# puzzlepaint/surfelmeshing

Measured on NVIDIA H100. Metric: RGB-D frames/s at 640x480 (depth pre-processing + Integrate()), higher is better.
Workload: dtype f32

## Files before the change

### surfelmeshing_b200/csrc/api.cu

```cuda

#include <algorithm>
#include <atomic>
#include <chrono>
#include <cstdio>
#include <cstdlib>
#include <cstring>
#include <limits>
#include <mutex>
#include <string>
#include <vector>

#include "sm_handle.cuh"

namespace smb {

namespace {
thread_local std::string g_last_error;
std::atomic<unsigned long long> g_launches{0};
}

int SetError(int code, const char* message) {
  g_last_error = message ? message : "";
  return code;
}
// ... 143 lines not shown
}

using namespace smb;

#define SM_CUDA(call)                                                                        \
  do {                                                                                       \
    const cudaError_t e_ = (call);                                                           \
    if (e_ != cudaSuccess) {                                                                 \
      g_last_error = std::string(#call) + ": " + cudaGetErrorString(e_);                     \
      return SM_ERR_CUDA;                                                                    \
    }                                                                                        \
  } while (0)

namespace smb {

int FetchCounters(sm_reconstruction* r, cudaStream_t stream) {
  SM_CUDA(cudaMemcpyAsync(r->host_counters, r->d.counters, sizeof(Counters), cudaMemcpyDeviceToHost, stream));
  SM_CUDA(cudaStreamSynchronize(stream));
  if (r->host_counters->capacity_overflow) {
    return SetError(SM_ERR_CAPACITY, "surfel cap exceeded: new surfels of at least one frame were dropped "
                                     "(the reference writes out of bounds here)");
  }
  return SM_OK;
}

FrameParams MakeFrameParams(const sm_reconstruction* r, u32 frame_index, int count_slot, const sm_integrate_params& p,
                            u16* depth, size_t depth_pitch, const u16* depth_pre, size_t depth_pre_pitch,
                            const float* normals, size_t normals_pitch, const float* radius, size_t radius_pitch,
                            const uint8_t* color, size_t color_pitch, const float* global_T_local,
                            const float* local_T_global) {
  FrameParams f;
  f.frame_index = frame_index;
  f.count_slot = count_slot;
  f.skip = 0;
  f.op_epoch = r->op_epoch;
  f.tb = MakeTieBreak(r->tiebreak, frame_index);
  f.active_window = p.surfel_integration_active_window_size;
  f.fx = r->fx; f.fy = r->fy; f.cx = r->cx; f.cy = r->cy;
  f.fx_inv = 1.0f / r->fx;
  f.fy_inv = 1.0f / r->fy;
  const float cx_pixel_center = r->cx - 0.5f;
  const float cy_pixel_center = r->cy - 0.5f;
  f.cx_inv = -cx_pixel_center / r->fx;
  f.cy_inv = -cy_pixel_center / r->fy;
  f.sensor_noise_factor = p.sensor_noise_factor;
  f.cos_normal_compatibility_threshold = cosf(M_PI / 180.0f * p.normal_compatibility_threshold_deg);
  f.max_surfel_confidence = p.max_surfel_confidence;
  f.inv_depth_scaling = 1.0f / p.depth_scaling;
  f.depth_scaling = 1.0f / f.inv_depth_scaling;
  f.radius_factor_squared =
      p.radius_factor_for_regularization_neighbors * p.radius_factor_for_regularization_neighbors;
  f.blend_radius = p.measurement_blending_radius;
  f.local_T_global = MakeMat3x4(local_T_global);
  f.global_T_local = MakeMat3x4(global_T_local);
  f.depth = depth; f.depth_pitch = depth_pitch;
  f.depth_pre = depth_pre; f.depth_pre_pitch = depth_pre_pitch;
  f.normals = reinterpret_cast<const float2*>(normals); f.normals_pitch = normals_pitch;
  f.radius = radius; f.radius_pitch = radius_pitch;
  f.color = reinterpret_cast<const uchar3*>(color); f.color_pitch = color_pitch;
  return f;
}

int IntegrateImpl(sm_reconstruction* r, cudaStream_t stream, u32 frame_index, const sm_integrate_params& p,
                  u16* depth, size_t depth_pitch, const float* normals, size_t normals_pitch, const float* radius,
                  size_t radius_pitch, const uint8_t* color, size_t color_pitch, const float* global_T_local,
                  const float* local_T_global) {
  r->last_stream = stream;
  RecordOperation(r, static_cast<int>(frame_index - static_cast<u32>(p.regularization_frame_window_size)));
  const u16* depth_pre = depth;
  size_t depth_pre_pitch = depth_pitch;
  if (p.do_blending) {
    SM_CUDA(cudaMemcpy2DAsync(r->blend_src, r->blend_src_pitch, depth, depth_pitch, r->d.width * sizeof(u16),
                              r->d.height, cudaMemcpyDeviceToDevice, stream));
    depth_pre = r->blend_src;
    depth_pre_pitch = r->blend_src_pitch;
  }
  const FrameParams f = MakeFrameParams(r, frame_index, r->count_slot, p, depth, depth_pitch, depth_pre, depth_pre_pitch,
                                        normals, normals_pitch, radius, radius_pitch, color, color_pitch,
                                        global_T_local, local_T_global);
  r->last_tiebreak = f.tb;
  int status = IntegrateFrame(stream, r->d, f, p.do_blending != 0, r->rasters_cleared, r->plan, &r->events);
  r->rasters_cleared = false;
  if (status != SM_OK) return status;
  const int old_slot = r->count_slot;
  r->count_slot = (r->count_slot + 1) % kCountSlots;
  if (r->events.enabled) cudaEventRecord(r->events.ev[12], stream);
  const int iterations = p.regularization_iterations_per_integration_iteration;
  if (iterations == 0) {
    status = RegularizeSurfels(stream, r->d,  true, frame_index,
                               p.radius_factor_for_regularization_neighbors, p.regularizer_weight,
                               p.regularization_frame_window_size, r->count_slot, old_slot, r->plan);
  } else {
    for (int i = 0; i < iterations && status == SM_OK; ++i) {
      status = RegularizeSurfels(stream, r->d,  false, frame_index,
                                 p.radius_factor_for_regularization_neighbors, p.regularizer_weight,
                                 p.regularization_frame_window_size, r->count_slot, i == 0 ? old_slot : -1, r->plan);
    }
  }
  if (r->events.enabled) cudaEventRecord(r->events.ev[13], stream);
  return status;
}

}

namespace {

int CreateImpl(sm_reconstruction* r, uint64_t max_surfel_count, int32_t width, int32_t height, float fx, float fy,
               float cx, float cy) {
  SM_CUDA(cudaGetDevice(&r->device));
  cudaDeviceProp prop;
  SM_CUDA(cudaGetDeviceProperties(&prop, r->device));
  r->sm_count = prop.multiProcessorCount;
  r->plan.sm_count = r->sm_count;
  {
    const char* e = std::getenv("SM_B200_CARVEOUT");
    const int percent = e ? std::atoi(e) : 47;
    int status = ConfigurePreprocessKernels(percent);
    if (status == SM_OK) status = ConfigureIntegrateKernels(percent, &r->plan);
    if (status == SM_OK) status = ConfigureRegularizeKernels(percent, &r->plan);
    if (status != SM_OK) return status;
  }
  r->fx = fx; r->fy = fy; r->cx = cx; r->cy = cy;
  DeviceState& d = r->d;
  d.width = width; d.height = height;
  d.capacity = static_cast<u32>(max_surfel_count);
  const size_t padded = (max_surfel_count + kSegment - 1) / kSegment * kSegment;
  d.stride = padded;
  const size_t P = static_cast<size_t>(width) * height;
  const size_t scan_tiles = (P + kSegment - 1) / kSegment;
  SM_CUDA(cudaMalloc(&d.surfels, sizeof(float) * SM_ROW_COUNT * d.stride));
  SM_CUDA(cudaMalloc(&d.gradient, sizeof(float4) * d.stride));
  SM_CUDA(cudaMalloc(&r->smooth_alt, sizeof(float) * 3 * d.stride));
  d.smooth = d.surfels + static_cast<size_t>(SM_ROW_SMOOTH_X) * d.stride;
  d.smooth_next = r->smooth_alt;
  SM_CUDA(cudaMemset(d.gradient, 0, sizeof(float4) * d.stride));
  for (int i = 0; i < kSets; ++i) {
    SM_CUDA(cudaMalloc(&r->assoc_set[i], sizeof(PixelAssoc) * P));
    SM_CUDA(cudaMalloc(&r->first_depth_set[i], sizeof(float) * P));
    SM_CUDA(cudaMalloc(&r->supported_set[i], P));
    SM_CUDA(cudaMalloc(&r->vis_set[i], sizeof(VisEntry) * padded));
    SM_CUDA(cudaMalloc(&r->seg_count_set[i], sizeof(u32) * (padded / kSegment)));
    SM_CUDA(cudaMalloc(&r->merge_flag_set[i], padded));
  }
  d.assoc = r->assoc_set[0]; d.first_depth = r->first_depth_set[0]; d.supported = r->supported_set[0];
  d.vis = r->vis_set[0]; d.seg_count = r->seg_count_set[0]; d.merge_flag = r->merge_flag_set[0];
  SM_CUDA(cudaMalloc(&d.new_list, sizeof(u32) * P));
  SM_CUDA(cudaMalloc(&d.new_flag, P));
  SM_CUDA(cudaMalloc(&d.new_index, sizeof(u32) * P));
  SM_CUDA(cudaMalloc(&d.scan_state, sizeof(unsigned long long) * scan_tiles));
  SM_CUDA(cudaMalloc(&d.counters, sizeof(Counters)));
  SM_CUDA(cudaMemset(d.counters, 0, sizeof(Counters)));
  d.timeline = nullptr;
  d.timeline_frames = 0;
  SM_CUDA(cudaMemset(d.new_flag, 0, P));
  SM_CUDA(cudaMemset(d.new_index, 0, sizeof(u32) * P));
  SM_CUDA(cudaMemset(d.scan_state, 0, sizeof(unsigned long long) * scan_tiles));
  SM_CUDA(cudaMallocHost(&r->host_counters, sizeof(Counters)));
  std::memset(r->host_counters, 0, sizeof(Counters));
  SM_CUDA(cudaMallocPitch(reinterpret_cast<void**>(&r->scratch_B), &r->scratch_B_pitch, width * sizeof(u16), height));
  SM_CUDA(cudaMallocPitch(reinterpret_cast<void**>(&r->blend_src), &r->blend_src_pitch, width * sizeof(u16), height));
  {
    const char* e = std::getenv("SM_B200_TAIL_FILL");
    const bool want_tma = !(e && std::string(e) == "vector");
    if (want_tma) {
      const int status = MakeDepthTensorMap(&r->scratch_B_map, r->scratch_B, r->scratch_B_pitch, width, height);
      if (status != SM_OK) return status;
      r->scratch_B_map_valid = true;
    }
  }
  for (int i = 0; i < 14; ++i) SM_CUDA(cudaEventCreate(&r->events.ev[i]));
  r->events.enabled = false;
  {
    u32 wave = kDefaultTieBreakWave, lanes = 1u << kDefaultTieBreakLaneShift;
    double early = kDefaultTieBreakEarlyFraction, index_order = kDefaultTieBreakIndexOrderFraction;
    u32 offset = kDefaultTieBreakWaveOffset;
    if (const char* e = std::getenv("SM_B200_TIEBREAK")) {
      unsigned w = 0, l = 0, o = 0; double q = 0, b = 0;
      const int got = std::sscanf(e, "%u,%lf,%lf,%u,%u", &w, &q, &b, &l, &o);
      if (got >= 2) { wave = w; early = q; }
      if (got >= 3) index_order = b;
      if (got >= 4) lanes = l;
      if (got >= 5) offset = o ? 1u : 0u;
    }
    r->tiebreak.wave_offset = offset;
    u32 lane_shift = 0;
    while ((1u << lane_shift) < lanes && lane_shift < 10) ++lane_shift;
    if (wave != 0 && (static_cast<unsigned long long>(d.capacity) / wave + 2) * 2ull * wave >= 0xFFFFFFFFull) wave = 0;
    r->tiebreak.lane_request = lane_shift;
    const int status = SetTieBreakWave(&r->tiebreak, wave, d.capacity);
    if (status != SM_OK) return status;
    r->tiebreak.early_fraction = early;
    r->tiebreak.index_order_fraction = index_order;
    r->tiebreak.early_fraction_later = kDefaultTieBreakEarlyFractionLater;
    r->tiebreak.index_order_fraction_later = kDefaultTieBreakIndexOrderFractionLater;
    r->tiebreak.early_fraction_second = kDefaultTieBreakEarlyFractionSecond;
  }
  const int status = ClearAssociationRasters(nullptr, d);
  if (status != SM_OK) return status;
  SM_CUDA(cudaDeviceSynchronize());
  return SM_OK;
}

}

extern "C" {

void sm_default_integrate_params(sm_integrate_params* p) {
  p->depth_scaling = 5000;
  p->sensor_noise_factor = 0.05f;
  p->max_surfel_confidence = 5.0f;
  p->regularizer_weight = 10.0f;
  p->regularization_frame_window_size = 30;
  p->do_blending = 1;
  p->measurement_blending_radius = 12;
  p->regularization_iterations_per_integration_iteration = 1;
  p->radius_factor_for_regularization_neighbors = 2;
  p->normal_compatibility_threshold_deg = 40;
  p->surfel_integration_active_window_size = std::numeric_limits<int>::max();
}

void sm_default_preprocess_params(sm_preprocess_params* p) {
  p->depth_scaling = 5000;
  p->max_depth = 3.0f;
  p->depth_valid_region_radius = 333;
  p->bilateral_filter_sigma_xy = 3;
  p->bilateral_filter_radius_factor = 2.0f;
  p->bilateral_filter_sigma_depth_factor = 0.05;
  p->outlier_filtering_frame_count = 8;
  p->outlier_filtering_required_inliers = -1;
  p->outlier_filtering_depth_tolerance_factor = 0.02f;
  p->depth_erosion_radius = 2;
  p->observation_angle_threshold_deg = 85;
  p->point_radius_extension_factor = 1.5f;
  p->point_radius_clamp_factor = std::numeric_limits<float>::infinity();
}

const char* sm_last_error(void) { return g_last_error.c_str(); }
const char* sm_version(void) { return "surfel_b200 0.1 (sm_90a)"; }
uint64_t sm_kernel_launch_count(void) { return g_launches.load(); }

int sm_profile_kernels(int32_t enable) {
  std::lock_guard<std::mutex> lock(g_profile_mutex);
  g_profile_enabled = enable != 0;
  return SM_OK;
}

int32_t sm_profile_kernel_count(void) { return KID_COUNT; }
const char* sm_profile_kernel_name(int32_t id) { return KernelName(id); }

int sm_profile_report(double* total_ms, uint64_t* launches, int32_t n) {
  SM_CUDA(cudaDeviceSynchronize());
  std::lock_guard<std::mutex> lock(g_profile_mutex);
  for (int i = 0; i < n; ++i) { total_ms[i] = 0; launches[i] = 0; }
  for (const ProfileRecord& r : g_profile_records) {
    float ms = 0;
    if (cudaEventElapsedTime(&ms, r.start, r.stop) == cudaSuccess && r.id < n) {
      total_ms[r.id] += ms;
      launches[r.id] += 1;
    }
    g_event_pool.push_back(r.start);
    g_event_pool.push_back(r.stop);
  }
  g_profile_records.clear();
  return SM_OK;
}

int sm_create(sm_reconstruction** out, uint64_t max_surfel_count, int32_t width, int32_t height, float fx, float fy,
              float cx, float cy) {
  if (out) *out = nullptr;
  if (!out || width <= 0 || height <= 0 || max_surfel_count == 0 || max_surfel_count > 0x7FFFFFFFull - kSegment) {
    return SetError(SM_ERR_INVALID_ARGUMENT, "sm_create: bad argument");
  }
  sm_reconstruction* r = new sm_reconstruction();
  const int status = CreateImpl(r, max_surfel_count, width, height, fx, fy, cx, cy);
  if (status != SM_OK) {
    const std::string message = g_last_error;
    sm_destroy(r);
    g_last_error = message;
    return status;
  }
  *out = r;
  return SM_OK;
}

int sm_destroy(sm_reconstruction* r) {
  if (!r) return SM_OK;
  cudaDeviceSynchronize();
  cudaGetLastError();
  DestroyFrameGraph(r->graph);
  DeviceState& d = r->d;
  cudaFree(d.surfels); cudaFree(d.gradient); cudaFree(r->smooth_alt); cudaFree(d.new_list);
  for (int i = 0; i < kSets; ++i) {
    cudaFree(r->vis_set[i]); cudaFree(r->seg_count_set[i]); cudaFree(r->merge_flag_set[i]);
    cudaFree(r->assoc_set[i]); cudaFree(r->first_depth_set[i]); cudaFree(r->supported_set[i]);
    cudaFree(r->run_depth[i]); cudaFree(r->run_depth_pre[i]); cudaFree(r->run_normals[i]); cudaFree(r->run_radius[i]);
  }
  cudaFree(d.new_flag); cudaFree(d.new_index); cudaFree(d.scan_state); cudaFree(d.counters);
  cudaFree(d.timeline);
  if (r->host_counters) cudaFreeHost(r->host_counters);
  cudaFree(r->scratch_B);
  cudaFree(r->blend_src);
  cudaFree(r->median_stage[0]); cudaFree(r->median_stage[1]);
  cudaFree(r->pyramid_depth_stage); cudaFree(r->pyramid_color_stage);
  FreeTransferBuffers(r);
  for (int i = 0; i < 2; ++i) {
    if (r->pipe.ev_create[i]) cudaEventDestroy(r->pipe.ev_create[i]);
    if (r->pipe.ev_update[i]) cudaEventDestroy(r->pipe.ev_update[i]);
    if (r->pre_done[i]) cudaEventDestroy(r->pre_done[i]);
    if (r->int_done[i]) cudaEventDestroy(r->int_done[i]);
  }
  for (cudaStream_t st : {r->pre_stream, r->pipe.crit, r->pipe.front, r->pipe.side, r->upload_stream, r->graph_stream})
    if (st) cudaStreamDestroy(st);
  for (cudaEvent_t e : {r->pipe.ev_assoc, r->pipe.ev_merge, r->pipe.ev_blend, r->pipe.ev_integrate, r->pipe.ev_reg,
                        r->entry_event, r->upload_done, r->graph_exit})
    if (e) cudaEventDestroy(e);
  for (cudaEvent_t e : r->iteration_done) if (e) cudaEventDestroy(e);
  for (u16* b : r->ring_depth) cudaFree(b);
  for (uchar3* b : r->ring_color) cudaFree(b);
  for (int i = 0; i < 14; ++i) if (r->events.ev[i]) cudaEventDestroy(r->events.ev[i]);
  delete r;
  cudaGetLastError();
  return SM_OK;
}

int sm_reset(sm_reconstruction* r, void* stream) {
  SM_CUDA(cudaMemsetAsync(r->d.counters, 0, sizeof(Counters), static_cast<cudaStream_t>(stream)));
  r->count_slot = 0;
  r->rasters_cleared = false;
  r->last_stream = static_cast<cudaStream_t>(stream);
  ++r->state_generation;
  r->op_history.clear();
  return SM_OK;
}

int sm_preprocess(sm_reconstruction* r, void* stream, const sm_preprocess_params* p, const uint16_t* raw_depth,
                  size_t raw_pitch, const uint16_t* const* other_depths, const size_t* other_pitches,
                  const float* others_TR_reference, uint16_t* out_depth, size_t out_depth_pitch, float* out_normals,
                  size_t out_normals_pitch, float* out_radius, size_t out_radius_pitch) {
  const int status = PreprocessFused(static_cast<cudaStream_t>(stream), *p, r->d.width, r->d.height, r->fx, r->fy,
                                     r->cx, r->cy, raw_depth, raw_pitch, other_depths, other_pitches,
                                     others_TR_reference, r->scratch_B, r->scratch_B_pitch, out_depth,
                                     out_depth_pitch, reinterpret_cast<float2*>(out_normals), out_normals_pitch,
                                     out_radius, out_radius_pitch, r->d.assoc, r->d.first_depth, r->d.supported, nullptr, 0,
                                     nullptr, nullptr, r->ScratchBMap());
  if (status == SM_OK) r->rasters_cleared = true;
  return status;
}

int sm_bilateral_filter_and_depth_cutoff(void* stream, float sigma_xy, float sigma_value_factor,
                                         uint16_t value_to_ignore, float radius_factor, uint16_t max_depth,
                                         float depth_valid_region_radius, int32_t width, int32_t height,
                                         const uint16_t* in_depth, size_t in_pitch, uint16_t* out_depth,
                                         size_t out_pitch) {
  return StageBilateral(static_cast<cudaStream_t>(stream), sigma_xy, sigma_value_factor, value_to_ignore,
                        radius_factor, max_depth, depth_valid_region_radius, width, height, in_depth, in_pitch,
                        out_depth, out_pitch);
}

int sm_outlier_depth_map_fusion(void* stream, int32_t other_count, int32_t required_count, float tolerance, float fx,
                                float fy, float cx, float cy, int32_t width, int32_t height, const uint16_t* in_depth,
                                size_t in_pitch, const uint16_t* const* other_depths, const size_t* other_pitches,
                                const float* others_TR_reference, uint16_t* out_depth, size_t out_pitch) {
  return StageOutlier(static_cast<cudaStream_t>(stream), other_count, required_count, tolerance, fx, fy, cx, cy,
                      width, height, in_depth, in_pitch, other_depths, other_pitches, others_TR_reference, out_depth,
                      out_pitch);
}

int sm_median_filter_and_densify_depth_map(void* stream, int32_t iterations, int32_t width, int32_t height,
                                           const uint16_t* in_depth, size_t in_pitch, uint16_t* out_depth,
                                           size_t out_pitch, uint16_t* scratch, size_t scratch_pitch) {
  return StageMedianDensify(static_cast<cudaStream_t>(stream), iterations, width, height, in_depth, in_pitch, out_depth,
                            out_pitch, scratch, scratch_pitch);
}

int sm_downscale_using_median_while_excluding(void* stream, uint16_t value_to_ignore, int32_t in_width,
                                              int32_t in_height, const uint16_t* in, size_t in_pitch,
// ... 62 lines not shown
  return status;
}

int sm_transfer_all_to_cpu(sm_reconstruction* r, void* stream_v, uint32_t , float* x, float* y,
                           float* z, float* radius_squared, float* nx, float* ny, float* nz,
                           uint32_t* last_update_stamp, uint64_t* out_count) {
  cudaStream_t stream = static_cast<cudaStream_t>(stream_v);
  const int status = FetchCounters(r, stream);
  const u32 n = r->host_counters->surfel_count[r->count_slot];
  if (out_count) *out_count = n;
  if (n == 0) return status;
  const size_t bytes = sizeof(float) * n;
  const float* s = r->d.surfels;
  const size_t st = r->d.stride;
  SM_CUDA(cudaMemcpyAsync(x, r->d.smooth + 0 * st, bytes, cudaMemcpyDeviceToHost, stream));
  SM_CUDA(cudaMemcpyAsync(y, r->d.smooth + 1 * st, bytes, cudaMemcpyDeviceToHost, stream));
  SM_CUDA(cudaMemcpyAsync(z, r->d.smooth + 2 * st, bytes, cudaMemcpyDeviceToHost, stream));
  SM_CUDA(cudaMemcpyAsync(radius_squared, s + SM_ROW_RADIUS_SQUARED * st, bytes, cudaMemcpyDeviceToHost, stream));
  SM_CUDA(cudaMemcpyAsync(nx, s + SM_ROW_NORMAL_X * st, bytes, cudaMemcpyDeviceToHost, stream));
  SM_CUDA(cudaMemcpyAsync(ny, s + SM_ROW_NORMAL_Y * st, bytes, cudaMemcpyDeviceToHost, stream));
  SM_CUDA(cudaMemcpyAsync(nz, s + SM_ROW_NORMAL_Z * st, bytes, cudaMemcpyDeviceToHost, stream));
  SM_CUDA(cudaMemcpyAsync(last_update_stamp, s + SM_ROW_LAST_UPDATE_STAMP * st, bytes, cudaMemcpyDeviceToHost, stream));
  return status;
}

int sm_transfer_delta_to_cpu(sm_reconstruction* r, void* stream, uint32_t frame_index, sm_transfer_token* token,
                             float* x, float* y, float* z, float* radius_squared, float* nx, float* ny, float* nz,
                             uint32_t* last_update_stamp, sm_transfer_stats* stats) {
  if (!r || !token) return SetError(SM_ERR_INVALID_ARGUMENT, "sm_transfer_delta_to_cpu: null argument");
  return TransferDelta(r, static_cast<cudaStream_t>(stream), frame_index, token, x, y, z, radius_squared, nx, ny, nz,
                       last_update_stamp, stats);
}

int sm_update_visualization_buffers(sm_reconstruction* r, void* stream, const sm_visualization_params* p,
                                    float* vertex_buffer, uint32_t* neighbor_index_buffer, float* normal_vertex_buffer) {
  if (!r || !p) return SetError(SM_ERR_INVALID_ARGUMENT, "sm_update_visualization_buffers: null argument");
  return UpdateVisualizationBuffers(r, static_cast<cudaStream_t>(stream), *p, vertex_buffer, neighbor_index_buffer,
                                    normal_vertex_buffer);
}

int sm_export_vertices(sm_reconstruction* r, void* stream, float* position_buffer, uint8_t* color_buffer) {
  return ExportVertices(static_cast<cudaStream_t>(stream), r->d, r->count_slot, r->sm_count, position_buffer,
                        color_buffer);
}

int sm_get_timings(sm_reconstruction* r, float out_ms[7]) {
  if (!r->events.enabled) return SetError(SM_ERR_INVALID_ARGUMENT, "timings are not enabled (sm_enable_timings)");
  SM_CUDA(cudaEventSynchronize(r->events.ev[13]));
  for (int i = 0; i < 7; ++i) SM_CUDA(cudaEventElapsedTime(&out_ms[i], r->events.ev[2 * i], r->events.ev[2 * i + 1]));
  return SM_OK;
}

int sm_enable_timings(sm_reconstruction* r, int32_t enable) {
  r->events.enabled = enable != 0;
  return SM_OK;
}

int sm_dump_state(sm_reconstruction* r, void* stream_v, float* host_rows, uint64_t host_row_stride_elems,
                  uint32_t* surfels_size, uint32_t* merge_count) {
  cudaStream_t stream = static_cast<cudaStream_t>(stream_v);
  const int status = FetchCounters(r, stream);
  const u32 n = r->host_counters->surfel_count[r->count_slot];
  if (surfels_size) *surfels_size = n;
  if (merge_count) *merge_count = r->host_counters->merge_count;
  if (host_rows && n > host_row_stride_elems) return SetError(SM_ERR_INVALID_ARGUMENT, "sm_dump_state: host rows shorter than surfels_size()");
  if (host_rows && n > 0) {
    SM_CUDA(cudaMemcpy2DAsync(host_rows, host_row_stride_elems * sizeof(float), r->d.surfels,
                              r->d.stride * sizeof(float), n * sizeof(float), SM_ROW_COUNT, cudaMemcpyDeviceToHost,
                              stream));
    SM_CUDA(cudaMemcpy2DAsync(host_rows + SM_ROW_SMOOTH_X * host_row_stride_elems, host_row_stride_elems * sizeof(float),
                              r->d.smooth, r->d.stride * sizeof(float), n * sizeof(float), 3, cudaMemcpyDeviceToHost,
                              stream));
    SM_CUDA(cudaStreamSynchronize(stream));
  }
  return status;
}

int sm_load_state(sm_reconstruction* r, void* stream_v, const float* host_rows, uint64_t host_row_stride_elems,
                  uint32_t surfels_size, uint32_t merge_count) {
  cudaStream_t stream = static_cast<cudaStream_t>(stream_v);
  if (surfels_size > r->d.capacity) return SetError(SM_ERR_CAPACITY, "sm_load_state: state larger than the surfel cap");
  r->d.smooth = r->d.surfels + static_cast<size_t>(SM_ROW_SMOOTH_X) * r->d.stride;
  r->d.smooth_next = r->smooth_alt;
  if (surfels_size > 0) {
    SM_CUDA(cudaMemcpy2DAsync(r->d.surfels, r->d.stride * sizeof(float), host_rows,
                              host_row_stride_elems * sizeof(float), surfels_size * sizeof(float), SM_ROW_COUNT,
                              cudaMemcpyHostToDevice, stream));
    SM_CUDA(cudaMemsetAsync(r->d.gradient, 0, surfels_size * sizeof(float4), stream));
    const int zero_rows[4] = {SM_ROW_GRADIENT_X, SM_ROW_GRADIENT_Y, SM_ROW_GRADIENT_Z, SM_ROW_GRADIENT_COUNT};
    for (int row : zero_rows) {
      SM_CUDA(cudaMemsetAsync(r->d.surfels + row * r->d.stride, 0, surfels_size * sizeof(float), stream));
    }
    SM_CUDA(cudaMemsetAsync(r->d.surfels + kRowMergeEpoch * r->d.stride, 0, surfels_size * sizeof(float), stream));
    const int status = RebuildMetaRow(stream, r->d, surfels_size, r->sm_count);
    if (status != SM_OK) return status;
  }
  Counters c{};
  for (int i = 0; i < kCountSlots; ++i) c.surfel_count[i] = surfels_size;
  c.merge_count = merge_count;
  *r->host_counters = c;
  SM_CUDA(cudaMemcpyAsync(r->d.counters, r->host_counters, sizeof(Counters), cudaMemcpyHostToDevice, stream));
  SM_CUDA(cudaStreamSynchronize(stream));
  r->count_slot = 0;
  r->last_stream = stream;
  ++r->state_generation;
  r->op_history.clear();
  return SM_OK;
}

int sm_download_rasters(sm_reconstruction* r, void* stream_v, uint32_t* supporting_surfels,
                        uint32_t* supporting_surfel_counts, float* supporting_surfel_depth_sums,
                        uint32_t* conflicting_surfels, float* first_surfel_depth, uint8_t* new_surfel_flag_vector,
                        uint32_t* new_surfel_indices) {
  cudaStream_t stream = static_cast<cudaStream_t>(stream_v);
  const size_t P = static_cast<size_t>(r->d.width) * r->d.height;
  std::vector<PixelAssoc> assoc(P);
  SM_CUDA(cudaMemcpyAsync(assoc.data(), r->d.assoc, sizeof(PixelAssoc) * P, cudaMemcpyDeviceToHost, stream));
  if (first_surfel_depth)
    SM_CUDA(cudaMemcpyAsync(first_surfel_depth, r->d.first_depth, sizeof(float) * P, cudaMemcpyDeviceToHost, stream));
  if (new_surfel_flag_vector)
    SM_CUDA(cudaMemcpyAsync(new_surfel_flag_vector, r->d.new_flag, P, cudaMemcpyDeviceToHost, stream));
  if (new_surfel_indices)
    SM_CUDA(cudaMemcpyAsync(new_surfel_indices, r->d.new_index, sizeof(u32) * P, cudaMemcpyDeviceToHost, stream));
  SM_CUDA(cudaStreamSynchronize(stream));
  for (size_t i = 0; i < P; ++i) {
    if (supporting_surfels) supporting_surfels[i] = supporting_index(r->last_tiebreak, assoc[i].x, static_cast<u32>(i));
    if (conflicting_surfels) conflicting_surfels[i] = assoc[i].y;
    if (supporting_surfel_counts) supporting_surfel_counts[i] = assoc[i].z;
    if (supporting_surfel_depth_sums) std::memcpy(&supporting_surfel_depth_sums[i], &assoc[i].w, sizeof(float));
  }
  return SM_OK;
}

int sm_frame_counters(sm_reconstruction* r, void* stream_v, uint64_t out[4]) {
  cudaStream_t stream = static_cast<cudaStream_t>(stream_v);
  const int status = FetchCounters(r, stream);
  const u32 n_after = r->host_counters->surfel_count[r->count_slot];
  const u32 n_swept = n_after - r->host_counters->new_surfel_count;
  const size_t segments = (static_cast<size_t>(n_swept) + kSegment - 1) / kSegment;
  std::vector<u32> seg(segments);
  if (segments) SM_CUDA(cudaMemcpy(seg.data(), r->d.seg_count, sizeof(u32) * segments, cudaMemcpyDeviceToHost));
  uint64_t visible = 0;
  for (u32 c : seg) visible += c;
  const size_t P = static_cast<size_t>(r->d.width) * r->d.height;
  std::vector<PixelAssoc> assoc(P);
  SM_CUDA(cudaMemcpy(assoc.data(), r->d.assoc, sizeof(PixelAssoc) * P, cudaMemcpyDeviceToHost));
  uint64_t support = 0;
  for (const PixelAssoc& a : assoc) support += a.z;
  out[0] = n_swept; out[1] = visible; out[2] = support; out[3] = r->host_counters->new_surfel_count;
  return status;
}

int sm_timeline_enable(sm_reconstruction* r, int32_t frames) {
  if (r == nullptr || frames < 0) return SetError(SM_ERR_INVALID_ARGUMENT, "sm_timeline_enable: bad arguments");
  SM_CUDA(cudaDeviceSynchronize());
  if (r->d.timeline) {
    cudaFree(r->d.timeline);
    r->d.timeline = nullptr;
    r->d.timeline_frames = 0;
  }
  if (frames == 0) return SM_OK;
  const size_t slots = static_cast<size_t>(frames) * KID_COUNT;
  SM_CUDA(cudaMalloc(&r->d.timeline, slots * 2 * sizeof(unsigned long long)));
  std::vector<unsigned long long> init(slots * 2);
  for (size_t i = 0; i < slots; ++i) { init[2 * i] = ~0ull; init[2 * i + 1] = 0ull; }
  SM_CUDA(cudaMemcpy(r->d.timeline, init.data(), init.size() * sizeof(unsigned long long), cudaMemcpyHostToDevice));
// ... 69 lines not shown
```

### surfelmeshing_b200/csrc/integrate.cu

```cuda

#include <algorithm>
#include <cstdio>
#include <cstdlib>

#include "sm_kernels.cuh"

namespace smb {

namespace {

#define SM_S(row, i) d.surfels[static_cast<size_t>(row) * d.stride + (i)]
#define SM_SU(row, i) reinterpret_cast<u32*>(d.surfels)[static_cast<size_t>(row) * d.stride + (i)]
#define SM_SMOOTH(axis, i) d.smooth[static_cast<size_t>(axis) * d.stride + (i)]

constexpr int kBlock = 256;

__device__ __forceinline__ bool is_active(u32 last_update_stamp, u32 frame_index, int window) {
  return static_cast<int>(last_update_stamp) > static_cast<int>(frame_index - static_cast<u32>(window));
}

struct Projection {
  float u, v;
  int px, py;
  bool in_image;
};

__device__ __forceinline__ Projection project(const FrameParams& f, int width, int height, float x, float y, float z) {
  Projection p;
  const float inv_z = frcp(z);
  p.u = ffma(fmul(x, inv_z), f.fx, f.cx);
  p.v = ffma(fmul(y, inv_z), f.fy, f.cy);
  p.px = f2i_trunc(p.u);
  p.py = f2i_trunc(p.v);
  p.in_image = !(p.u < 0.f || p.v < 0.f || p.px < 0 || p.py < 0 || p.px >= width || p.py >= height);
  return p;
}

__device__ __forceinline__ bool secondary_pixel(const Projection& p, int width, int height, int* ox, int* oy) {
  const float x_frac = fsub(p.u, i2f(p.px));
  const float y_frac = fsub(p.v, i2f(p.py));
  if (x_frac < y_frac) {
    if (x_frac < fadd(-y_frac, 1.0f)) {
      if (p.px > 1) { *ox = p.px - 1; *oy = p.py; return true; }
      return false;
    }
    if (p.py < height - 1) { *ox = p.px; *oy = p.py + 1; return true; }
    return false;
  }
  if (x_frac < fadd(-y_frac, 1.0f)) {
    if (p.py > 0) { *ox = p.px; *oy = p.py - 1; return true; }
    return false;
  }
  if (p.px < width - 1) { *ox = p.px + 1; *oy = p.py; return true; }
  return false;
}

__device__ __forceinline__ float normal_z_abs(float nx, float ny) {
  return fsqrt_approx(fmaxf(0.f, ffma(-ny, ny, ffma(-nx, nx, 1.0f))));
}

__device__ __forceinline__ float facing_dot(const FrameParams& f, float x, float y, float z, float nx, float ny,
                                            float nz, float3* local_normal) {
  const float rs = frsqrt_approx(squared_norm(x, y, z));
  *local_normal = rotate_vec(f.local_T_global, nx, ny, nz);
  return fmul(rs, ffma(z, local_normal->z, ffma(x, local_normal->x, fmul(y, local_normal->y))));
}

template <typename Body>
__device__ __forceinline__ void for_each_visible(const DeviceState& d, const u32* surfel_count, Body&& body) {
  constexpr u32 kItemsPerSegment = kSegment / kBlock;
  const u32 max_items = ((d.capacity + kSegment - 1) / kSegment) * kItemsPerSegment;
  const u32 n = *surfel_count;
  u32 item = blockIdx.x;
  u32 cnt = 0;
  VisEntry e = make_uint4(0u, 0u, 0u, 0u);
  if (item < max_items) {
    cnt = d.seg_count[item / kItemsPerSegment];
    e = d.vis[static_cast<size_t>(item) * kBlock + threadIdx.x];
  }
  const u32 items = ((n + kSegment - 1) / kSegment) * kItemsPerSegment;
  while (item < items) {
    const u32 next = item + gridDim.x;
    u32 cnt_next = 0;
    VisEntry e_next = e;
    if (next < items) {
      cnt_next = d.seg_count[next / kItemsPerSegment];
      e_next = d.vis[static_cast<size_t>(next) * kBlock + threadIdx.x];
    }
    const u32 k = (item % kItemsPerSegment) * kBlock + threadIdx.x;
    if (k < cnt) body(static_cast<size_t>(item) * kBlock + threadIdx.x, e);
    item = next;
    cnt = cnt_next;
    e = e_next;
  }
}

__global__ void __launch_bounds__(kBlock) k_clear(DeviceState d) {
  pdl_prologue();
  const int n = d.width * d.height;
  for (int i = blockIdx.x * blockDim.x + threadIdx.x; i < n; i += gridDim.x * blockDim.x) {
    d.assoc[i] = make_uint4(kInvalidIndex, kInvalidIndex, 0u, 0u);
    d.first_depth[i] = __int_as_float(0x7f800000);
    d.supported[i] = 0;
  }
}

constexpr int kProjectBlock = 512;

enum { kProjectAll = 0, kProjectMain = 1, kProjectTail = 2 };

__global__ void __launch_bounds__(kProjectBlock) k_project(DeviceState d, FrameParams f, int part) {
  pdl_prologue();
  if (f.skip) return;
  const TimelineScope timeline_scope(d, f.frame_index, part == kProjectTail ? KID_PROJECT_TAIL : KID_PROJECT);
  __shared__ u32 warp_totals[kProjectBlock / 32];
  const int lane = threadIdx.x & 31, warp = threadIdx.x >> 5;
  const u32 first_seg_if_all = blockIdx.x;

  if (blockIdx.x == 0 && part != kProjectMain) {
    const int tiles = (d.width * d.height + kSegment - 1) / kSegment;
    for (int t = threadIdx.x; t < tiles; t += blockDim.x) d.scan_state[t] = 0ull;
    if (threadIdx.x == 0) d.counters->scan_ticket = 0;
  }

  struct SlotRows { float2 X, Y, Z; uint2 T; };
  auto fetch = [&](u32 seg) {
    SlotRows r;
    const size_t base = static_cast<size_t>(seg) * kSegment + threadIdx.x * 2;
    r.X = *reinterpret_cast<const float2*>(&SM_S(SM_ROW_X, base));
    r.Y = *reinterpret_cast<const float2*>(&SM_S(SM_ROW_Y, base));
    r.Z = *reinterpret_cast<const float2*>(&SM_S(SM_ROW_Z, base));
    r.T = *reinterpret_cast<const uint2*>(&SM_SU(SM_ROW_LAST_UPDATE_STAMP, base));
    return r;
  };
  SlotRows rows = {};
  if (part != kProjectTail && (static_cast<size_t>(first_seg_if_all) + 1) * kSegment <= d.stride) rows = fetch(first_seg_if_all);
  const u32 n_before = part == kProjectAll ? 0u : d.counters->surfel_count[(f.count_slot + kCountSlots - 1) % kCountSlots];
  const u32 seg_begin = part == kProjectTail ? n_before / kSegment : 0u;
  const u32 n = part == kProjectMain ? (n_before / kSegment) * kSegment
                                     : d.counters->surfel_count[f.count_slot];
  if (part == kProjectTail && static_cast<u64>(seg_begin + blockIdx.x) * kSegment < n) rows = fetch(seg_begin + blockIdx.x);
  for (u32 seg = seg_begin + blockIdx.x; static_cast<u64>(seg) * kSegment < n; seg += gridDim.x) {
    const u32 base = seg * kSegment + threadIdx.x * 2;
    const SlotRows cur = rows;
    if (static_cast<u64>(seg + gridDim.x) * kSegment < n) rows = fetch(seg + gridDim.x);
    VisEntry e[2];
    bool visible[2] = {false, false};
    u32 cnt = 0;
    if (base < n) {
      const float xs[2] = {cur.X.x, cur.X.y}, ys[2] = {cur.Y.x, cur.Y.y}, zs[2] = {cur.Z.x, cur.Z.y};
      const u32 ts[2] = {cur.T.x, cur.T.y};
#pragma unroll
      for (int j = 0; j < 2; ++j) {
        const u32 i = base + j;
        if (i >= n) break;
        const float z = transform_row(f.local_T_global.r2, xs[j], ys[j], zs[j]);
        if (!(z > 0.f)) continue;
        const float x = transform_row(f.local_T_global.r0, xs[j], ys[j], zs[j]);
        const float y = transform_row(f.local_T_global.r1, xs[j], ys[j], zs[j]);
        const Projection p = project(f, d.width, d.height, x, y, z);
        if (!p.in_image) continue;
        const bool active = is_active(ts[j], f.frame_index, f.active_window);
        e[j] = make_uint4(i | (active ? kActiveBit : 0u), __float_as_uint(x), __float_as_uint(y), __float_as_uint(z));
        visible[j] = true;
        ++cnt;
        if (active) {
          atomicMin(reinterpret_cast<int*>(&d.first_depth[p.py * d.width + p.px]), __float_as_int(z));
          int ox, oy;
          if (secondary_pixel(p, d.width, d.height, &ox, &oy)) {
            atomicMin(reinterpret_cast<int*>(&d.first_depth[oy * d.width + ox]), __float_as_int(z));
          }
        }
      }
    }
    u32 incl = cnt;
#pragma unroll
    for (int o = 1; o < 32; o <<= 1) {
      const u32 t = __shfl_up_sync(0xffffffffu, incl, o);
      if (lane >= o) incl += t;
    }
    if (lane == 31) warp_totals[warp] = incl;
    __syncthreads();
    u32 warp_base = 0, total = 0;
#pragma unroll
    for (int w = 0; w < kProjectBlock / 32; ++w) {
      const u32 t = warp_totals[w];
      if (w < warp) warp_base += t;
      total += t;
    }
    VisEntry* out = d.vis + static_cast<size_t>(seg) * kSegment + warp_base + (incl - cnt);
#pragma unroll
    for (int j = 0; j < 2; ++j) {
      if (visible[j]) *out++ = e[j];
    }
    if (threadIdx.x == 0) d.seg_count[seg] = total;
    __syncthreads();
  }
}


struct PixelGate {
  float measurement_depth;
  float first;
  float2 normal;
};
// ... 504 lines not shown
}

__device__ __forceinline__ void integrate_or_conflict(const FrameParams& f, const PixelMeasurement& m, int x, int y,
                                                      u32 idx, float cx_, float cy_, float cz_, SurfelState& s) {
  if (!(m.measurement_depth > 0.f)) return;
  bool integrate = true, conflicting = false;
  if (m.first < fmul(m.measurement_depth, fadd(-f.sensor_noise_factor, 1.0f))) {
    if (m.first == cz_ && m.conflicting == idx) conflicting = true;
    integrate = false;
  }
  if (!integrate && !conflicting) return;
  if (cz_ > fmul(fadd(f.sensor_noise_factor, 1.0f), m.measurement_depth)) integrate = false;
  if (!integrate && !conflicting) return;

  const float lx = fmul(m.measurement_depth, ffma(i2f(x), f.fx_inv, f.cx_inv));
  const float ly = fmul(m.measurement_depth, ffma(i2f(y), f.fy_inv, f.cy_inv));
  const float3 g = transform_point(f.global_T_local, lx, ly, m.measurement_depth);
  const float3 gn = rotate_vec(f.global_T_local, m.normal.x, m.normal.y, -normal_z_abs(m.normal.x, m.normal.y));

  if (conflicting) {
    const float confidence = fadd(s.confidence, -1.0f);
    if (confidence <= 0.f) {
      s.x = g.x; s.y = g.y; s.z = g.z;
      s.smooth_x = g.x; s.smooth_y = g.y; s.smooth_z = g.z;
      s.nx = gn.x; s.ny = gn.y; s.nz = gn.z;
      s.color = m.r | (m.g << 8) | (m.b << 16) | (1u << 24);
      s.radius_squared = m.radius_squared;
      s.confidence = 1.0f;
      s.creation_stamp = f.frame_index;
      s.stamped = true;
      s.replaced = true;
    } else {
      s.confidence = confidence;
    }
    s.dirty = true;
  }
  if (!integrate) return;

  float3 ln;
  if (facing_dot(f, cx_, cy_, cz_, s.nx, s.ny, s.nz, &ln) > 0.f) return;
  if (m.measurement_depth < cz_) {
    if (ffma(gn.z, s.nz, ffma(gn.x, s.nx, fmul(gn.y, s.ny))) < f.cos_normal_compatibility_threshold) return;
  }
  if (s.radius_squared < 0.f) return;

  const float weight = frcp(u2f(max(1u, m.count)));
  if (s.creation_stamp < f.frame_index) {
    const float confidence = s.confidence;
    const float cw = fadd(weight, confidence);
    s.confidence = (cw < f.max_surfel_confidence) ? cw : f.max_surfel_confidence;
    const float normalization_factor = frcp(cw);
    s.x = fmul(normalization_factor, ffma(g.x, weight, fmul(confidence, s.x)));
    s.y = fmul(normalization_factor, ffma(g.y, weight, fmul(confidence, s.y)));
    s.z = fmul(normalization_factor, ffma(g.z, weight, fmul(confidence, s.z)));
    const float nx = ffma(gn.x, weight, fmul(confidence, s.nx));
    const float ny = ffma(gn.y, weight, fmul(confidence, s.ny));
    const float nz = ffma(gn.z, weight, fmul(confidence, s.nz));
    const float normal_normalization = frsqrt_approx(ffma(nz, nz, ffma(nx, nx, fmul(ny, ny))));
    s.nx = fmul(nx, normal_normalization);
    s.ny = fmul(ny, normal_normalization);
    s.nz = fmul(nz, normal_normalization);
    s.radius_squared = fminf(s.radius_squared, m.radius_squared);
    const u32 old_color = s.color;
    const u32 r = f2u_trunc(ffma(normalization_factor, ffma(u2f(m.r), weight, fmul(confidence, u2f(old_color & 0xFFu))), 0.5f));
    const u32 gr = f2u_trunc(ffma(normalization_factor, ffma(u2f(m.g), weight, fmul(confidence, u2f((old_color >> 8) & 0xFFu))), 0.5f));
    const u32 b = f2u_trunc(ffma(normalization_factor, ffma(u2f(m.b), weight, fmul(confidence, u2f((old_color >> 16) & 0xFFu))), 0.5f));
    s.color = (r & 0xFFu) | ((gr & 0xFFu) << 8) | ((b & 0xFFu) << 16);
    s.stamped = true;
    s.dirty = true;
  }
}

#ifndef SM_INTEGRATE_LEVELS
#define SM_INTEGRATE_LEVELS 2
#endif

__device__ __forceinline__ bool pixel_can_touch(const FrameParams& f, float measurement_depth, float first, u32 conflicting,
                                                u32 idx, float cz_) {
  if (!(measurement_depth > 0.f)) return false;
  if (first < fmul(measurement_depth, fadd(-f.sensor_noise_factor, 1.0f))) return first == cz_ && conflicting == idx;
  return !(cz_ > fmul(fadd(f.sensor_noise_factor, 1.0f), measurement_depth));
}

__global__ void __launch_bounds__(kBlock, 4) k_integrate(DeviceState d, FrameParams f) {
  pdl_prologue();
  if (f.skip) return;
  const TimelineScope timeline_scope(d, f.frame_index, KID_INTEGRATE);
  for_each_visible(d, &d.counters->surfel_count[f.count_slot], [&](size_t pos, const VisEntry& e) {
    const u32 idx = e.x & ~kActiveBit;
    const float x = __uint_as_float(e.y), y = __uint_as_float(e.z), z = __uint_as_float(e.w);
    const Projection p = project(f, d.width, d.height, x, y, z);
    int ox = p.px, oy = p.py;
    const bool has2 = secondary_pixel(p, d.width, d.height, &ox, &oy);
    const u8 merged = d.merge_flag[pos];
    SurfelState s;
    PixelMeasurement m0, m1;
#if SM_INTEGRATE_LEVELS == 1
    m0 = load_pixel_measurement(d, f, p.px, p.py);
    m1 = load_pixel_measurement(d, f, ox, oy);
    s.x = SM_S(SM_ROW_X, idx); s.y = SM_S(SM_ROW_Y, idx); s.z = SM_S(SM_ROW_Z, idx);
    s.confidence = SM_S(SM_ROW_CONFIDENCE, idx);
    s.radius_squared = SM_S(SM_ROW_RADIUS_SQUARED, idx);
    s.nx = SM_S(SM_ROW_NORMAL_X, idx); s.ny = SM_S(SM_ROW_NORMAL_Y, idx); s.nz = SM_S(SM_ROW_NORMAL_Z, idx);
    s.color = SM_SU(SM_ROW_COLOR, idx);
    s.creation_stamp = SM_SU(SM_ROW_CREATION_STAMP, idx);
#else
    const int p0 = p.py * d.width + p.px, p1 = oy * d.width + ox;
    m0.measurement_depth = fmul(u2f(row_ptr(f.depth, f.depth_pitch, p.py)[p.px]), f.inv_depth_scaling);
    m1.measurement_depth = fmul(u2f(row_ptr(f.depth, f.depth_pitch, oy)[ox]), f.inv_depth_scaling);
    m0.first = d.first_depth[p0];
    m1.first = d.first_depth[p1];
    const PixelAssoc a0 = d.assoc[p0], a1 = d.assoc[p1];
    m0.conflicting = a0.y; m0.count = a0.z;
    m1.conflicting = a1.y; m1.count = a1.z;
    s.radius_squared = SM_S(SM_ROW_RADIUS_SQUARED, idx);
#endif
    s.last_update_stamp = 0;
    s.smooth_x = s.smooth_y = s.smooth_z = 0.f;
    s.replaced = false; s.dirty = false; s.stamped = false;
    if (merged) {
      SM_SU(SM_ROW_LAST_UPDATE_STAMP, idx) = 0;
      SM_S(SM_ROW_RADIUS_SQUARED, idx) = -1.0f;
      reinterpret_cast<u8*>(&SM_SU(SM_ROW_COLOR, idx))[3] = 1;
      SM_SU(kRowMeta, idx) = kMetaDetachBit;
      SM_SU(kRowMergeEpoch, idx) = f.op_epoch;
      return;
    }
    if (!(e.x & kActiveBit)) return;
    if (s.radius_squared < 0.f) return;
#if SM_INTEGRATE_LEVELS != 1
    const bool touch0 = pixel_can_touch(f, m0.measurement_depth, m0.first, m0.conflicting, idx, z);
    const bool touch1 = has2 && pixel_can_touch(f, m1.measurement_depth, m1.first, m1.conflicting, idx, z);
    if (!touch0 && !touch1) return;
    {
      const int qx0 = touch0 ? p.px : ox, qy0 = touch0 ? p.py : oy;
      const int qx1 = touch1 ? ox : qx0, qy1 = touch1 ? oy : qy0;
      m0.normal = row_ptr(f.normals, f.normals_pitch, qy0)[qx0];
      m1.normal = row_ptr(f.normals, f.normals_pitch, qy1)[qx1];
      m0.radius_squared = row_ptr(f.radius, f.radius_pitch, qy0)[qx0];
      m1.radius_squared = row_ptr(f.radius, f.radius_pitch, qy1)[qx1];
      const uchar3 c0 = row_ptr(f.color, f.color_pitch, qy0)[qx0];
      const uchar3 c1 = row_ptr(f.color, f.color_pitch, qy1)[qx1];
      m0.r = c0.x; m0.g = c0.y; m0.b = c0.z;
      m1.r = c1.x; m1.g = c1.y; m1.b = c1.z;
      s.x = SM_S(SM_ROW_X, idx); s.y = SM_S(SM_ROW_Y, idx); s.z = SM_S(SM_ROW_Z, idx);
      s.confidence = SM_S(SM_ROW_CONFIDENCE, idx);
      s.nx = SM_S(SM_ROW_NORMAL_X, idx); s.ny = SM_S(SM_ROW_NORMAL_Y, idx); s.nz = SM_S(SM_ROW_NORMAL_Z, idx);
      s.color = SM_SU(SM_ROW_COLOR, idx);
      s.creation_stamp = SM_SU(SM_ROW_CREATION_STAMP, idx);
    }
    if (touch0) integrate_or_conflict(f, m0, p.px, p.py, idx, x, y, z, s);
    if (touch1) integrate_or_conflict(f, m1, ox, oy, idx, x, y, z, s);
#else
    integrate_or_conflict(f, m0, p.px, p.py, idx, x, y, z, s);
    if (has2) integrate_or_conflict(f, m1, ox, oy, idx, x, y, z, s);
#endif
    if (!s.dirty) return;
    SM_S(SM_ROW_X, idx) = s.x; SM_S(SM_ROW_Y, idx) = s.y; SM_S(SM_ROW_Z, idx) = s.z;
    SM_S(SM_ROW_CONFIDENCE, idx) = s.confidence;
    SM_S(SM_ROW_RADIUS_SQUARED, idx) = s.radius_squared;
    SM_S(SM_ROW_NORMAL_X, idx) = s.nx; SM_S(SM_ROW_NORMAL_Y, idx) = s.ny; SM_S(SM_ROW_NORMAL_Z, idx) = s.nz;
    SM_SU(SM_ROW_COLOR, idx) = s.color;
    if (s.stamped) {
      SM_SU(SM_ROW_LAST_UPDATE_STAMP, idx) = f.frame_index;
      SM_SU(kRowMeta, idx) = f.frame_index | (((s.color >> 24) & 1u) ? kMetaDetachBit : 0u);
    }
    if (s.replaced) {
      SM_SMOOTH(0, idx) = s.smooth_x; SM_SMOOTH(1, idx) = s.smooth_y; SM_SMOOTH(2, idx) = s.smooth_z;
      SM_SU(SM_ROW_CREATION_STAMP, idx) = f.frame_index;
#pragma unroll
      for (int i = 0; i < 4; ++i) SM_SU(SM_ROW_NEIGHBOR0 + i, idx) = kInvalidIndex;
    }
  });
}

#ifndef SM_UPDATE_ANYNEW_FIRST
#define SM_UPDATE_ANYNEW_FIRST 0
#endif
#ifndef SM_UPDATE_EARLY_GATE
#define SM_UPDATE_EARLY_GATE 1
#endif
#ifndef SM_UPDATE_COMPACT
#define SM_UPDATE_COMPACT 0
#endif

#ifndef SM_UPDATE_COMPACT_MIN_BLOCKS
#define SM_UPDATE_COMPACT_MIN_BLOCKS 3
#endif
#if SM_UPDATE_COMPACT
__device__ __forceinline__ void update_neighbors_survivor(const DeviceState& d, const FrameParams& f, u32 idx, int x, int y) {
  const int kDirectionsX[4] = {-1, 1, 0, 0};
  const int kDirectionsY[4] = {0, 0, -1, 1};
  const float gx = SM_S(SM_ROW_X, idx), gy = SM_S(SM_ROW_Y, idx), gz = SM_S(SM_ROW_Z, idx);
  const float nx = SM_S(SM_ROW_NORMAL_X, idx), ny = SM_S(SM_ROW_NORMAL_Y, idx), nz = SM_S(SM_ROW_NORMAL_Z, idx);
  const float radius_squared = SM_S(SM_ROW_RADIUS_SQUARED, idx);
  u32 neighbor_surfel_indices[4];
#pragma unroll
  for (int m = 0; m < 4; ++m) neighbor_surfel_indices[m] = SM_SU(SM_ROW_NEIGHBOR0 + m, idx);
  const float observation_radius_squared = row_ptr(f.radius, f.radius_pitch, y)[x];
  u32 candidate[4];
#pragma unroll
  for (int direction = 0; direction < 4; ++direction) {
    const int candidate_pixel = (y + kDirectionsY[direction]) * d.width + x + kDirectionsX[direction];
    candidate[direction] = supporting_index(f.tb, d.assoc[candidate_pixel].x, static_cast<u32>(candidate_pixel));
  }
  const float cz_ = transform_row(f.local_T_global.r2, gx, gy, gz);
  const float cx_ = transform_row(f.local_T_global.r0, gx, gy, gz);
  const float cy_ = transform_row(f.local_T_global.r1, gx, gy, gz);
  float3 ln;
  if (facing_dot(f, cx_, cy_, cz_, nx, ny, nz, &ln) > 0.f) return;
  if (radius_squared < 0.f) return;
  if (fmul(observation_radius_squared, frcp(radius_squared)) > 2.25f) return;
  bool any_new = false;
#pragma unroll
  for (int direction = 0; direction < 4; ++direction) {
    const u32 q = candidate[direction];
    if (q == kInvalidIndex || q == idx) { candidate[direction] = kInvalidIndex; continue; }
    any_new |= q != neighbor_surfel_indices[0] && q != neighbor_surfel_indices[1] &&
               q != neighbor_surfel_indices[2] && q != neighbor_surfel_indices[3];
  }
  if (!any_new) return;

  float neighbor_distances_squared[4];
#pragma unroll
  for (int m = 0; m < 4; ++m) {
    const u32 q = neighbor_surfel_indices[m];
    if (q == kInvalidIndex) {
      neighbor_distances_squared[m] = __int_as_float(0x7f800000);
    } else {
      neighbor_distances_squared[m] = squared_norm(fsub(gx, SM_S(SM_ROW_X, q)), fsub(gy, SM_S(SM_ROW_Y, q)),
                                                   fsub(gz, SM_S(SM_ROW_Z, q)));
    }
  }
  const float max_distance_squared = fmul(radius_squared, f.radius_factor_squared);
  float cand_distance[4], cand_dot[4];
#pragma unroll
  for (int direction = 0; direction < 4; ++direction) {
    const u32 q = candidate[direction];
    if (q == kInvalidIndex) continue;
    cand_distance[direction] = squared_norm(fsub(SM_S(SM_ROW_X, q), gx), fsub(SM_S(SM_ROW_Y, q), gy),
                                            fsub(SM_S(SM_ROW_Z, q), gz));
    cand_dot[direction] = dot3(nx, ny, nz, SM_S(SM_ROW_NORMAL_X, q), SM_S(SM_ROW_NORMAL_Y, q), SM_S(SM_ROW_NORMAL_Z, q));
  }
  bool changed = false;
#pragma unroll
  for (int direction = 0; direction < 4; ++direction) {
    const u32 q = candidate[direction];
    if (q == kInvalidIndex) continue;
    const float distance_squared = cand_distance[direction];
    if (distance_squared > max_distance_squared) continue;
    if (cand_dot[direction] <= 0.f) continue;
    int best_n = -1;
    float best_distance_squared = -1.f;
#pragma unroll
    for (int m = 0; m < 4; ++m) {
      if (q == neighbor_surfel_indices[m]) { best_n = -1; break; }
      if (neighbor_distances_squared[m] > best_distance_squared) {
        best_n = m;
        best_distance_squared = neighbor_distances_squared[m];
      }
    }
    if (best_n >= 0 && distance_squared < best_distance_squared) {
#pragma unroll
      for (int m = 0; m < 4; ++m) {
        if (m == best_n) { neighbor_surfel_indices[m] = q; neighbor_distances_squared[m] = distance_squared; }
      }
      changed = true;
    }
  }
  if (changed) {
#pragma unroll
    for (int m = 0; m < 4; ++m) SM_SU(SM_ROW_NEIGHBOR0 + m, idx) = neighbor_surfel_indices[m];
  }
}

__global__ void __launch_bounds__(kBlock, SM_UPDATE_COMPACT_MIN_BLOCKS) k_update_neighbors(DeviceState d, FrameParams f) {
  pdl_prologue();
  if (f.skip) return;
  const TimelineScope timeline_scope(d, f.frame_index, KID_UPDATE_NEIGHBORS);
  constexpr int kPerThread = kSegment / kBlock;
  constexpr int kBorder = 1;
  __shared__ u32 s_survivor[kSegment];
  __shared__ u32 s_pixel[kSegment];
  __shared__ u32 s_count;
  const u32 n = d.counters->surfel_count[f.count_slot];
  const u32 segments = (n + kSegment - 1) / kSegment;
  const int lane = threadIdx.x & 31;
  for (u32 segment = blockIdx.x; segment < segments; segment += gridDim.x) {
    if (threadIdx.x == 0) s_count = 0;
    __syncthreads();
    const u32 cnt = d.seg_count[segment];
    u32 surfel[kPerThread], stamp[kPerThread];
    float gx[kPerThread], gy[kPerThread], gz[kPerThread];
    u16 raw_depth[kPerThread];
    int cached_px[kPerThread], cached_py[kPerThread];
    bool live[kPerThread];
    {
      VisEntry e[kPerThread];
#pragma unroll
      for (int u = 0; u < kPerThread; ++u) {
        const u32 k = u * kBlock + threadIdx.x;
        live[u] = k < cnt;
        if (live[u]) e[u] = d.vis[static_cast<size_t>(segment) * kSegment + k];
      }
#pragma unroll
      for (int u = 0; u < kPerThread; ++u) {
        if (!live[u]) continue;
        surfel[u] = e[u].x & ~kActiveBit;
        const Projection cached = project(f, d.width, d.height, __uint_as_float(e[u].y), __uint_as_float(e[u].z), __uint_as_float(e[u].w));
        cached_px[u] = cached.px;
        cached_py[u] = cached.py;
      }
    }
#pragma unroll
    for (int u = 0; u < kPerThread; ++u) {
      if (!live[u]) continue;
      const u32 idx = surfel[u];
      stamp[u] = SM_SU(SM_ROW_LAST_UPDATE_STAMP, idx);
      gx[u] = SM_S(SM_ROW_X, idx); gy[u] = SM_S(SM_ROW_Y, idx); gz[u] = SM_S(SM_ROW_Z, idx);
      raw_depth[u] = row_ptr(f.depth, f.depth_pitch, cached_py[u])[cached_px[u]];
    }
#pragma unroll
    for (int u = 0; u < kPerThread; ++u) {
      bool pass = live[u];
      int x = 0, y = 0;
      if (pass) pass = is_active(stamp[u], f.frame_index, f.active_window);
      if (pass) {
        const float cz_ = transform_row(f.local_T_global.r2, gx[u], gy[u], gz[u]);
        pass = cz_ > 0.f;
        if (pass) {
          const float cx_ = transform_row(f.local_T_global.r0, gx[u], gy[u], gz[u]);
          const float cy_ = transform_row(f.local_T_global.r1, gx[u], gy[u], gz[u]);
          const float inv_z = frcp(cz_);
          x = f2i_trunc(ffma(fmul(cx_, inv_z), f.fx, f.cx));
          y = f2i_trunc(ffma(fmul(cy_, inv_z), f.fy, f.cy));
          pass = !(x < kBorder || y < kBorder || x >= d.width - kBorder || y >= d.height - kBorder);
          if (pass) {
            u16 depth_here = raw_depth[u];
            if (x != cached_px[u] || y != cached_py[u]) depth_here = row_ptr(f.depth, f.depth_pitch, y)[x];
            const float measurement_depth = fmul(u2f(depth_here), f.inv_depth_scaling);
            pass = !(cz_ > fmul(measurement_depth, fadd(f.sensor_noise_factor, 1.0f)));
          }
        }
      }
      const unsigned ballot = __ballot_sync(0xFFFFFFFFu, pass);
      if (ballot) {
        u32 base = 0;
        if (lane == 0) base = atomicAdd(&s_count, static_cast<u32>(__popc(ballot)));
        base = __shfl_sync(0xFFFFFFFFu, base, 0);
        if (pass) {
          const u32 slot = base + __popc(ballot & ((1u << lane) - 1u));
          s_survivor[slot] = surfel[u];
          s_pixel[slot] = static_cast<u32>(x) | (static_cast<u32>(y) << 16);
        }
      }
    }
    __syncthreads();
    const u32 survivors = s_count;
    for (u32 q = threadIdx.x; q < survivors; q += kBlock) {
      const u32 pixel = s_pixel[q];
      update_neighbors_survivor(d, f, s_survivor[q], static_cast<int>(pixel & 0xFFFFu), static_cast<int>(pixel >> 16));
    }
    __syncthreads();
  }
}
#else
__global__ void __launch_bounds__(kBlock) k_update_neighbors(DeviceState d, FrameParams f) {
  pdl_prologue();
  if (f.skip) return;
  const TimelineScope timeline_scope(d, f.frame_index, KID_UPDATE_NEIGHBORS);
  for_each_visible(d, &d.counters->surfel_count[f.count_slot], [&](size_t, const VisEntry& e) {
    const u32 idx = e.x & ~kActiveBit;
    constexpr int kBorder = 1;
    const int kDirectionsX[4] = {-1, 1, 0, 0};
    const int kDirectionsY[4] = {0, 0, -1, 1};
#if SM_UPDATE_EARLY_GATE
    const Projection cached = project(f, d.width, d.height, __uint_as_float(e.y), __uint_as_float(e.z), __uint_as_float(e.w));
    const u32 stamp = SM_SU(SM_ROW_LAST_UPDATE_STAMP, idx);
    const float gx = SM_S(SM_ROW_X, idx), gy = SM_S(SM_ROW_Y, idx), gz = SM_S(SM_ROW_Z, idx);
    u16 raw_depth = row_ptr(f.depth, f.depth_pitch, cached.py)[cached.px];
    if (!is_active(stamp, f.frame_index, f.active_window)) return;
    const float cz_ = transform_row(f.local_T_global.r2, gx, gy, gz);
    if (!(cz_ > 0.f)) return;
    const float cx_ = transform_row(f.local_T_global.r0, gx, gy, gz);
    const float cy_ = transform_row(f.local_T_global.r1, gx, gy, gz);
    const float inv_z = frcp(cz_);
    const int x = f2i_trunc(ffma(fmul(cx_, inv_z), f.fx, f.cx));
    const int y = f2i_trunc(ffma(fmul(cy_, inv_z), f.fy, f.cy));
    if (x < kBorder || y < kBorder || x >= d.width - kBorder || y >= d.height - kBorder) return;
    if (x != cached.px || y != cached.py) raw_depth = row_ptr(f.depth, f.depth_pitch, y)[x];
    const float measurement_depth = fmul(u2f(raw_depth), f.inv_depth_scaling);
    if (cz_ > fmul(measurement_depth, fadd(f.sensor_noise_factor, 1.0f))) return;
#if SM_UPDATE_ANYNEW_FIRST
    u32 neighbor_surfel_indices[4];
#pragma unroll
    for (int m = 0; m < 4; ++m) neighbor_surfel_indices[m] = SM_SU(SM_ROW_NEIGHBOR0 + m, idx);
    u32 candidate[4];
#pragma unroll
    for (int direction = 0; direction < 4; ++direction) {
      const int candidate_pixel = (y + kDirectionsY[direction]) * d.width + x + kDirectionsX[direction];
      candidate[direction] = supporting_index(f.tb, d.assoc[candidate_pixel].x, static_cast<u32>(candidate_pixel));
    }
    {
      bool any_new_first = false;
#pragma unroll
      for (int direction = 0; direction < 4; ++direction) {
        const u32 q = candidate[direction];
        if (q == kInvalidIndex || q == idx) continue;
        any_new_first |= q != neighbor_surfel_indices[0] && q != neighbor_surfel_indices[1] &&
                         q != neighbor_surfel_indices[2] && q != neighbor_surfel_indices[3];
      }
      if (!any_new_first) return;
    }
    const float nx = SM_S(SM_ROW_NORMAL_X, idx), ny = SM_S(SM_ROW_NORMAL_Y, idx), nz = SM_S(SM_ROW_NORMAL_Z, idx);
    const float radius_squared = SM_S(SM_ROW_RADIUS_SQUARED, idx);
    const float observation_radius_squared = row_ptr(f.radius, f.radius_pitch, y)[x];
#else
    const float nx = SM_S(SM_ROW_NORMAL_X, idx), ny = SM_S(SM_ROW_NORMAL_Y, idx), nz = SM_S(SM_ROW_NORMAL_Z, idx);
    const float radius_squared = SM_S(SM_ROW_RADIUS_SQUARED, idx);
    u32 neighbor_surfel_indices[4];
#pragma unroll
    for (int m = 0; m < 4; ++m) neighbor_surfel_indices[m] = SM_SU(SM_ROW_NEIGHBOR0 + m, idx);
    const float observation_radius_squared = row_ptr(f.radius, f.radius_pitch, y)[x];
    u32 candidate[4];
#pragma unroll
    for (int direction = 0; direction < 4; ++direction) {
      const int candidate_pixel = (y + kDirectionsY[direction]) * d.width + x + kDirectionsX[direction];
      candidate[direction] = supporting_index(f.tb, d.assoc[candidate_pixel].x, static_cast<u32>(candidate_pixel));
    }
#endif
#else
    const u32 stamp = SM_SU(SM_ROW_LAST_UPDATE_STAMP, idx);
    const float gx = SM_S(SM_ROW_X, idx), gy = SM_S(SM_ROW_Y, idx), gz = SM_S(SM_ROW_Z, idx);
    const float nx = SM_S(SM_ROW_NORMAL_X, idx), ny = SM_S(SM_ROW_NORMAL_Y, idx), nz = SM_S(SM_ROW_NORMAL_Z, idx);
    const float radius_squared = SM_S(SM_ROW_RADIUS_SQUARED, idx);
    u32 neighbor_surfel_indices[4];
#pragma unroll
    for (int m = 0; m < 4; ++m) neighbor_surfel_indices[m] = SM_SU(SM_ROW_NEIGHBOR0 + m, idx);
    if (!is_active(stamp, f.frame_index, f.active_window)) return;
    const float cz_ = transform_row(f.local_T_global.r2, gx, gy, gz);
    if (!(cz_ > 0.f)) return;
    const float cx_ = transform_row(f.local_T_global.r0, gx, gy, gz);
    const float cy_ = transform_row(f.local_T_global.r1, gx, gy, gz);
    const float inv_z = frcp(cz_);
    const int x = f2i_trunc(ffma(fmul(cx_, inv_z), f.fx, f.cx));
    const int y = f2i_trunc(ffma(fmul(cy_, inv_z), f.fy, f.cy));
    if (x < kBorder || y < kBorder || x >= d.width - kBorder || y >= d.height - kBorder) return;

    const float measurement_depth = fmul(u2f(row_ptr(f.depth, f.depth_pitch, y)[x]), f.inv_depth_scaling);
    const float observation_radius_squared = row_ptr(f.radius, f.radius_pitch, y)[x];
    u32 candidate[4];
#pragma unroll
    for (int direction = 0; direction < 4; ++direction) {
      const int candidate_pixel = (y + kDirectionsY[direction]) * d.width + x + kDirectionsX[direction];
      candidate[direction] = supporting_index(f.tb, d.assoc[candidate_pixel].x, static_cast<u32>(candidate_pixel));
    }
    if (cz_ > fmul(measurement_depth, fadd(f.sensor_noise_factor, 1.0f))) return;
#endif
    float3 ln;
    if (facing_dot(f, cx_, cy_, cz_, nx, ny, nz, &ln) > 0.f) return;
    if (radius_squared < 0.f) return;
    if (fmul(observation_radius_squared, frcp(radius_squared)) > 2.25f) return;
    bool any_new = false;
#pragma unroll
    for (int direction = 0; direction < 4; ++direction) {
      const u32 q = candidate[direction];
      if (q == kInvalidIndex || q == idx) { candidate[direction] = kInvalidIndex; continue; }
      any_new |= q != neighbor_surfel_indices[0] && q != neighbor_surfel_indices[1] &&
                 q != neighbor_surfel_indices[2] && q != neighbor_surfel_indices[3];
    }
    if (!any_new) return;

    float neighbor_distances_squared[4];
#pragma unroll
    for (int m = 0; m < 4; ++m) {
      const u32 q = neighbor_surfel_indices[m];
      if (q == kInvalidIndex) {
        neighbor_distances_squared[m] = __int_as_float(0x7f800000);
      } else {
        neighbor_distances_squared[m] = squared_norm(fsub(gx, SM_S(SM_ROW_X, q)), fsub(gy, SM_S(SM_ROW_Y, q)),
                                                     fsub(gz, SM_S(SM_ROW_Z, q)));
      }
    }
    const float max_distance_squared = fmul(radius_squared, f.radius_factor_squared);
    float cand_distance[4], cand_dot[4];
#pragma unroll
    for (int direction = 0; direction < 4; ++direction) {
      const u32 q = candidate[direction];
      if (q == kInvalidIndex) continue;
      cand_distance[direction] = squared_norm(fsub(SM_S(SM_ROW_X, q), gx), fsub(SM_S(SM_ROW_Y, q), gy),
                                              fsub(SM_S(SM_ROW_Z, q), gz));
      cand_dot[direction] = dot3(nx, ny, nz, SM_S(SM_ROW_NORMAL_X, q), SM_S(SM_ROW_NORMAL_Y, q), SM_S(SM_ROW_NORMAL_Z, q));
    }
    bool changed = false;
#pragma unroll
    for (int direction = 0; direction < 4; ++direction) {
      const u32 q = candidate[direction];
      if (q == kInvalidIndex) continue;
      const float distance_squared = cand_distance[direction];
      if (distance_squared > max_distance_squared) continue;
      if (cand_dot[direction] <= 0.f) continue;
      int best_n = -1;
      float best_distance_squared = -1.f;
#pragma unroll
      for (int m = 0; m < 4; ++m) {
        if (q == neighbor_surfel_indices[m]) { best_n = -1; break; }
        if (neighbor_distances_squared[m] > best_distance_squared) {
          best_n = m;
          best_distance_squared = neighbor_distances_squared[m];
        }
      }
      if (best_n >= 0 && distance_squared < best_distance_squared) {
#pragma unroll
        for (int m = 0; m < 4; ++m) {
          if (m == best_n) { neighbor_surfel_indices[m] = q; neighbor_distances_squared[m] = distance_squared; }
        }
        changed = true;
      }
    }
    if (changed) {
#pragma unroll
      for (int m = 0; m < 4; ++m) SM_SU(SM_ROW_NEIGHBOR0 + m, idx) = neighbor_surfel_indices[m];
    }
  });
}
#endif

__device__ __forceinline__ unsigned long long load_scan_state(unsigned long long* p) { return atomicAdd(p, 0ull); }

__global__ void __launch_bounds__(kBlock) k_new_surfel_scan(DeviceState d, FrameParams f) {
  pdl_prologue();
  if (f.skip) return;
  const TimelineScope timeline_scope(d, f.frame_index, KID_NEW_SURFEL_SCAN);
  __shared__ u32 s_tile, s_prefix;
  __shared__ u32 warp_totals[kBlock / 32];
  const int total_pixels = d.width * d.height;
  const int tiles = (total_pixels + kSegment - 1) / kSegment;
  if (threadIdx.x == 0) s_tile = atomicAdd(&d.counters->scan_ticket, 1u);
  __syncthreads();
  const u32 tile = s_tile;
  if (tile >= static_cast<u32>(tiles)) return;

  const int base = tile * kSegment + threadIdx.x * 4;
  u32 flags[4];
  u32 cnt = 0;
#pragma unroll
  for (int j = 0; j < 4; ++j) {
    const int seq = base + j;
    u32 flag = 0;
    if (seq < total_pixels) {
      const int y = seq / d.width, x = seq - y * d.width;
      constexpr int kBorder = 1;
      if (x >= kBorder && y >= kBorder && x < d.width - kBorder && y < d.height - kBorder &&
          row_ptr(f.depth, f.depth_pitch, y)[x] > 0 && !d.supported[seq]) {
        flag = (d.assoc[seq].y == kInvalidIndex) ? 1u : 0u;
      }
    }
    flags[j] = flag;
    cnt += flag;
  }
  const int lane = threadIdx.x & 31, warp = threadIdx.x >> 5;
  u32 incl = cnt;
#pragma unroll
  for (int o = 1; o < 32; o <<= 1) {
    const u32 t = __shfl_up_sync(0xffffffffu, incl, o);
    if (lane >= o) incl += t;
  }
  if (lane == 31) warp_totals[warp] = incl;
  __syncthreads();
  u32 warp_base = 0, block_total = 0;
#pragma unroll
  for (int w = 0; w < kBlock / 32; ++w) {
    const u32 t = warp_totals[w];
    if (w < warp) warp_base += t;
    block_total += t;
  }
  if (warp == 0) {
    if (lane == 0) atomicExch(&d.scan_state[tile], ((tile == 0 ? 2ull : 1ull) << 32) | block_total);
    u32 exclusive = 0;
    int window_end = static_cast<int>(tile) - 1;
    while (window_end >= 0) {
      const int t = window_end - lane;
      unsigned long long v = 2ull << 32;
      if (t >= 0) {
        do { v = load_scan_state(&d.scan_state[t]); } while ((v >> 32) == 0ull);
      }
      const unsigned inclusive_mask = __ballot_sync(0xffffffffu, (v >> 32) == 2ull);
      const int first_inclusive = __ffs(inclusive_mask) - 1;
      const u32 contribution = (first_inclusive < 0 || lane <= first_inclusive) ? static_cast<u32>(v) : 0u;
      exclusive += __reduce_add_sync(0xffffffffu, contribution);
      if (first_inclusive >= 0) break;
      window_end -= 32;
    }
    if (lane == 0) {
      if (tile != 0) atomicExch(&d.scan_state[tile], (2ull << 32) | (exclusive + block_total));
      s_prefix = exclusive;
      if (tile == static_cast<u32>(tiles) - 1) {
        const u32 n_old = d.counters->surfel_count[f.count_slot];
        u32 new_count = exclusive + block_total;
        if (static_cast<u64>(n_old) + new_count > d.capacity) {
          d.counters->capacity_overflow = 1;
          new_count = 0;
        }
        d.counters->new_surfel_count = new_count;
        d.counters->surfel_count[(f.count_slot + 1) % kCountSlots] = n_old + new_count;
      }
    }
  }
  __syncthreads();
// ... 5 lines not shown
      d.new_flag[seq] = static_cast<u8>(flags[j]);
      d.new_index[seq] = running;
      if (flags[j]) d.new_list[running] = seq;
    }
    running += flags[j];
  }
}

__global__ void __launch_bounds__(kBlock) k_create_surfels(DeviceState d, FrameParams f) {
  pdl_prologue();
  if (f.skip) return;
  const TimelineScope timeline_scope(d, f.frame_index, KID_CREATE_SURFELS);
  const u32 new_count = d.counters->new_surfel_count;
  const u32 surfel_count = d.counters->surfel_count[f.count_slot];
  for (u32 k = blockIdx.x * blockDim.x + threadIdx.x; k < new_count; k += gridDim.x * blockDim.x) {
    const int seq = d.new_list[k];
    const int y = seq / d.width, x = seq - y * d.width;
    const u32 idx = surfel_count + k;
    const float depth = fmul(u2f(row_ptr(f.depth, f.depth_pitch, y)[x]), f.inv_depth_scaling);
    const float2 nm = row_ptr(f.normals, f.normals_pitch, y)[x];
    const uchar3 color = row_ptr(f.color, f.color_pitch, y)[x];
    const float radius_squared = row_ptr(f.radius, f.radius_pitch, y)[x];
    const int kDirectionsX[4] = {-1, 1, 0, 0};
    const int kDirectionsY[4] = {0, 0, -1, 1};
    u32 neighbor_index[4], neighbor_new_index[4];
    u8 neighbor_is_new[4];
    u16 neighbor_depth[4];
#pragma unroll
    for (int direction = 0; direction < 4; ++direction) {
      const int nx_ = x + kDirectionsX[direction], ny_ = y + kDirectionsY[direction];
      const int nseq = ny_ * d.width + nx_;
      neighbor_index[direction] = supporting_index(f.tb, d.assoc[nseq].x, static_cast<u32>(nseq));
      neighbor_is_new[direction] = d.new_flag[nseq];
      neighbor_new_index[direction] = d.new_index[nseq];
      neighbor_depth[direction] = row_ptr(f.depth, f.depth_pitch, ny_)[nx_];
    }
    const float lx = fmul(depth, ffma(i2f(x), f.fx_inv, f.cx_inv));
    const float ly = fmul(depth, ffma(u2f(y), f.fy_inv, f.cy_inv));
    const float3 g = transform_point(f.global_T_local, lx, ly, depth);
    const float3 gn = rotate_vec(f.global_T_local, nm.x, nm.y, -normal_z_abs(nm.x, nm.y));
    const float max_distance_squared = fmul(radius_squared, f.radius_factor_squared);
    float ndist[4], nsx[4], nsy[4], nsz[4];
#pragma unroll
    for (int direction = 0; direction < 4; ++direction) {
      const u32 q = neighbor_index[direction];
      if (q == kInvalidIndex) continue;
      ndist[direction] = squared_norm(fsub(SM_S(SM_ROW_X, q), g.x), fsub(SM_S(SM_ROW_Y, q), g.y), fsub(SM_S(SM_ROW_Z, q), g.z));
      nsx[direction] = SM_SMOOTH(0, q);
      nsy[direction] = SM_SMOOTH(1, q);
      nsz[direction] = SM_SMOOTH(2, q);
    }
    float sum_x = 0.f, sum_y = 0.f, sum_z = 0.f;
    int existing_neighbor_count_plus_1 = 1;
#pragma unroll
    for (int direction = 0; direction < 4; ++direction) {
      u32 q = neighbor_index[direction];
      if (q != kInvalidIndex) {
        if (ndist[direction] > max_distance_squared) {
          q = kInvalidIndex;
        } else {
          sum_x = fadd(sum_x, nsx[direction]);
          sum_y = fadd(sum_y, nsy[direction]);
          sum_z = fadd(sum_z, nsz[direction]);
          ++existing_neighbor_count_plus_1;
        }
      } else if (neighbor_is_new[direction] == 1) {
        const float diff = ffma(-u2f(neighbor_depth[direction]), f.inv_depth_scaling, depth);
        if (!(fmul(diff, diff) > max_distance_squared)) q = surfel_count + neighbor_new_index[direction];
      }
      SM_SU(SM_ROW_NEIGHBOR0 + direction, idx) = q;
    }
    SM_S(SM_ROW_X, idx) = g.x; SM_S(SM_ROW_Y, idx) = g.y; SM_S(SM_ROW_Z, idx) = g.z;
    SM_S(SM_ROW_NORMAL_X, idx) = gn.x; SM_S(SM_ROW_NORMAL_Y, idx) = gn.y; SM_S(SM_ROW_NORMAL_Z, idx) = gn.z;
    SM_SU(SM_ROW_COLOR, idx) = color.x | (color.y << 8) | (color.z << 16);
    SM_S(SM_ROW_CONFIDENCE, idx) = 1.0f;
    SM_SU(SM_ROW_CREATION_STAMP, idx) = f.frame_index;
    SM_SU(SM_ROW_LAST_UPDATE_STAMP, idx) = f.frame_index;
    SM_SU(kRowMeta, idx) = f.frame_index;
    SM_S(SM_ROW_RADIUS_SQUARED, idx) = radius_squared;
    SM_S(SM_ROW_GRADIENT_X, idx) = 0.f; SM_S(SM_ROW_GRADIENT_Y, idx) = 0.f; SM_S(SM_ROW_GRADIENT_Z, idx) = 0.f;
    SM_S(SM_ROW_GRADIENT_COUNT, idx) = 0.f;
    d.gradient[idx] = make_float4(0.f, 0.f, 0.f, 0.f);
    const float rcp_count = frcp(i2f(existing_neighbor_count_plus_1));
    SM_SMOOTH(0, idx) = fmul(fadd(g.x, sum_x), rcp_count);
    SM_SMOOTH(1, idx) = fmul(fadd(g.y, sum_y), rcp_count);
    SM_SMOOTH(2, idx) = fmul(fadd(g.z, sum_z), rcp_count);
  }
}

__global__ void __launch_bounds__(kBlock) k_export_vertices(DeviceState d, int count_slot, float* position_buffer,
                                                            u8* color_buffer) {
  pdl_prologue();
  const u32 n = d.counters->surfel_count[count_slot];
  for (u32 i = blockIdx.x * blockDim.x + threadIdx.x; i < n; i += gridDim.x * blockDim.x) {
    const bool merged = SM_S(SM_ROW_RADIUS_SQUARED, i) < 0.f;
    const float nan = __int_as_float(0x7fffffff);
    position_buffer[3 * i + 0] = merged ? nan : SM_SMOOTH(0, i);
    position_buffer[3 * i + 1] = merged ? nan : SM_SMOOTH(1, i);
    position_buffer[3 * i + 2] = merged ? nan : SM_SMOOTH(2, i);
    const u32 c = SM_SU(SM_ROW_COLOR, i);
    color_buffer[3 * i + 0] = c & 0xFF;
    color_buffer[3 * i + 1] = (c >> 8) & 0xFF;
    color_buffer[3 * i + 2] = (c >> 16) & 0xFF;
  }
}

}

namespace {
size_t BlendSmemBytes(int radius) {
  const size_t rw = kBlendTileW + 2 * blend_halo_x(radius), rh = kBlendTileH + 2 * blend_halo_y(radius);
  const size_t rn16 = (rw * rh + 15) & ~static_cast<size_t>(15);
  const size_t mask_words = rh * ((rw + 31) / 32);
  return rn16 * 14 + mask_words * 11 * 4 + 16;
}
constexpr size_t kBlendSmemLimit = 224 * 1024;

#define SM_EV(call)                                                              \
  do {                                                                           \
    const cudaError_t e_ = (call);                                               \
    if (e_ != cudaSuccess) return SetError(SM_ERR_CUDA, cudaGetErrorString(e_)); \
  } while (0)
}

int DescribeFrameKernel(FrameKernel which, const LaunchPlan& plan, const DeviceState& d, const FrameParams& f,
                        KernelLaunch* out) {
  static_assert(sizeof(DeviceState) + sizeof(FrameParams) + 32 <= sizeof(out->storage), "KernelLaunch::storage too small");
  const int scan_tiles = (d.width * d.height + kSegment - 1) / kSegment;
  switch (which) {
    case FK_PROJECT:
    case FK_PROJECT_MAIN:
      out->Reset(reinterpret_cast<const void*>(k_project), dim3(plan.project), dim3(kProjectBlock), 0, KID_PROJECT);
      break;
    case FK_PROJECT_TAIL:
      out->Reset(reinterpret_cast<const void*>(k_project), dim3(plan.sm_count), dim3(kProjectBlock), 0, KID_PROJECT_TAIL);
      break;
    case FK_ASSOCIATE:
      out->Reset(reinterpret_cast<const void*>(k_associate), dim3(plan.associate), dim3(kBlock), 0, KID_ASSOCIATE);
      break;
    case FK_MERGE:
      out->Reset(reinterpret_cast<const void*>(k_merge), dim3(plan.merge), dim3(kBlock), 0, KID_MERGE);
      break;
    case FK_BLEND: {
      const size_t smem = BlendSmemBytes(f.blend_radius);
      if (f.blend_radius < 1 || f.blend_radius > kMaxBlendRadius || smem > kBlendSmemLimit)
        return SetError(SM_ERR_INVALID_ARGUMENT, "measurement_blending_radius too large for one tile region per SM");
      const dim3 pixel_tiles((d.width + kBlendTileW - 1) / kBlendTileW, (d.height + kBlendTileH - 1) / kBlendTileH);
      out->Reset(reinterpret_cast<const void*>(k_blend), pixel_tiles, dim3(kBlendBlock), smem, KID_BLEND);
      break;
    }
    case FK_INTEGRATE:
      out->Reset(reinterpret_cast<const void*>(k_integrate), dim3(plan.integrate), dim3(kBlock), 0, KID_INTEGRATE);
      break;
    case FK_UPDATE_NEIGHBORS:
      out->Reset(reinterpret_cast<const void*>(k_update_neighbors), dim3(plan.update_neighbors), dim3(kBlock), 0,
                 KID_UPDATE_NEIGHBORS);
      break;
    case FK_SCAN:
      out->Reset(reinterpret_cast<const void*>(k_new_surfel_scan), dim3(scan_tiles), dim3(kBlock), 0, KID_NEW_SURFEL_SCAN);
      break;
    case FK_CREATE:
      out->Reset(reinterpret_cast<const void*>(k_create_surfels), dim3(plan.sm_count * 2), dim3(kBlock), 0, KID_CREATE_SURFELS);
      break;
    default:
      return SetError(SM_ERR_INVALID_ARGUMENT, "DescribeFrameKernel");
  }
  out->Arg(d);
  out->Arg(f);
  if (which == FK_PROJECT) out->Arg(static_cast<int>(kProjectAll));
// ... 2 lines not shown
  return SM_OK;
}

namespace {
int LaunchFrameKernel(cudaStream_t stream, FrameKernel which, const LaunchPlan& plan, const DeviceState& d,
                      const FrameParams& f, bool dependent) {
  KernelLaunch k;
  const int status = DescribeFrameKernel(which, plan, d, f, &k);
  if (status != SM_OK) return status;
  LaunchOnStream(stream, k, dependent);
  return SM_OK;
}
}

int ClearAssociationRasters(cudaStream_t stream, const DeviceState& d) {
  const int blocks = (d.width * d.height + kBlock * 4 - 1) / (kBlock * 4);
  { LaunchScope scope(stream, KID_CLEAR); LaunchKernel(k_clear, dim3(blocks), dim3(kBlock), 0, stream, d); }
  return CheckLaunch("clear");
}

int IntegrateFrame(cudaStream_t stream, const DeviceState& d, const FrameParams& f, bool do_blending,
                   bool rasters_already_cleared, const LaunchPlan& plan, const IntegrateEvents* events) {
  const bool timed = events && events->enabled;
  auto record = [&](int i) { if (timed) cudaEventRecord(events->ev[i], stream); };
  int status = SM_OK;
  auto launch = [&](FrameKernel which, bool dependent) {
    if (status == SM_OK) status = LaunchFrameKernel(stream, which, plan, d, f, dependent);
  };
  record(0);
  if (!rasters_already_cleared) {
    status = ClearAssociationRasters(stream, d);
    if (status != SM_OK) return status;
  }
  launch(FK_PROJECT, false);
  launch(FK_ASSOCIATE, true);
  record(1); record(2);
  launch(FK_MERGE, false);
  record(3); record(4);
  if (do_blending) launch(FK_BLEND, true);
  record(5); record(6);
  launch(FK_INTEGRATE, false);
  record(7); record(8);
  launch(FK_UPDATE_NEIGHBORS, false);
  record(9); record(10);
  launch(FK_SCAN, false);
  launch(FK_CREATE, false);
  record(11);
  if (status != SM_OK) return status;
  return CheckLaunch("integrate");
}

int IntegrateFramePipelined(cudaStream_t stream, PipelineCtx* pc, int set, DeviceState& d, const FrameParams& f,
                            bool do_blending, const RegularizeArgs& reg, const LaunchPlan& plan) {
  cudaStream_t crit = pc->crit, side = pc->side;
  int status = SM_OK;
  auto launch = [&](cudaStream_t s, FrameKernel which, bool dependent) {
    if (status == SM_OK) status = LaunchFrameKernel(s, which, plan, d, f, dependent);
  };
  if (pc->have_frame) SM_EV(cudaStreamWaitEvent(stream, pc->ev_create[set ^ 1], 0));
  launch(stream, FK_PROJECT, false);
  launch(stream, FK_ASSOCIATE, true);
  SM_EV(cudaEventRecord(pc->ev_assoc, stream));
  SM_EV(cudaStreamWaitEvent(side, pc->ev_assoc, 0));
  launch(side, FK_MERGE, false);
  SM_EV(cudaEventRecord(pc->ev_merge, side));
  if (do_blending) launch(stream, FK_BLEND, true);
  SM_EV(cudaEventRecord(pc->ev_blend, stream));
  SM_EV(cudaStreamWaitEvent(side, pc->ev_blend, 0));
  launch(side, FK_SCAN, false);
  SM_EV(cudaStreamWaitEvent(crit, pc->ev_blend, 0));
  SM_EV(cudaStreamWaitEvent(crit, pc->ev_merge, 0));
  launch(crit, FK_INTEGRATE, false);
  SM_EV(cudaEventRecord(pc->ev_integrate, crit));
  launch(crit, FK_UPDATE_NEIGHBORS, true);
  SM_EV(cudaEventRecord(pc->ev_update[set], crit));
  SM_EV(cudaStreamWaitEvent(side, pc->ev_integrate, 0));
  launch(side, FK_CREATE, false);
  SM_EV(cudaEventRecord(pc->ev_create[set], side));
  SM_EV(cudaStreamWaitEvent(crit, pc->ev_create[set], 0));
  if (status != SM_OK) return status;
  status = CheckLaunch("integrate (pipelined)");
  if (status != SM_OK) return status;
  const int old_slot = f.count_slot, new_slot = (f.count_slot + 1) % kCountSlots;
  if (reg.disable_denoising) {
    status = RegularizeSurfels(crit, d, true, f.frame_index, reg.radius_factor, reg.regularizer_weight, reg.window,
                               new_slot, old_slot, plan);
  } else {
    for (int i = 0; i < reg.iterations && status == SM_OK; ++i) {
      status = RegularizeSurfels(crit, d, false, f.frame_index, reg.radius_factor, reg.regularizer_weight, reg.window,
                                 new_slot, i == 0 ? old_slot : -1, plan);
    }
  }
  SM_EV(cudaEventRecord(pc->ev_reg, crit));
  pc->have_frame = true;
  return status;
}

int ExportVertices(cudaStream_t stream, const DeviceState& d, int count_slot, int sm_count, float* position_buffer,
                   u8* color_buffer) {
  { LaunchScope scope(stream, KID_EXPORT_VERTICES); LaunchKernel(k_export_vertices, dim3(sm_count * 8), dim3(kBlock), 0, stream, d, count_slot, position_buffer, color_buffer); }
  return CheckLaunch("export vertices");
}

int ConfigureIntegrateKernels(int carveout_percent, LaunchPlan* plan) {
  if (carveout_percent >= 0) {
    cudaFuncSetAttribute(k_clear, cudaFuncAttributePreferredSharedMemoryCarveout, carveout_percent);
    cudaFuncSetAttribute(k_project, cudaFuncAttributePreferredSharedMemoryCarveout, carveout_percent);
    cudaFuncSetAttribute(k_associate, cudaFuncAttributePreferredSharedMemoryCarveout, carveout_percent);
    cudaFuncSetAttribute(k_merge, cudaFuncAttributePreferredSharedMemoryCarveout, carveout_percent);
    cudaFuncSetAttribute(k_blend, cudaFuncAttributePreferredSharedMemoryCarveout, carveout_percent);
    cudaFuncSetAttribute(k_integrate, cudaFuncAttributePreferredSharedMemoryCarveout, carveout_percent);
    cudaFuncSetAttribute(k_update_neighbors, cudaFuncAttributePreferredSharedMemoryCarveout, carveout_percent);
    cudaFuncSetAttribute(k_new_surfel_scan, cudaFuncAttributePreferredSharedMemoryCarveout, carveout_percent);
    cudaFuncSetAttribute(k_create_surfels, cudaFuncAttributePreferredSharedMemoryCarveout, carveout_percent);
    cudaFuncSetAttribute(k_export_vertices, cudaFuncAttributePreferredSharedMemoryCarveout, carveout_percent);
    cudaGetLastError();
  }
  if (cudaFuncSetAttribute(k_blend, cudaFuncAttributeMaxDynamicSharedMemorySize, static_cast<int>(kBlendSmemLimit)) != cudaSuccess) {
    return SetError(SM_ERR_CUDA, "cudaFuncSetAttribute(k_blend, MaxDynamicSharedMemorySize)");
  }
  const int sm_count = plan->sm_count;
  const char* e = std::getenv("SM_B200_RESIDENT_GRIDS");
  if (e && e[0] == '0') {
    plan->project = sm_count * 4;
    plan->associate = plan->merge = plan->integrate = plan->update_neighbors = sm_count * 8;
    return SM_OK;
  }
  auto resident = [&](auto kernel, int block, int fallback_per_sm) {
    int per_sm = 0;
    if (cudaOccupancyMaxActiveBlocksPerMultiprocessor(&per_sm, kernel, block, 0) != cudaSuccess || per_sm < 1) {
      cudaGetLastError();
      per_sm = fallback_per_sm;
    }
    return ScaleGrid(sm_count * per_sm);
  };
  plan->project = resident(k_project, kProjectBlock, 2);
  plan->associate = resident(k_associate, kBlock, 8);
  plan->merge = resident(k_merge, kBlock, 4);
  plan->integrate = resident(k_integrate, kBlock, 3);
  plan->update_neighbors = resident(k_update_neighbors, kBlock, 3);
#if SM_UPDATE_COMPACT
  plan->update_neighbors = ScaleGrid(sm_count * 8);
#endif
  if (const char* pe = std::getenv("SM_B200_OFFCHAIN_GRID_PERCENT")) {
    const int percent = std::atoi(pe);
    if (percent > 0 && percent < 100) {
      plan->update_neighbors = std::max(sm_count, plan->update_neighbors * percent / 100);
      plan->merge = std::max(sm_count, plan->merge * percent / 100);
    }
  }
  return SM_OK;
}

}
```

### surfelmeshing_b200/csrc/pipeline.cu

```cuda

#include <chrono>
#include <cstdio>
#include <cstdlib>
#include <string>

#include "sm_handle.cuh"

namespace smb {

namespace {

#define SM_CUDA(call)                                                                                   \
  do {                                                                                                  \
    const cudaError_t e_ = (call);                                                                      \
    if (e_ != cudaSuccess) return SetError(SM_ERR_CUDA, (std::string(#call) + ": " + cudaGetErrorString(e_)).c_str()); \
  } while (0)

constexpr int kDepthRing = 16;
constexpr int kColorRing = 6;
constexpr int kIterationEvents = 32;

int EnvInt(const char* name, int fallback) {
  const char* e = std::getenv(name);
  return (e && e[0]) ? std::atoi(e) : fallback;
// ... 22 lines not shown
    SM_CUDA(cudaEventCreateWithFlags(&r->graph_exit, cudaEventDisableTiming));
    int least_priority = 0, greatest_priority = 0;
    SM_CUDA(cudaDeviceGetStreamPriorityRange(&least_priority, &greatest_priority));
    const int prio_mode = EnvInt("SM_B200_PRIO", 0);
    SM_CUDA(cudaStreamCreateWithPriority(&r->pipe.crit, cudaStreamNonBlocking, prio_mode >= 1 ? greatest_priority : least_priority));
    SM_CUDA(cudaStreamCreateWithPriority(&r->pipe.side, cudaStreamNonBlocking, prio_mode >= 1 ? greatest_priority : least_priority));
    SM_CUDA(cudaStreamCreateWithPriority(&r->pipe.front, cudaStreamNonBlocking, prio_mode >= 2 ? greatest_priority : least_priority));
    for (cudaEvent_t* e : {&r->pipe.ev_assoc, &r->pipe.ev_merge, &r->pipe.ev_blend, &r->pipe.ev_integrate,
                           &r->pipe.ev_reg}) {
      SM_CUDA(cudaEventCreateWithFlags(e, cudaEventDisableTiming));
    }
  }
  if ((on_host || depth_ring) && !r->upload_stream) {
    SM_CUDA(cudaStreamCreateWithFlags(&r->upload_stream, cudaStreamNonBlocking));
    SM_CUDA(cudaEventCreateWithFlags(&r->upload_done, cudaEventDisableTiming));
    r->iteration_done.assign(kIterationEvents, nullptr);
    for (auto& e : r->iteration_done) SM_CUDA(cudaEventCreateWithFlags(&e, cudaEventDisableTiming));
  }
  if (depth_ring && r->ring_depth.empty()) {
    r->ring_depth.assign(kDepthRing, nullptr);
    for (auto& b : r->ring_depth) {
      SM_CUDA(cudaMallocPitch(reinterpret_cast<void**>(&b), &r->ring_depth_pitch, W * sizeof(u16), H));
    }
  }
  if (color_ring && r->ring_color.empty()) {
    r->ring_color.assign(kColorRing, nullptr);
    for (auto& b : r->ring_color) {
      SM_CUDA(cudaMallocPitch(reinterpret_cast<void**>(&b), &r->ring_color_pitch, W * 3, H));
    }
  }
  if (on_host && r->pyramid_level > 0 &&
      (r->pyramid_stage_width != source_width || r->pyramid_stage_height != source_height)) {
    SM_CUDA(cudaFree(r->pyramid_depth_stage));
    SM_CUDA(cudaFree(r->pyramid_color_stage));
    r->pyramid_depth_stage = nullptr;
    r->pyramid_color_stage = nullptr;
    r->pyramid_stage_width = r->pyramid_stage_height = 0;
    SM_CUDA(cudaMallocPitch(reinterpret_cast<void**>(&r->pyramid_depth_stage), &r->pyramid_depth_stage_pitch,
                            source_width * sizeof(u16), source_height));
    SM_CUDA(cudaMallocPitch(reinterpret_cast<void**>(&r->pyramid_color_stage), &r->pyramid_color_stage_pitch,
                            static_cast<size_t>(source_width) * 3, source_height));
    r->pyramid_stage_width = source_width;
    r->pyramid_stage_height = source_height;
  }
  if (r->median_iterations > 0 && !r->median_stage[0]) {
    for (int i = 0; i < 2; ++i) {
      SM_CUDA(cudaMallocPitch(reinterpret_cast<void**>(&r->median_stage[i]), &r->median_stage_pitch, W * sizeof(u16), H));
    }
  }
  return SM_OK;
}

struct RunContext {
  sm_reconstruction* r;
  const sm_stream_desc* s;
  const sm_preprocess_params* pp;
  const sm_integrate_params* ip;
  int W, H, K, half, first, last;
  size_t frame_elems;
  int pyramid;
  int source_W, source_H;
  size_t source_elems;
  bool on_host;
  bool depth_ring;
  bool color_ring;
  int base_slot;
  uint64_t h2d = 0;

  int CountSlot(int frame) const { return (base_slot + (frame - first)) % kCountSlots; }
  const u16* Raw(int frame, size_t* pitch) const {
    if (depth_ring) { *pitch = r->ring_depth_pitch; return r->ring_depth[frame % kDepthRing]; }
    *pitch = W * sizeof(u16);
    return s->depth + frame_elems * frame;
  }
  const uint8_t* Color(int frame, size_t* pitch) const {
    if (color_ring) { *pitch = r->ring_color_pitch; return reinterpret_cast<const uint8_t*>(r->ring_color[frame % kColorRing]); }
    *pitch = static_cast<size_t>(W) * 3;
    return s->color + 3 * frame_elems * frame;
  }
  DeviceState SetState(int set) const {
    DeviceState d = r->d;
    d.assoc = r->assoc_set[set]; d.first_depth = r->first_depth_set[set]; d.supported = r->supported_set[set];
    d.vis = r->vis_set[set]; d.seg_count = r->seg_count_set[set]; d.merge_flag = r->merge_flag_set[set];
    return d;
  }
  FrameParams Params(int frame, int set) const {
    size_t color_pitch;
    const uint8_t* color = Color(frame, &color_pitch);
    return MakeFrameParams(r, static_cast<u32>(frame), CountSlot(frame), *ip, r->run_depth[set], r->run_depth_pitch,
                           r->run_depth_pre[set], r->run_depth_pitch,
                           reinterpret_cast<const float*>(r->run_normals[set]), r->run_normals_pitch,
                           r->run_radius[set], r->run_radius_pitch, color, color_pitch, s->global_T_frame + 12 * frame,
                           s->frame_T_global + 12 * frame);
  }
  int EnqueueRawFrame(int frame) {
    u16* const slot = r->ring_depth[frame % kDepthRing];
    const u16* const src = s->depth + source_elems * frame;
    if (pyramid > 0) {
      const u16* full = src;
      size_t full_pitch = source_W * sizeof(u16);
      if (on_host) {
        SM_CUDA(cudaMemcpy2DAsync(r->pyramid_depth_stage, r->pyramid_depth_stage_pitch, src, full_pitch, full_pitch,
                                  source_H, cudaMemcpyHostToDevice, r->upload_stream));
        h2d += source_elems * sizeof(u16);
        full = r->pyramid_depth_stage;
        full_pitch = r->pyramid_depth_stage_pitch;
      }
      return StageDownscaleMedian(r->upload_stream, 0, source_W, source_H, full, full_pitch, W, H, slot,
                                  r->ring_depth_pitch);
    }
    const int n = r->median_iterations;
    u16* const target = n > 0 ? r->median_stage[0] : slot;
    const size_t target_pitch = n > 0 ? r->median_stage_pitch : r->ring_depth_pitch;
    SM_CUDA(cudaMemcpy2DAsync(target, target_pitch, src, W * sizeof(u16), W * sizeof(u16), H, cudaMemcpyDefault, r->upload_stream));
    if (on_host) h2d += frame_elems * sizeof(u16);
    if (n > 0) {
      return StageMedianDensify(r->upload_stream, n, W, H, r->median_stage[0], r->median_stage_pitch, slot,
                                r->ring_depth_pitch, r->median_stage[1], r->median_stage_pitch);
    }
    return SM_OK;
  }
  int EnqueueColorFrame(int frame) {
    if (pyramid > 0) {
      const uint8_t* full = s->color + 3 * source_elems * frame;
      size_t full_pitch = static_cast<size_t>(source_W) * 3;
      if (on_host) {
        SM_CUDA(cudaMemcpy2DAsync(r->pyramid_color_stage, r->pyramid_color_stage_pitch, full, full_pitch, full_pitch,
                                  source_H, cudaMemcpyHostToDevice, r->upload_stream));
        h2d += source_elems * 3;
        full = r->pyramid_color_stage;
        full_pitch = r->pyramid_color_stage_pitch;
      }
      return StageColorPyramid(r->upload_stream, pyramid, source_W, source_H, full, full_pitch,
                               reinterpret_cast<u8*>(r->ring_color[frame % kColorRing]), r->ring_color_pitch);
    }
    SM_CUDA(cudaMemcpy2DAsync(r->ring_color[frame % kColorRing], r->ring_color_pitch, s->color + 3 * frame_elems * frame,
                              static_cast<size_t>(W) * 3, static_cast<size_t>(W) * 3, H, cudaMemcpyHostToDevice,
                              r->upload_stream));
    h2d += frame_elems * 3;
    return SM_OK;
  }
  void Others(int frame, const u16** others, size_t* pitches) const {
    for (int i = 0; i < half; ++i) {
      others[i] = Raw(frame - (i + 1), &pitches[i]);
      others[half + i] = Raw(frame + (i + 1), &pitches[half + i]);
    }
  }
};

int RunStreams(RunContext& c, cudaStream_t stream, bool pipelined, uint32_t* integrated) {
  sm_reconstruction* r = c.r;
  const int W = c.W, H = c.H, half = c.half;
  r->pipe.have_frame = false;
  SM_CUDA(cudaEventRecord(r->entry_event, stream));
  for (cudaStream_t st : {r->pre_stream, r->pipe.crit, r->pipe.front, r->pipe.side}) {
    SM_CUDA(cudaStreamWaitEvent(st, r->entry_event, 0));
  }
  if (c.depth_ring) SM_CUDA(cudaStreamWaitEvent(r->upload_stream, r->entry_event, 0));
  int uploaded_until = c.first - half - 1;

  auto enqueue_preprocess = [&](int frame) -> int {
    const int set = frame & 1;
    const bool reuse = frame >= c.first + 2;
    if (c.depth_ring) {
      if (reuse) {
        SM_CUDA(cudaStreamWaitEvent(r->upload_stream, r->pre_done[set], 0));
        SM_CUDA(cudaStreamWaitEvent(r->upload_stream, pipelined ? r->pipe.ev_create[set] : r->int_done[set], 0));
      }
      for (int f = uploaded_until + 1; f <= frame + half; ++f) {
        const int st = c.EnqueueRawFrame(f);
        if (st != SM_OK) return st;
      }
      uploaded_until = frame + half;
      if (c.color_ring) {
        const int st = c.EnqueueColorFrame(frame);
        if (st != SM_OK) return st;
      }
      SM_CUDA(cudaEventRecord(r->upload_done, r->upload_stream));
      SM_CUDA(cudaStreamWaitEvent(r->pre_stream, r->upload_done, 0));
    }
    if (reuse) {
      if (pipelined) {
        SM_CUDA(cudaStreamWaitEvent(r->pre_stream, r->pipe.ev_create[set], 0));
        SM_CUDA(cudaStreamWaitEvent(r->pre_stream, r->pipe.ev_update[set], 0));
      } else {
        SM_CUDA(cudaStreamWaitEvent(r->pre_stream, r->int_done[set], 0));
      }
    }
    const u16* others[8];
    size_t other_pitches[8];
    c.Others(frame, others, other_pitches);
    size_t raw_pitch;
    const u16* raw = c.Raw(frame, &raw_pitch);
    const int st = PreprocessFused(r->pre_stream, *c.pp, W, H, r->fx, r->fy, r->cx, r->cy, raw, raw_pitch, others,
                                   other_pitches, c.s->others_TR_reference + static_cast<size_t>(frame) * c.K * 12,
                                   r->scratch_B, r->scratch_B_pitch, r->run_depth[set], r->run_depth_pitch,
                                   r->run_normals[set], r->run_normals_pitch, r->run_radius[set], r->run_radius_pitch,
                                   r->assoc_set[set], r->first_depth_set[set], r->supported_set[set],
                                   pipelined ? r->run_depth_pre[set] : nullptr, r->run_depth_pitch,
                                   TimelineSlot(r->d, static_cast<u32>(frame), KID_BILATERAL_OUTLIER),
                                   TimelineSlot(r->d, static_cast<u32>(frame), KID_ERODE_NORMALS_RADII), r->ScratchBMap());
    if (st != SM_OK) return st;
    SM_CUDA(cudaEventRecord(r->pre_done[set], r->pre_stream));
    return SM_OK;
  };

  int status = SM_OK;
  if (c.first < c.last) {
    status = enqueue_preprocess(c.first);
    if (status != SM_OK) return status;
  }
  for (int frame = c.first; frame < c.last; ++frame) {
    const int set = frame & 1;
    if (frame + 1 < c.last) {
      status = enqueue_preprocess(frame + 1);
      if (status != SM_OK) return status;
    }
    SM_CUDA(cudaStreamWaitEvent(pipelined ? r->pipe.front : stream, r->pre_done[set], 0));
    r->d.assoc = r->assoc_set[set]; r->d.first_depth = r->first_depth_set[set]; r->d.supported = r->supported_set[set];
    r->d.vis = r->vis_set[set]; r->d.seg_count = r->seg_count_set[set]; r->d.merge_flag = r->merge_flag_set[set];
    if (pipelined) {
      RecordOperation(r, static_cast<int>(static_cast<u32>(frame) - static_cast<u32>(c.ip->regularization_frame_window_size)));
      const FrameParams f = c.Params(frame, set);
      r->last_tiebreak = f.tb;
      RegularizeArgs reg;
      reg.iterations = c.ip->regularization_iterations_per_integration_iteration;
      reg.disable_denoising = reg.iterations == 0;
      reg.radius_factor = c.ip->radius_factor_for_regularization_neighbors;
      reg.regularizer_weight = c.ip->regularizer_weight;
      reg.window = c.ip->regularization_frame_window_size;
      status = IntegrateFramePipelined(r->pipe.front, &r->pipe, set, r->d, f, c.ip->do_blending != 0, reg, r->plan);
      if (status != SM_OK) return status;
      r->count_slot = (r->count_slot + 1) % kCountSlots;
    } else {
      r->rasters_cleared = true;
      size_t color_pitch;
      const uint8_t* color = c.Color(frame, &color_pitch);
      status = IntegrateImpl(r, stream, static_cast<u32>(frame), *c.ip, r->run_depth[set], r->run_depth_pitch,
                             reinterpret_cast<const float*>(r->run_normals[set]), r->run_normals_pitch,
                             r->run_radius[set], r->run_radius_pitch, color, color_pitch,
                             c.s->global_T_frame + 12 * frame, c.s->frame_T_global + 12 * frame);
      if (status != SM_OK) return status;
      SM_CUDA(cudaEventRecord(r->int_done[set], stream));
    }
    ++*integrated;
  }
  if (pipelined && r->pipe.have_frame) SM_CUDA(cudaStreamWaitEvent(stream, r->pipe.ev_reg, 0));
  return SM_OK;
}

}

struct FrameGraph {
  cudaGraph_t graph = nullptr;
  cudaGraphExec_t exec = nullptr;
  std::vector<cudaGraphNode_t> nodes;
  std::vector<const void*> funcs;
  int blending = -1, reg_launches = -1, pdl = -1, prio = -1, order = -1;
  size_t blend_smem = 0;
  dim3 scan_grid;
};

void DestroyFrameGraph(FrameGraph* g) {
  if (!g) return;
  if (g->exec) cudaGraphExecDestroy(g->exec);
  if (g->graph) cudaGraphDestroy(g->graph);
  delete g;
}

namespace {

struct StepLayout {
  int integrate, scan, update, create, reg0, reg_count, project, project_tail , associate,
      merge, blend , bilateral, tail, count;
};

StepLayout MakeLayout(bool blending, int reg_launches, bool split_project) {
  StepLayout l;
  int n = 0;
  l.integrate = n++; l.scan = n++; l.update = n++; l.create = n++;
  l.reg0 = n; l.reg_count = reg_launches; n += reg_launches;
  l.project = n++;
  l.project_tail = split_project ? n++ : -1;
  l.associate = n++; l.merge = n++;
  l.blend = blending ? n++ : -1;
  l.bilateral = n++; l.tail = n++;
  l.count = n;
  return l;
}

cudaKernelNodeParams NodeParams(const KernelLaunch& k) {
  cudaKernelNodeParams p = {};
  p.func = const_cast<void*>(k.func);
  p.gridDim = k.grid;
  p.blockDim = k.block;
  p.sharedMemBytes = static_cast<unsigned>(k.smem);
  p.kernelParams = const_cast<void**>(k.args);
  p.extra = nullptr;
  return p;
}

constexpr int kDefaultGraphOrder = 0;

// ... 44 lines not shown
  if (l.project_tail >= 0) {
    edge(l.integrate, l.project, false);
    edge(l.create, l.project_tail, false);
    edge(l.project, l.associate, false);
    edge(l.project_tail, l.associate, false);
  } else {
    edge(l.create, l.project, false);
    edge(l.project, l.associate, true);
  }
  edge(l.associate, l.merge, false);
  if (l.blend >= 0) edge(l.associate, l.blend, true);
  edge(l.bilateral, l.tail, true);
  const int order = EnvInt("SM_B200_GRAPH_ORDER", kDefaultGraphOrder);
  if (order & 1) edge(l.create, l.update, false);
  if ((order & 2) && l.reg_count > 0) edge(l.associate, l.reg0, false);
  if ((order & 4) && l.reg_count > 0) edge(l.merge, l.reg0, false);
  if (order & 8) edge(l.project_tail >= 0 ? l.project_tail : l.project, l.update, false);
  SM_CUDA(cudaGraphAddDependencies_v2(g->graph, from.data(), to.data(), data.data(), from.size()));
  SM_CUDA(cudaGraphInstantiate(&g->exec, g->graph, 0));
  return SM_OK;
}

int RunGraph(RunContext& c, cudaStream_t stream, uint32_t* integrated) {
  sm_reconstruction* r = c.r;
  const int W = c.W, H = c.H, half = c.half;
  const bool blending = c.ip->do_blending != 0;
  const int iterations = c.ip->regularization_iterations_per_integration_iteration;
  const bool disable_denoising = iterations == 0;
  const int reg_launches = disable_denoising ? 1 : 2 * iterations;
  const bool split_project = EnvInt("SM_B200_SPLIT_PROJECT", 0) != 0;
  const StepLayout l = MakeLayout(blending, reg_launches, split_project);
  const int pdl = EnvInt("SM_B200_GRAPH_PDL", 0);
  std::vector<KernelLaunch> launches(l.count);

  cudaStream_t gs = r->graph_stream;
  SM_CUDA(cudaEventRecord(r->entry_event, stream));
  SM_CUDA(cudaStreamWaitEvent(gs, r->entry_event, 0));
  if (c.depth_ring) SM_CUDA(cudaStreamWaitEvent(r->upload_stream, r->entry_event, 0));
  int uploaded_until = c.first - half - 1;
  const int it0 = c.first - 2;

  float* smooth = r->d.smooth;
  float* smooth_next = r->d.smooth_next;

  auto active = [&](int frame) { return frame >= c.first && frame < c.last; };
  auto clamp_frame = [&](int frame) { return frame < c.first ? c.first : (frame >= c.last ? c.last - 1 : frame); };

  for (int it = it0; it < c.last; ++it) {
    const int crit = it, front = it + 1, pre = it + 2;
    if (c.depth_ring && active(pre)) {
      for (int f = uploaded_until + 1; f <= pre + half; ++f) {
        const int last_reader_step = f - kDepthRing + half - 2;
        if (last_reader_step >= it0) SM_CUDA(cudaStreamWaitEvent(r->upload_stream, r->iteration_done[(last_reader_step - it0) % kIterationEvents], 0));
        const int st = c.EnqueueRawFrame(f);
        if (st != SM_OK) return st;
      }
      uploaded_until = pre + half;
      if (c.color_ring) {
        const int last_color_step = pre - kColorRing;
        if (last_color_step >= it0) SM_CUDA(cudaStreamWaitEvent(r->upload_stream, r->iteration_done[(last_color_step - it0) % kIterationEvents], 0));
        const int st = c.EnqueueColorFrame(pre);
        if (st != SM_OK) return st;
      }
      SM_CUDA(cudaEventRecord(r->upload_done, r->upload_stream));
      SM_CUDA(cudaStreamWaitEvent(gs, r->upload_done, 0));
    }

    int status = SM_OK;
    {
      const int frame = clamp_frame(crit), set = frame % kSets;
      DeviceState d = c.SetState(set);
      d.smooth = smooth; d.smooth_next = smooth_next;
      if (active(crit)) RecordOperation(r, static_cast<int>(static_cast<u32>(frame) - static_cast<u32>(c.ip->regularization_frame_window_size)));
      FrameParams f = c.Params(frame, set);
      f.skip = active(crit) ? 0 : 1;
      if (active(crit)) r->last_tiebreak = f.tb;
      const FrameKernel kernels[4] = {FK_INTEGRATE, FK_SCAN, FK_UPDATE_NEIGHBORS, FK_CREATE};
      const int slots[4] = {l.integrate, l.scan, l.update, l.create};
      for (int i = 0; i < 4; ++i) {
        status = DescribeFrameKernel(kernels[i], r->plan, d, f, &launches[slots[i]]);
        if (status != SM_OK) return status;
      }
      const int old_slot = f.count_slot, new_slot = (f.count_slot + 1) % kCountSlots;
      for (int i = 0; i < (disable_denoising ? 1 : iterations); ++i) {
        KernelLaunch* first = &launches[l.reg0 + (disable_denoising ? 0 : 2 * i)];
        KernelLaunch* second = disable_denoising ? nullptr : first + 1;
        DescribeRegularize(first, second, !active(crit), r->plan, d, disable_denoising, static_cast<u32>(frame),
                           c.ip->radius_factor_for_regularization_neighbors, c.ip->regularizer_weight,
                           c.ip->regularization_frame_window_size, new_slot, i == 0 ? old_slot : -1);
        if (!disable_denoising && active(crit)) {
          float* const filled = smooth_next;
          smooth_next = smooth;
          smooth = filled;
          d.smooth = smooth; d.smooth_next = smooth_next;
        }
      }
      if (active(crit)) ++*integrated;
    }
    {
      const int frame = clamp_frame(front), set = frame % kSets;
      const DeviceState d = c.SetState(set);
      FrameParams f = c.Params(frame, set);
      f.skip = active(front) ? 0 : 1;
      const FrameKernel kernels[5] = {split_project ? FK_PROJECT_MAIN : FK_PROJECT, FK_PROJECT_TAIL, FK_ASSOCIATE, FK_MERGE, FK_BLEND};
      const int slots[5] = {l.project, l.project_tail, l.associate, l.merge, l.blend};
      for (int i = 0; i < 5; ++i) {
        if (slots[i] < 0) continue;
        status = DescribeFrameKernel(kernels[i], r->plan, d, f, &launches[slots[i]]);
        if (status != SM_OK) return status;
      }
    }
    {
      const int frame = clamp_frame(pre), set = frame % kSets;
      const u16* others[8];
      size_t other_pitches[8];
      c.Others(frame, others, other_pitches);
      size_t raw_pitch;
      const u16* raw = c.Raw(frame, &raw_pitch);
      status = DescribePreprocess(&launches[l.bilateral], &launches[l.tail], !active(pre), *c.pp, W, H, r->fx, r->fy,
                                  r->cx, r->cy, raw, raw_pitch, others, other_pitches,
                                  c.s->others_TR_reference + static_cast<size_t>(frame) * c.K * 12, r->scratch_B,
                                  r->scratch_B_pitch, r->run_depth[set], r->run_depth_pitch, r->run_normals[set],
                                  r->run_normals_pitch, r->run_radius[set], r->run_radius_pitch, r->assoc_set[set],
                                  r->first_depth_set[set], r->supported_set[set], r->run_depth_pre[set],
                                  r->run_depth_pitch, TimelineSlot(r->d, static_cast<u32>(frame), KID_BILATERAL_OUTLIER),
                                  TimelineSlot(r->d, static_cast<u32>(frame), KID_ERODE_NORMALS_RADII), r->ScratchBMap());
      if (status != SM_OK) return status;
    }

    FrameGraph* g = r->graph;
    const int prio = EnvInt("SM_B200_GRAPH_PRIO", 0);
    const int order = EnvInt("SM_B200_GRAPH_ORDER", kDefaultGraphOrder);
    bool rebuild = g == nullptr || g->blending != (blending ? 1 : 0) || g->reg_launches != reg_launches || g->pdl != pdl ||
                   g->prio != prio || g->order != order || static_cast<int>(g->nodes.size()) != l.count;
    if (!rebuild) {
      for (int i = 0; i < l.count && !rebuild; ++i) rebuild = g->funcs[i] != launches[i].func;
      if (l.blend >= 0) rebuild = rebuild || g->blend_smem != launches[l.blend].smem;
    }
    if (rebuild) {
      if (g) { SM_CUDA(cudaStreamSynchronize(gs)); DestroyFrameGraph(g); r->graph = nullptr; }
      g = new FrameGraph();
      r->graph = g;
      g->blending = blending ? 1 : 0; g->reg_launches = reg_launches; g->pdl = pdl; g->prio = prio; g->order = order;
      g->blend_smem = l.blend >= 0 ? launches[l.blend].smem : 0;
      status = BuildFrameGraph(g, l, launches, pdl);
      if (status != SM_OK) return status;
    } else {
      for (int i = 0; i < l.count; ++i) {
        const cudaKernelNodeParams p = NodeParams(launches[i]);
        SM_CUDA(cudaGraphExecKernelNodeSetParams(g->exec, g->nodes[i], &p));
      }
    }
    SM_CUDA(cudaGraphLaunch(g->exec, gs));
    CountLaunches(static_cast<unsigned long long>(l.count));
    if (c.depth_ring) SM_CUDA(cudaEventRecord(r->iteration_done[(it - it0) % kIterationEvents], gs));
  }
  r->d.smooth = smooth;
  r->d.smooth_next = smooth_next;
  {
    const DeviceState last_set = c.SetState((c.last - 1) % kSets);
    r->d.assoc = last_set.assoc; r->d.first_depth = last_set.first_depth; r->d.supported = last_set.supported;
    r->d.vis = last_set.vis; r->d.seg_count = last_set.seg_count; r->d.merge_flag = last_set.merge_flag;
  }
  r->count_slot = c.CountSlot(c.last);
  SM_CUDA(cudaEventRecord(r->graph_exit, gs));
  SM_CUDA(cudaStreamWaitEvent(stream, r->graph_exit, 0));
  return SM_OK;
}

}

int StreamRun(sm_reconstruction* r, cudaStream_t stream, const sm_stream_desc* s, const sm_preprocess_params* pp,
              const sm_integrate_params* ip, int first_frame, int last_frame, sm_stream_stats* stats) {
  RunContext c;
  c.r = r; c.s = s; c.pp = pp; c.ip = ip;
  c.W = r->d.width; c.H = r->d.height;
  c.pyramid = r->pyramid_level;
  if (c.pyramid > 0) {
    if (r->median_iterations > 0) {
      return SetError(SM_ERR_INVALID_ARGUMENT, "pyramid_level > 0 cannot be combined with median_filter_and_densify_iterations > 0");
    }
    const int step = 1 << c.pyramid;
    if (s->width <= 0 || s->height <= 0 || s->width % step != 0 || s->height % step != 0 ||
        (s->width >> c.pyramid) != c.W || (s->height >> c.pyramid) != c.H) {
      return SetError(SM_ERR_INVALID_ARGUMENT, "stream size must be the handle's size times 2^pyramid_level");
    }
  } else if (s->width != c.W || s->height != c.H) {
    return SetError(SM_ERR_INVALID_ARGUMENT, "stream size mismatch");
  }
  c.source_W = s->width; c.source_H = s->height;
  c.source_elems = static_cast<size_t>(c.source_W) * c.source_H;
  c.K = pp->outlier_filtering_frame_count;
  c.half = c.K / 2;
  if (c.K < 2 || c.K > 8 || first_frame < c.half || last_frame > s->frame_count - c.half || first_frame > last_frame) {
    return SetError(SM_ERR_INVALID_ARGUMENT,
                    "frame range needs outlier_filtering_frame_count/2 frames on both sides (main.cc:987-992)");
  }
  c.first = first_frame; c.last = last_frame;
  c.frame_elems = static_cast<size_t>(c.W) * c.H;
  c.on_host = s->frames_on_host != 0;
  c.depth_ring = c.on_host || r->median_iterations > 0 || c.pyramid > 0;
  c.color_ring = c.on_host || c.pyramid > 0;
  c.base_slot = r->count_slot;
  int status = EnsureRunBuffers(r, c.on_host, c.depth_ring, c.color_ring, c.source_W, c.source_H);
  if (status != SM_OK) return status;
  const unsigned long long launches_before = LaunchCount();
  const auto host_t0 = std::chrono::steady_clock::now();
  r->last_stream = stream;

  const bool serial = r->events.enabled || ProfilingEnabled();
  const int radius = static_cast<int>(pp->bilateral_filter_radius_factor * pp->bilateral_filter_sigma_xy + 0.5f);
  const bool use_graph = !serial && EnvInt("SM_B200_GRAPH", 1) != 0 && radius == 6 && first_frame < last_frame;
  uint32_t integrated = 0;
  if (use_graph) {
    status = RunGraph(c, stream, &integrated);
    if (status != SM_OK) cudaStreamSynchronize(r->graph_stream);
  } else {
    status = RunStreams(c, stream, !serial, &integrated);
    if (status != SM_OK) cudaDeviceSynchronize();
  }
  if (status != SM_OK) return status;
  const double host_enqueue_ms = std::chrono::duration<double, std::milli>(std::chrono::steady_clock::now() - host_t0).count();
  status = FetchCounters(r, stream);
  if (stats) {
    stats->frames_integrated = integrated;
    stats->surfels_size = r->host_counters->surfel_count[r->count_slot];
    stats->surfel_count = stats->surfels_size - r->host_counters->merge_count;
    stats->kernel_launches = LaunchCount() - launches_before;
    stats->h2d_bytes = c.h2d;
    stats->d2h_bytes = sizeof(Counters);
    stats->host_enqueue_ms = host_enqueue_ms;
  }
  return status;
}

}
```

### surfelmeshing_b200/csrc/regularize.cu

```cuda

#include <algorithm>
#include <cstdlib>

#include "sm_kernels.cuh"

namespace smb {

namespace {

#define SM_S(row, i) d.surfels[static_cast<size_t>(row) * d.stride + (i)]
#define SM_SU(row, i) reinterpret_cast<u32*>(d.surfels)[static_cast<size_t>(row) * d.stride + (i)]
#define SM_SMOOTH(axis, i) d.smooth[static_cast<size_t>(axis) * d.stride + (i)]
#define SM_SMOOTH_NEXT(axis, i) d.smooth_next[static_cast<size_t>(axis) * d.stride + (i)]

constexpr int kBlock = 256;
#ifndef SM_REG_ACCUMULATE_MIN_BLOCKS
#define SM_REG_ACCUMULATE_MIN_BLOCKS 1
#endif
#ifndef SM_REG_STEP_MIN_BLOCKS
#define SM_REG_STEP_MIN_BLOCKS 1
#endif

struct RegParams {
  u32 frame_index;
  int window;
  float radius_factor_squared;
  float regularizer_weight;
  int count_slot;
  int remove_below_slot;
  int skip;
};

__device__ __forceinline__ bool outside_window(u32 stamp, const RegParams& p) {
  return static_cast<int>(stamp) < static_cast<int>(p.frame_index - static_cast<u32>(p.window));
}

__global__ void __launch_bounds__(kBlock, SM_REG_ACCUMULATE_MIN_BLOCKS) k_reg_accumulate(DeviceState d, RegParams p) {
  pdl_prologue();
  if (p.skip) return;
  const TimelineScope timeline_scope(d, p.frame_index, KID_REG_ACCUMULATE);
  const u32 n = d.counters->surfel_count[p.count_slot];
  const u32 n_remove = p.remove_below_slot >= 0 ? d.counters->surfel_count[p.remove_below_slot] : 0u;
  const u32 step = gridDim.x * blockDim.x;
  u32 i = blockIdx.x * blockDim.x + threadIdx.x;
  u32 nbr_ahead[4] = {kInvalidIndex, kInvalidIndex, kInvalidIndex, kInvalidIndex};
  if (i < d.stride) {
#pragma unroll
    for (int k = 0; k < 4; ++k) nbr_ahead[k] = SM_SU(SM_ROW_NEIGHBOR0 + k, i);
  }
  for (; i < n; i += step) {
    u32 nbr[4];
#pragma unroll
    for (int k = 0; k < 4; ++k) nbr[k] = nbr_ahead[k];
    if (i + step < n) {
#pragma unroll
      for (int k = 0; k < 4; ++k) nbr_ahead[k] = SM_SU(SM_ROW_NEIGHBOR0 + k, i + step);
    }
    if ((nbr[0] & nbr[1] & nbr[2] & nbr[3]) == kInvalidIndex) continue;

    u32 meta[4];
#pragma unroll
    for (int k = 0; k < 4; ++k) {
      const u32 q = nbr[k] != kInvalidIndex ? nbr[k] : i;
      meta[k] = SM_SU(kRowMeta, q);
    }
    const float sx = SM_SMOOTH(0, i), sy = SM_SMOOTH(1, i), sz = SM_SMOOTH(2, i);
    const float nx = SM_S(SM_ROW_NORMAL_X, i), ny = SM_S(SM_ROW_NORMAL_Y, i), nz = SM_S(SM_ROW_NORMAL_Z, i);
    const float radius_squared = SM_S(SM_ROW_RADIUS_SQUARED, i);

    bool use[4];
    int neighbor_count = 0;
#pragma unroll
    for (int k = 0; k < 4; ++k) {
      if (i < n_remove && nbr[k] != kInvalidIndex && (meta[k] & kMetaDetachBit)) {
        nbr[k] = kInvalidIndex;
        SM_SU(SM_ROW_NEIGHBOR0 + k, i) = kInvalidIndex;
      }
      use[k] = nbr[k] != kInvalidIndex && !outside_window(meta[k] & ~kMetaDetachBit, p);
      neighbor_count += use[k] ? 1 : 0;
    }
    if (neighbor_count == 0) continue;

    float qx[4], qy[4], qz[4];
#pragma unroll
    for (int k = 0; k < 4; ++k) {
      const u32 q = use[k] ? nbr[k] : i;
      qx[k] = SM_SMOOTH(0, q);
      qy[k] = SM_SMOOTH(1, q);
      qz[k] = SM_SMOOTH(2, q);
    }
    const float max_distance_squared = fmul(radius_squared, p.radius_factor_squared);
    const float rcp_count = frcp(i2f(neighbor_count));
    const float factor = fmul(fadd(p.regularizer_weight, p.regularizer_weight), rcp_count);
    const float weight_term = fmul(rcp_count, p.regularizer_weight);
#pragma unroll
    for (int k = 0; k < 4; ++k) {
      if (!use[k]) continue;
      const u32 q = nbr[k];
      const float dx = fsub(qx[k], sx);
      const float dy = fsub(qy[k], sy);
      const float dz = fsub(qz[k], sz);
      const float f = fmul(factor, ffma(nz, dz, ffma(nx, dx, fmul(ny, dy))));
      atomicAdd(&d.gradient[q], make_float4(fmul(nx, f), fmul(ny, f), fmul(nz, f), weight_term));
      if (squared_norm(dx, dy, dz) > max_distance_squared) SM_SU(SM_ROW_NEIGHBOR0 + k, i) = kInvalidIndex;
    }
  }
}

__global__ void __launch_bounds__(kBlock, SM_REG_STEP_MIN_BLOCKS) k_reg_step(DeviceState d, RegParams p) {
  pdl_prologue();
  if (p.skip) return;
  const TimelineScope timeline_scope(d, p.frame_index, KID_REG_STEP);
  const u32 n = d.counters->surfel_count[p.count_slot];
  const u32 step = gridDim.x * blockDim.x;
  u32 i = blockIdx.x * blockDim.x + threadIdx.x;
  u32 stamp_ahead = 0, nbr_ahead[4] = {kInvalidIndex, kInvalidIndex, kInvalidIndex, kInvalidIndex};
  if (i < d.stride) {
    stamp_ahead = SM_SU(SM_ROW_LAST_UPDATE_STAMP, i);
#pragma unroll
    for (int k = 0; k < 4; ++k) nbr_ahead[k] = SM_SU(SM_ROW_NEIGHBOR0 + k, i);
  }
  for (; i < n; i += step) {
    const u32 stamp = stamp_ahead;
    u32 nbr[4];
#pragma unroll
    for (int k = 0; k < 4; ++k) nbr[k] = nbr_ahead[k];
    if (i + step < n) {
      stamp_ahead = SM_SU(SM_ROW_LAST_UPDATE_STAMP, i + step);
#pragma unroll
      for (int k = 0; k < 4; ++k) nbr_ahead[k] = SM_SU(SM_ROW_NEIGHBOR0 + k, i + step);
    }
    const float sx = SM_SMOOTH(0, i), sy = SM_SMOOTH(1, i), sz = SM_SMOOTH(2, i);
    if (outside_window(stamp, p)) {
      SM_SMOOTH_NEXT(0, i) = sx; SM_SMOOTH_NEXT(1, i) = sy; SM_SMOOTH_NEXT(2, i) = sz;
      continue;
    }
    const float nx = SM_S(SM_ROW_NORMAL_X, i), ny = SM_S(SM_ROW_NORMAL_Y, i), nz = SM_S(SM_ROW_NORMAL_Z, i);
    const float4 accumulated = d.gradient[i];
    float gx = ffma(fsub(sx, SM_S(SM_ROW_X, i)), 2.0f, accumulated.x);
    float gy = ffma(fsub(sy, SM_S(SM_ROW_Y, i)), 2.0f, accumulated.y);
    float gz = ffma(fsub(sz, SM_S(SM_ROW_Z, i)), 2.0f, accumulated.z);
    int neighbor_count = 0;
    float rx = 0.f, ry = 0.f, rz = 0.f;
    float qx[4], qy[4], qz[4];
#pragma unroll
    for (int k = 0; k < 4; ++k) {
      const u32 q = nbr[k] != kInvalidIndex ? nbr[k] : i;
      qx[k] = SM_SMOOTH(0, q);
      qy[k] = SM_SMOOTH(1, q);
      qz[k] = SM_SMOOTH(2, q);
    }
#pragma unroll
    for (int k = 0; k < 4; ++k) {
      if (nbr[k] == kInvalidIndex) continue;
      ++neighbor_count;
      const float dx = fsub(qx[k], sx);
      const float dy = fsub(qy[k], sy);
      const float dz = fsub(qz[k], sz);
      const float normal_dot_difference = ffma(nz, dz, ffma(nx, dx, fmul(ny, dy)));
      rx = ffma(-nx, normal_dot_difference, rx);
      ry = ffma(-ny, normal_dot_difference, ry);
      rz = ffma(-nz, normal_dot_difference, rz);
    }
    if (neighbor_count > 0) {
      const float factor = fmul(fadd(p.regularizer_weight, p.regularizer_weight), frcp(i2f(neighbor_count)));
      gx = ffma(factor, rx, gx);
      gy = ffma(factor, ry, gy);
      gz = ffma(factor, rz, gz);
    }
    const float gradient_length = fsqrt_approx(ffma(gz, gz, ffma(gx, gx, fmul(gy, gy))));
    const float residual_terms_weight_sum = fadd(fadd(p.regularizer_weight, 1.0f), accumulated.w);
    float step_factor = fmul(frcp(residual_terms_weight_sum), 0.5f);
    const float max_step_length = fsqrt_approx(SM_S(SM_ROW_RADIUS_SQUARED, i));
    const float step_length = fmul(step_factor, gradient_length);
    if (step_length > max_step_length) step_factor = fmul(step_factor, fmul(max_step_length, frcp(step_length)));
    SM_SMOOTH_NEXT(0, i) = ffma(step_factor, -gx, sx);
    SM_SMOOTH_NEXT(1, i) = ffma(step_factor, -gy, sy);
    SM_SMOOTH_NEXT(2, i) = ffma(step_factor, -gz, sz);
    d.gradient[i] = make_float4(0.f, 0.f, 0.f, 0.f);
  }
}

__global__ void __launch_bounds__(kBlock) k_reg_copy_only(DeviceState d, RegParams p) {
  pdl_prologue();
  if (p.skip) return;
  const TimelineScope timeline_scope(d, p.frame_index, KID_REG_COPY_ONLY);
  const u32 n = d.counters->surfel_count[p.count_slot];
  const u32 n_remove = p.remove_below_slot >= 0 ? d.counters->surfel_count[p.remove_below_slot] : 0u;
  for (u32 i = blockIdx.x * blockDim.x + threadIdx.x; i < n; i += gridDim.x * blockDim.x) {
    if (i < n_remove) {
#pragma unroll
      for (int k = 0; k < 4; ++k) {
        const u32 q = SM_SU(SM_ROW_NEIGHBOR0 + k, i);
        if (q != kInvalidIndex && (SM_SU(SM_ROW_COLOR, q) >> 24) == 1u) SM_SU(SM_ROW_NEIGHBOR0 + k, i) = kInvalidIndex;
      }
    }
    if (outside_window(SM_SU(SM_ROW_LAST_UPDATE_STAMP, i), p)) continue;
    SM_SMOOTH(0, i) = SM_S(SM_ROW_X, i);
    SM_SMOOTH(1, i) = SM_S(SM_ROW_Y, i);
    SM_SMOOTH(2, i) = SM_S(SM_ROW_Z, i);
  }
}

}

namespace {
__global__ void __launch_bounds__(kBlock) k_rebuild_meta(DeviceState d, u32 count) {
  for (u32 i = blockIdx.x * blockDim.x + threadIdx.x; i < count; i += gridDim.x * blockDim.x) {
    const u32 flag = (SM_SU(SM_ROW_COLOR, i) >> 24) == 1u ? kMetaDetachBit : 0u;
    SM_SU(kRowMeta, i) = (SM_SU(SM_ROW_LAST_UPDATE_STAMP, i) & ~kMetaDetachBit) | flag;
  }
}
}

int RebuildMetaRow(cudaStream_t stream, const DeviceState& d, u32 count, int sm_count) {
  if (count == 0) return SM_OK;
  k_rebuild_meta<<<sm_count * 4, kBlock, 0, stream>>>(d, count);
  return CheckLaunch("rebuild meta row");
}

int DescribeRegularize(KernelLaunch* first, KernelLaunch* second, bool skip, const LaunchPlan& plan,
                       const DeviceState& d, bool disable_denoising, u32 frame_index,
                       float radius_factor_for_regularization_neighbors, float regularizer_weight,
                       int regularization_frame_window_size, int count_slot, int remove_replaced_below_slot) {
  RegParams p;
  p.frame_index = frame_index;
  p.window = regularization_frame_window_size;
  p.radius_factor_squared =
      radius_factor_for_regularization_neighbors * radius_factor_for_regularization_neighbors;
  p.regularizer_weight = regularizer_weight;
  p.count_slot = count_slot;
  p.remove_below_slot = remove_replaced_below_slot;
  p.skip = skip ? 1 : 0;
  static_assert(sizeof(DeviceState) + sizeof(RegParams) + 32 <= sizeof(first->storage), "KernelLaunch::storage too small");
  if (disable_denoising) {
    first->Reset(reinterpret_cast<const void*>(k_reg_copy_only), dim3(plan.reg_copy), dim3(kBlock), 0, KID_REG_COPY_ONLY);
    first->Arg(d);
    first->Arg(p);
    return 1;
  }
  first->Reset(reinterpret_cast<const void*>(k_reg_accumulate), dim3(plan.reg_accumulate), dim3(kBlock), 0, KID_REG_ACCUMULATE);
  first->Arg(d);
  first->Arg(p);
  second->Reset(reinterpret_cast<const void*>(k_reg_step), dim3(plan.reg_step), dim3(kBlock), 0, KID_REG_STEP);
  second->Arg(d);
  second->Arg(p);
  return 2;
}

int RegularizeSurfels(cudaStream_t stream, DeviceState& d, bool disable_denoising, u32 frame_index,
                      float radius_factor_for_regularization_neighbors, float regularizer_weight,
                      int regularization_frame_window_size, int count_slot, int remove_replaced_below_slot,
                      const LaunchPlan& plan) {
  KernelLaunch first, second;
  const int n = DescribeRegularize(&first, &second, false, plan, d, disable_denoising, frame_index,
                                   radius_factor_for_regularization_neighbors, regularizer_weight,
                                   regularization_frame_window_size, count_slot, remove_replaced_below_slot);
  LaunchOnStream(stream, first, false);
  if (n == 1) return CheckLaunch("regularize (copy only)");
  LaunchOnStream(stream, second, true);
  float* const filled = d.smooth_next;
  d.smooth_next = d.smooth;
  d.smooth = filled;
  return CheckLaunch("regularize");
}

int ConfigureRegularizeKernels(int carveout_percent, LaunchPlan* plan) {
  if (carveout_percent >= 0) {
    cudaFuncSetAttribute(k_reg_accumulate, cudaFuncAttributePreferredSharedMemoryCarveout, carveout_percent);
    cudaFuncSetAttribute(k_reg_step, cudaFuncAttributePreferredSharedMemoryCarveout, carveout_percent);
    cudaFuncSetAttribute(k_reg_copy_only, cudaFuncAttributePreferredSharedMemoryCarveout, carveout_percent);
    cudaGetLastError();
  }
  const char* e = std::getenv("SM_B200_RESIDENT_GRIDS");
  auto resident = [&](auto kernel) {
    int per_sm = 0;
    if ((e && e[0] == '0') || cudaOccupancyMaxActiveBlocksPerMultiprocessor(&per_sm, kernel, kBlock, 0) != cudaSuccess || per_sm < 1) {
      cudaGetLastError();
      per_sm = 8;
    }
    return ScaleGrid(plan->sm_count * per_sm);
  };
  plan->reg_accumulate = resident(k_reg_accumulate);
  plan->reg_step = resident(k_reg_step);
  plan->reg_copy = resident(k_reg_copy_only);
  if (const char* pe = std::getenv("SM_B200_OFFCHAIN_GRID_PERCENT")) {
    const int percent = std::atoi(pe);
    if (percent > 0 && percent < 100) {
      plan->reg_accumulate = std::max(plan->sm_count, plan->reg_accumulate * percent / 100);
      plan->reg_step = std::max(plan->sm_count, plan->reg_step * percent / 100);
    }
  }
  return SM_OK;
}

}
```

### surfelmeshing_b200/csrc/sm_handle.cuh

```cuda
#pragma once

#include <vector>

#include "sm_kernels.cuh"

namespace smb {

constexpr int kSets = 3;

struct TieBreakConfig {
  u32 wave;
  double early_fraction;
  double index_order_fraction;
  double early_fraction_later, index_order_fraction_later;
  double early_fraction_second;
  u32 wave_offset;
  u32 lane_request;
  u32 lane_shift;
  u32 mul, mul_inv;
};
constexpr u32 kDefaultTieBreakWave = 264 * 1024;
constexpr u32 kDefaultTieBreakLaneShift = 5;
constexpr u32 kDefaultTieBreakWaveOffset = 0;
constexpr double kDefaultTieBreakEarlyFraction = 0.015;
constexpr double kDefaultTieBreakIndexOrderFraction = 0.25;
constexpr double kDefaultTieBreakEarlyFractionLater = 0.04;
constexpr double kDefaultTieBreakIndexOrderFractionLater = 0.45;
constexpr double kDefaultTieBreakEarlyFractionSecond = 0.02;
TieBreak MakeTieBreak(const TieBreakConfig& cfg, u32 frame_index);
int SetTieBreakWave(TieBreakConfig* cfg, u32 wave, u32 capacity);

struct FrameGraph;
void DestroyFrameGraph(FrameGraph* g);

}

struct sm_reconstruction {
  smb::DeviceState d{};
  int device = 0;
  int sm_count = 0;
  smb::LaunchPlan plan{};
  float fx = 0, fy = 0, cx = 0, cy = 0;
  int count_slot = 0;
  bool rasters_cleared = false;
  smb::IntegrateEvents events{};
  smb::TieBreakConfig tiebreak{};
  smb::TieBreak last_tiebreak{};
  smb::Counters* host_counters = nullptr;
  cudaStream_t last_stream = nullptr;
  smb::u16* scratch_B = nullptr; size_t scratch_B_pitch = 0;
  smb::TensorMapStorage scratch_B_map{};
  bool scratch_B_map_valid = false;
  const smb::TensorMapStorage* ScratchBMap() const { return scratch_B_map_valid ? &scratch_B_map : nullptr; }
  smb::u16* blend_src = nullptr; size_t blend_src_pitch = 0;
  smb::PixelAssoc* assoc_set[smb::kSets] = {};
  float* first_depth_set[smb::kSets] = {};
  smb::u8* supported_set[smb::kSets] = {};
  smb::VisEntry* vis_set[smb::kSets] = {};
  smb::u32* seg_count_set[smb::kSets] = {};
  smb::u8* merge_flag_set[smb::kSets] = {};
  smb::u16* run_depth[smb::kSets] = {}; size_t run_depth_pitch = 0;
  float2* run_normals[smb::kSets] = {}; size_t run_normals_pitch = 0;
  float* run_radius[smb::kSets] = {}; size_t run_radius_pitch = 0;
  smb::u16* run_depth_pre[smb::kSets] = {};
  float* smooth_alt = nullptr;
  smb::PipelineCtx pipe{};
  cudaStream_t pre_stream = nullptr;
  cudaEvent_t pre_done[2] = {nullptr, nullptr}, int_done[2] = {nullptr, nullptr}, entry_event = nullptr;
  std::vector<smb::u16*> ring_depth; size_t ring_depth_pitch = 0;
  std::vector<uchar3*> ring_color; size_t ring_color_pitch = 0;
  cudaStream_t upload_stream = nullptr;
  cudaEvent_t upload_done = nullptr;
  int median_iterations = 0;
  smb::u16* median_stage[2] = {nullptr, nullptr}; size_t median_stage_pitch = 0;
  int pyramid_level = 0;
  smb::u16* pyramid_depth_stage = nullptr; size_t pyramid_depth_stage_pitch = 0;
  smb::u8* pyramid_color_stage = nullptr; size_t pyramid_color_stage_pitch = 0;
  int pyramid_stage_width = 0, pyramid_stage_height = 0;
  std::vector<cudaEvent_t> iteration_done;
  smb::u32 op_epoch = 0;
  uint64_t state_generation = 1;
  struct Operation { smb::u32 epoch; int stamp_threshold; };
  std::vector<Operation> op_history;
  smb::u32* delta_index = nullptr; float* delta_values = nullptr; smb::u32* delta_cursor = nullptr;
  smb::u32 delta_capacity = 0;
  smb::u32* delta_host = nullptr; size_t delta_host_capacity = 0;
  cudaStream_t graph_stream = nullptr;
  cudaEvent_t graph_exit = nullptr;
  smb::FrameGraph* graph = nullptr;
};

namespace smb {
int FetchCounters(sm_reconstruction* r, cudaStream_t stream);
FrameParams MakeFrameParams(const sm_reconstruction* r, u32 frame_index, int count_slot, const sm_integrate_params& p,
                            u16* depth, size_t depth_pitch, const u16* depth_pre, size_t depth_pre_pitch,
                            const float* normals, size_t normals_pitch, const float* radius, size_t radius_pitch,
                            const uint8_t* color, size_t color_pitch, const float* global_T_local,
                            const float* local_T_global);
int IntegrateImpl(sm_reconstruction* r, cudaStream_t stream, u32 frame_index, const sm_integrate_params& p, u16* depth,
                  size_t depth_pitch, const float* normals, size_t normals_pitch, const float* radius,
                  size_t radius_pitch, const uint8_t* color, size_t color_pitch, const float* global_T_local,
                  const float* local_T_global);
void CountLaunches(unsigned long long n);
unsigned long long LaunchCount();
void RecordOperation(sm_reconstruction* r, int stamp_threshold);
void FreeTransferBuffers(sm_reconstruction* r);
int TransferDelta(sm_reconstruction* r, cudaStream_t stream, uint32_t frame_index, sm_transfer_token* token, float* x,
                  float* y, float* z, float* radius_squared, float* nx, float* ny, float* nz,
                  uint32_t* last_update_stamp, sm_transfer_stats* stats);
int UpdateVisualizationBuffers(sm_reconstruction* r, cudaStream_t stream, const sm_visualization_params& p, float* vertex,
                               uint32_t* neighbor_index, float* normal_vertex);
int StreamRun(sm_reconstruction* r, cudaStream_t stream, const sm_stream_desc* s, const sm_preprocess_params* pp,
              const sm_integrate_params* ip, int first_frame, int last_frame, sm_stream_stats* stats);
}
```

### surfelmeshing_b200/csrc/sm_kernels.cuh

```cuda
#pragma once

#include <cuda_runtime.h>
#include <math.h>
#include <stddef.h>
#include <stdint.h>
#include <string.h>

#include "../../include/surfel_b200.h"
#include "sm_math.cuh"

namespace smb {

int SetError(int code, const char* message);
int CheckLaunch(const char* what);

enum KernelId {
  KID_CLEAR = 0, KID_BILATERAL_OUTLIER, KID_BILATERAL_GENERIC, KID_OUTLIER, KID_ERODE_NORMALS_RADII, KID_ERODE,
  KID_NORMALS, KID_RADII, KID_PROJECT, KID_ASSOCIATE, KID_MERGE, KID_BLEND, KID_INTEGRATE, KID_UPDATE_NEIGHBORS,
  KID_NEW_SURFEL_SCAN, KID_CREATE_SURFELS, KID_REG_ACCUMULATE, KID_REG_STEP, KID_REG_COPY_ONLY,
  KID_EXPORT_VERTICES, KID_MEDIAN_DENSIFY, KID_DELTA_SELECT, KID_VIZ_BUFFERS, KID_PROJECT_TAIL, KID_DOWNSCALE_DEPTH,
  KID_DOWNSCALE_COLOR, KID_COUNT
};
const char* KernelName(int id);
bool ProfilingEnabled();
// ... 40 lines not shown
  u64 group_reciprocal;
};
__host__ __device__ __forceinline__ u64 tb_divide(u64 x, u32 d, u64 reciprocal, u32* remainder) {
#if defined(__CUDA_ARCH__)
  u64 q = __umul64hi(x, reciprocal);
#else
  u64 q = static_cast<u64>((static_cast<unsigned __int128>(x) * reciprocal) >> 64);
#endif
  u64 r = x - q * d;
  while (r >= d) { r -= d; ++q; }
  *remainder = static_cast<u32>(r);
  return q;
}
__host__ __device__ __forceinline__ u32 tb_hash(u32 x) {
  x ^= x >> 16; x *= 0x7feb352du; x ^= x >> 15; x *= 0x846ca68bu; x ^= x >> 16;
  return x;
}
__host__ __device__ __forceinline__ bool tb_index_order(const TieBreak& t, u32 pixel, u32 wave_index) {
  return tb_hash(pixel ^ ~t.salt) < (wave_index == 0 ? t.index_order_threshold : t.index_order_threshold_later);
}
__host__ __device__ __forceinline__ u32 tb_phase(const TieBreak& t, u32 pixel) {
  if (!t.wave_offset) return 0u;
  u32 g;
  tb_divide(tb_hash(pixel ^ t.salt ^ 0x5bd1e995u), t.groups, t.group_reciprocal, &g);
  return g << t.lane_shift;
}
__host__ __device__ __forceinline__ u32 tb_encode(const TieBreak& t, u32 idx, bool secondary, u32 pixel) {
  if (t.wave == 0) return idx | (secondary ? kSecondaryBit : 0u);
  u32 r, rp;
  const u32 w = static_cast<u32>(tb_divide(static_cast<u64>(idx) + tb_phase(t, pixel), t.wave, t.wave_reciprocal, &r));
  if (tb_index_order(t, pixel, w)) {
    rp = r;
  } else {
    u32 gp;
    tb_divide(static_cast<u64>(r >> t.lane_shift) * t.mul + t.add, t.groups, t.group_reciprocal, &gp);
    rp = (gp << t.lane_shift) | (r & ((1u << t.lane_shift) - 1u));
  }
  const bool late = secondary && !(tb_hash(idx ^ t.salt) <
                                   (w == 0 ? t.early_threshold : (w == 1 ? t.early_threshold_second : t.early_threshold_later)));
  return w * (2u * t.wave) + (late ? t.wave : 0u) + rp;
}
__host__ __device__ __forceinline__ u32 supporting_index(const TieBreak& t, u32 key, u32 pixel) {
  if (key == kInvalidIndex) return kInvalidIndex;
  if (t.wave == 0) return key & ~kSecondaryBit;
  u32 rem;
  const u32 w2 = static_cast<u32>(tb_divide(key, t.wave, t.wave_reciprocal, &rem));
  const u32 w = w2 >> 1;
  u32 r = rem;
  if (!tb_index_order(t, pixel, w)) {
    const u32 gp = rem >> t.lane_shift;
    const u32 shifted = gp >= t.add ? gp - t.add : gp + t.groups - t.add;
    u32 g;
    tb_divide(static_cast<u64>(shifted) * t.mul_inv, t.groups, t.group_reciprocal, &g);
    r = (g << t.lane_shift) | (rem & ((1u << t.lane_shift) - 1u));
  }
  return w * t.wave + r - tb_phase(t, pixel);
}

typedef uint4 PixelAssoc;

typedef uint4 VisEntry;

constexpr int kCountSlots = 3;
struct Counters {
  u32 surfel_count[kCountSlots];
  u32 merge_count;
  u32 new_surfel_count;
  u32 capacity_overflow;
  u32 scan_ticket;
  u32 pad;
};

struct DeviceState {
  float* surfels;
  size_t stride;
  u32 capacity;
  int width, height;
  PixelAssoc* assoc;
  float* first_depth;
  u8* supported;
  VisEntry* vis;
  u32* seg_count;
  u8* merge_flag;
  u8* new_flag;
  u32* new_index;
  u32* new_list;
  unsigned long long* scan_state;
  Counters* counters;
  float4* gradient;
  float* smooth;
  float* smooth_next;
  unsigned long long* timeline;
  u32 timeline_frames;
};

struct FrameParams {
  u32 frame_index;
  int count_slot;
  int skip;
  u32 op_epoch;
  TieBreak tb;
  int active_window;
  float fx, fy, cx, cy;
  float fx_inv, fy_inv, cx_inv, cy_inv;
  float sensor_noise_factor;
  float cos_normal_compatibility_threshold;
  float max_surfel_confidence;
  float depth_scaling;
  float inv_depth_scaling;
  float radius_factor_squared;
  int blend_radius;
  Mat3x4 local_T_global;
  Mat3x4 global_T_local;
  u16* depth; size_t depth_pitch;
  const u16* depth_pre; size_t depth_pre_pitch;
  const float2* normals; size_t normals_pitch;
  const float* radius; size_t radius_pitch;
  const uchar3* color; size_t color_pitch;
};

__device__ __forceinline__ void pdl_prologue() {
#if defined(__CUDA_ARCH__)
  asm volatile("griddepcontrol.launch_dependents;");
  asm volatile("griddepcontrol.wait;" ::: "memory");
#endif
}
__device__ __forceinline__ unsigned long long globaltimer_ns() {
  unsigned long long t;
  asm volatile("mov.u64 %0, %globaltimer;" : "=l"(t));
  return t;
}
struct TimelineScope {
  unsigned long long* slot;
  __device__ __forceinline__ explicit TimelineScope(unsigned long long* s) : slot(s) { begin(); }
  __device__ __forceinline__ TimelineScope(const DeviceState& d, u32 frame, int kernel_id)
      : slot(d.timeline ? d.timeline + (static_cast<size_t>(frame % d.timeline_frames) * KID_COUNT + kernel_id) * 2 : nullptr) {
    begin();
  }
  __device__ __forceinline__ void begin() {
    if (slot && threadIdx.x == 0 && blockIdx.x < 8 && blockIdx.y == 0) atomicMin(slot, globaltimer_ns());
  }
  __device__ __forceinline__ ~TimelineScope() {
    if (slot && threadIdx.x == 0) atomicMax(slot + 1, globaltimer_ns());
  }
};
inline unsigned long long* TimelineSlot(const DeviceState& d, u32 frame, int kernel_id) {
  return d.timeline ? d.timeline + (static_cast<size_t>(frame % d.timeline_frames) * KID_COUNT + kernel_id) * 2 : nullptr;
}

int PdlMode();
int ScaleGrid(int blocks);

template <typename... KArgs, typename... Args>
inline void LaunchKernelImpl(bool dependent, void (*kernel)(KArgs...), dim3 grid, dim3 block, size_t smem,
                             cudaStream_t stream, Args&&... args) {
  cudaLaunchConfig_t cfg = {};
  cfg.gridDim = grid;
  cfg.blockDim = block;
  cfg.dynamicSmemBytes = smem;
  cfg.stream = stream;
  cudaLaunchAttribute attr[1];
  attr[0].id = cudaLaunchAttributeProgrammaticStreamSerialization;
  attr[0].val.programmaticStreamSerializationAllowed = 1;
  cfg.attrs = attr;
  const int mode = PdlMode();
  cfg.numAttrs = (mode == 2 || (mode == 1 && dependent)) ? 1 : 0;
  cudaLaunchKernelEx(&cfg, kernel, static_cast<KArgs>(args)...);
}
template <typename... KArgs, typename... Args>
inline void LaunchKernel(void (*kernel)(KArgs...), dim3 grid, dim3 block, size_t smem, cudaStream_t stream,
                         Args&&... args) {
  LaunchKernelImpl(false, kernel, grid, block, smem, stream, static_cast<Args&&>(args)...);
}
template <typename... KArgs, typename... Args>
// ... 26 lines not shown
void LaunchOnStream(cudaStream_t stream, const KernelLaunch& k, bool dependent);

struct LaunchPlan {
  int sm_count;
  int project, associate, merge, integrate, update_neighbors;
  int reg_accumulate, reg_step, reg_copy;
};
int ConfigurePreprocessKernels(int carveout_percent);
int ConfigureIntegrateKernels(int carveout_percent, LaunchPlan* plan);
int ConfigureRegularizeKernels(int carveout_percent, LaunchPlan* plan);

struct alignas(64) TensorMapStorage { unsigned char bytes[128]; };
int MakeDepthTensorMap(TensorMapStorage* out, const u16* base, size_t pitch_bytes, int width, int height);
int PreprocessFused(cudaStream_t stream, const sm_preprocess_params& p, int width, int height, float fx, float fy,
                    float cx, float cy, const u16* raw, size_t raw_pitch, const u16* const* other_depths,
                    const size_t* other_pitches, const float* others_TR_reference, u16* scratch_B,
                    size_t scratch_B_pitch, u16* out_depth, size_t out_depth_pitch, float2* out_normals,
                    size_t out_normals_pitch, float* out_radius, size_t out_radius_pitch, uint4* clear_assoc,
                    float* clear_first_depth, u8* clear_supported, u16* out_depth_copy = nullptr,
                    size_t out_depth_copy_pitch = 0, unsigned long long* timeline_bilateral = nullptr,
                    unsigned long long* timeline_tail = nullptr, const TensorMapStorage* scratch_B_map = nullptr);
int DescribePreprocess(KernelLaunch* bilateral, KernelLaunch* tail, bool skip, const sm_preprocess_params& p, int width,
                       int height, float fx, float fy, float cx, float cy, const u16* raw, size_t raw_pitch,
                       const u16* const* other_depths, const size_t* other_pitches, const float* others_TR_reference,
                       u16* scratch_B, size_t scratch_B_pitch, u16* out_depth, size_t out_depth_pitch,
                       float2* out_normals, size_t out_normals_pitch, float* out_radius, size_t out_radius_pitch,
                       uint4* clear_assoc, float* clear_first_depth, u8* clear_supported, u16* out_depth_copy,
                       size_t out_depth_copy_pitch, unsigned long long* timeline_bilateral,
                       unsigned long long* timeline_tail, const TensorMapStorage* scratch_B_map);
int StageBilateral(cudaStream_t stream, float sigma_xy, float sigma_value_factor, u16 value_to_ignore,
                   float radius_factor, u16 max_depth, float depth_valid_region_radius, int width, int height,
                   const u16* in, size_t in_pitch, u16* out, size_t out_pitch);
int StageOutlier(cudaStream_t stream, int other_count, int required_count, float tolerance, float fx, float fy,
                 float cx, float cy, int width, int height, const u16* in, size_t in_pitch,
                 const u16* const* other_depths, const size_t* other_pitches, const float* others_TR_reference,
                 u16* out, size_t out_pitch);
int StageErode(cudaStream_t stream, int radius, int width, int height, const u16* in, size_t in_pitch, u16* out,
               size_t out_pitch);
int StageMedianDensify(cudaStream_t stream, int iterations, int width, int height, const u16* in, size_t in_pitch,
                       u16* out, size_t out_pitch, u16* scratch, size_t scratch_pitch);
int StageDownscaleMedian(cudaStream_t stream, u16 value_to_ignore, int in_width, int in_height, const u16* in,
                         size_t in_pitch, int out_width, int out_height, u16* out, size_t out_pitch);
int StageColorPyramid(cudaStream_t stream, int levels, int width, int height, const u8* in, size_t in_pitch, u8* out,
                      size_t out_pitch);
int StageNormals(cudaStream_t stream, float observation_angle_threshold_deg, float depth_scaling, float fx, float fy,
                 float cx, float cy, int width, int height, const u16* in, size_t in_pitch, u16* out, size_t out_pitch,
                 float2* normals, size_t normals_pitch);
int StageRadii(cudaStream_t stream, float point_radius_extension_factor, float point_radius_clamp_factor,
               float depth_scaling, float fx, float fy, float cx, float cy, int width, int height, const u16* in,
               size_t in_pitch, float* radius, size_t radius_pitch, u16* out, size_t out_pitch);

struct IntegrateEvents {
  cudaEvent_t ev[14];
  bool enabled;
};
int IntegrateFrame(cudaStream_t stream, const DeviceState& d, const FrameParams& f, bool do_blending,
                   bool rasters_already_cleared, const LaunchPlan& plan, const IntegrateEvents* events);
enum FrameKernel { FK_PROJECT = 0, FK_ASSOCIATE, FK_MERGE, FK_BLEND, FK_INTEGRATE, FK_UPDATE_NEIGHBORS, FK_SCAN, FK_CREATE,
                   FK_PROJECT_MAIN, FK_PROJECT_TAIL, FK_COUNT };
int DescribeFrameKernel(FrameKernel which, const LaunchPlan& plan, const DeviceState& d, const FrameParams& f,
                        KernelLaunch* out);
int ClearAssociationRasters(cudaStream_t stream, const DeviceState& d);

struct PipelineCtx {
  cudaStream_t front;
  cudaStream_t crit;
  cudaStream_t side;
  cudaEvent_t ev_assoc, ev_merge, ev_blend, ev_integrate;
  cudaEvent_t ev_create[2], ev_update[2];
  cudaEvent_t ev_reg;
  bool have_frame;
};
struct RegularizeArgs {
  bool disable_denoising;
  int iterations;
  float radius_factor, regularizer_weight;
  int window;
};
int IntegrateFramePipelined(cudaStream_t stream, PipelineCtx* pc, int set, DeviceState& d, const FrameParams& f,
                            bool do_blending, const RegularizeArgs& reg, const LaunchPlan& plan);
int ExportVertices(cudaStream_t stream, const DeviceState& d, int count_slot, int sm_count, float* position_buffer,
                   u8* color_buffer);

int RebuildMetaRow(cudaStream_t stream, const DeviceState& d, u32 count, int sm_count);
int RegularizeSurfels(cudaStream_t stream, DeviceState& d, bool disable_denoising, u32 frame_index,
                      float radius_factor_for_regularization_neighbors, float regularizer_weight,
                      int regularization_frame_window_size, int count_slot, int remove_replaced_below_slot,
                      const LaunchPlan& plan);
int DescribeRegularize(KernelLaunch* first, KernelLaunch* second, bool skip, const LaunchPlan& plan,
                       const DeviceState& d, bool disable_denoising, u32 frame_index,
                       float radius_factor_for_regularization_neighbors, float regularizer_weight,
                       int regularization_frame_window_size, int count_slot, int remove_replaced_below_slot);

}
```

Before: 8626.

## Build update-neighbor worklist in integrate and skip redundant smooth-copy for stale surfels

The integrate kernel now applies the update-neighbors gating (activity, reprojection, border and depth tests) per surfel and appends survivors with their pixel to a compact list via warp-aggregated atomics. The update-neighbors kernel can then process only that list instead of rescanning all visible surfels. Separately, the regularizer tracks the oldest stamp touched since the last step and only copies smooth to smooth_next for out-of-window surfels that could have changed. To keep both smooth buffers consistent, integrate and creation paths write both. This adds host-side state and extra writes in integrate.

```diff
diff --git a/surfelmeshing_b200/csrc/api.cu b/surfelmeshing_b200/csrc/api.cu
--- a/surfelmeshing_b200/csrc/api.cu
+++ b/surfelmeshing_b200/csrc/api.cu
@@ -249,6 +249,7 @@
   int status = IntegrateFrame(stream, r->d, f, p.do_blending != 0, r->rasters_cleared, r->plan, &r->events);
   r->rasters_cleared = false;
   if (status != SM_OK) return status;
+  NoteIntegratedFrame(r->d, frame_index);
   const int old_slot = r->count_slot;
   r->count_slot = (r->count_slot + 1) % kCountSlots;
   if (r->events.enabled) cudaEventRecord(r->events.ev[12], stream);
@@ -308,9 +309,14 @@
     SM_CUDA(cudaMalloc(&r->vis_set[i], sizeof(VisEntry) * padded));
     SM_CUDA(cudaMalloc(&r->seg_count_set[i], sizeof(u32) * (padded / kSegment)));
     SM_CUDA(cudaMalloc(&r->merge_flag_set[i], padded));
+    SM_CUDA(cudaMalloc(&r->upd_list_set[i], sizeof(uint2) * padded));
+    SM_CUDA(cudaMalloc(&r->upd_count_set[i], sizeof(u32)));
   }
   d.assoc = r->assoc_set[0]; d.first_depth = r->first_depth_set[0]; d.supported = r->supported_set[0];
   d.vis = r->vis_set[0]; d.seg_count = r->seg_count_set[0]; d.merge_flag = r->merge_flag_set[0];
+  d.upd_list = r->upd_list_set[0]; d.upd_count = r->upd_count_set[0];
+  d.reg_t_prev = 0;
+  d.reg_full_sweep = 1;
   SM_CUDA(cudaMalloc(&d.new_list, sizeof(u32) * P));
   SM_CUDA(cudaMalloc(&d.new_flag, P));
   SM_CUDA(cudaMalloc(&d.new_index, sizeof(u32) * P));
@@ -459,6 +465,7 @@
   cudaFree(d.surfels); cudaFree(d.gradient); cudaFree(r->smooth_alt); cudaFree(d.new_list);
   for (int i = 0; i < kSets; ++i) {
     cudaFree(r->vis_set[i]); cudaFree(r->seg_count_set[i]); cudaFree(r->merge_flag_set[i]);
+    cudaFree(r->upd_list_set[i]); cudaFree(r->upd_count_set[i]);
     cudaFree(r->assoc_set[i]); cudaFree(r->first_depth_set[i]); cudaFree(r->supported_set[i]);
     cudaFree(r->run_depth[i]); cudaFree(r->run_depth_pre[i]); cudaFree(r->run_normals[i]); cudaFree(r->run_radius[i]);
   }
@@ -687,6 +694,7 @@
   if (surfels_size > r->d.capacity) return SetError(SM_ERR_CAPACITY, "sm_load_state: state larger than the surfel cap");
   r->d.smooth = r->d.surfels + static_cast<size_t>(SM_ROW_SMOOTH_X) * r->d.stride;
   r->d.smooth_next = r->smooth_alt;
+  r->d.reg_full_sweep = 1;
   if (surfels_size > 0) {
     SM_CUDA(cudaMemcpy2DAsync(r->d.surfels, r->d.stride * sizeof(float), host_rows,
                               host_row_stride_elems * sizeof(float), surfels_size * sizeof(float), SM_ROW_COUNT,
diff --git a/surfelmeshing_b200/csrc/integrate.cu b/surfelmeshing_b200/csrc/integrate.cu
--- a/surfelmeshing_b200/csrc/integrate.cu
+++ b/surfelmeshing_b200/csrc/integrate.cu
@@ -3,7 +3,11 @@
 #include <cstdio>
 #include <cstdlib>
 
+#include <cooperative_groups.h>
+
 #include "sm_kernels.cuh"
+
+namespace cg = cooperative_groups;
 
 namespace smb {
 
@@ -12,6 +16,7 @@
 #define SM_S(row, i) d.surfels[static_cast<size_t>(row) * d.stride + (i)]
 #define SM_SU(row, i) reinterpret_cast<u32*>(d.surfels)[static_cast<size_t>(row) * d.stride + (i)]
 #define SM_SMOOTH(axis, i) d.smooth[static_cast<size_t>(axis) * d.stride + (i)]
+#define SM_SMOOTH_NEXT(axis, i) d.smooth_next[static_cast<size_t>(axis) * d.stride + (i)]
 
 constexpr int kBlock = 256;
 
@@ -120,7 +125,7 @@
   if (blockIdx.x == 0 && part != kProjectMain) {
     const int tiles = (d.width * d.height + kSegment - 1) / kSegment;
     for (int t = threadIdx.x; t < tiles; t += blockDim.x) d.scan_state[t] = 0ull;
-    if (threadIdx.x == 0) d.counters->scan_ticket = 0;
+    if (threadIdx.x == 0) { d.counters->scan_ticket = 0; *d.upd_count = 0; }
   }
 
   struct SlotRows { float2 X, Y, Z; uint2 T; };
@@ -791,11 +796,8 @@
   return !(cz_ > fmul(fadd(f.sensor_noise_factor, 1.0f), measurement_depth));
 }
 
-__global__ void __launch_bounds__(kBlock, 4) k_integrate(DeviceState d, FrameParams f) {
-  pdl_prologue();
-  if (f.skip) return;
-  const TimelineScope timeline_scope(d, f.frame_index, KID_INTEGRATE);
-  for_each_visible(d, &d.counters->surfel_count[f.count_slot], [&](size_t pos, const VisEntry& e) {
+__device__ __forceinline__ bool integrate_entry(const DeviceState& d, const FrameParams& f, size_t pos, const VisEntry& e,
+                                                int* ux, int* uy) {
     const u32 idx = e.x & ~kActiveBit;
     const float x = __uint_as_float(e.y), y = __uint_as_float(e.z), z = __uint_as_float(e.w);
     const Projection p = project(f, d.width, d.height, x, y, z);
@@ -833,15 +835,16 @@
       reinterpret_cast<u8*>(&SM_SU(SM_ROW_COLOR, idx))[3] = 1;
       SM_SU(kRowMeta, idx) = kMetaDetachBit;
       SM_SU(kRowMergeEpoch, idx) = f.op_epoch;
-      return;
-    }
-    if (!(e.x & kActiveBit)) return;
-    if (s.radius_squared < 0.f) return;
+      SM_SMOOTH_NEXT(0, idx) = SM_SMOOTH(0, idx); SM_SMOOTH_NEXT(1, idx) = SM_SMOOTH(1, idx);
+      SM_SMOOTH_NEXT(2, idx) = SM_SMOOTH(2, idx);
+      return false;
+    }
+    if (!(e.x & kActiveBit)) return false;
+    if (s.radius_squared < 0.f) return false;
 #if SM_INTEGRATE_LEVELS != 1
     const bool touch0 = pixel_can_touch(f, m0.measurement_depth, m0.first, m0.conflicting, idx, z);
     const bool touch1 = has2 && pixel_can_touch(f, m1.measurement_depth, m1.first, m1.conflicting, idx, z);
-    if (!touch0 && !touch1) return;
-    {
+    if (touch0 || touch1) {
       const int qx0 = touch0 ? p.px : ox, qy0 = touch0 ? p.py : oy;
       const int qx1 = touch1 ? ox : qx0, qy1 = touch1 ? oy : qy0;
       m0.normal = row_ptr(f.normals, f.normals_pitch, qy0)[qx0];
@@ -857,46 +860,72 @@
       s.nx = SM_S(SM_ROW_NORMAL_X, idx); s.ny = SM_S(SM_ROW_NORMAL_Y, idx); s.nz = SM_S(SM_ROW_NORMAL_Z, idx);
       s.color = SM_SU(SM_ROW_COLOR, idx);
       s.creation_stamp = SM_SU(SM_ROW_CREATION_STAMP, idx);
-    }
-    if (touch0) integrate_or_conflict(f, m0, p.px, p.py, idx, x, y, z, s);
-    if (touch1) integrate_or_conflict(f, m1, ox, oy, idx, x, y, z, s);
+      if (touch0) integrate_or_conflict(f, m0, p.px, p.py, idx, x, y, z, s);
+      if (touch1) integrate_or_conflict(f, m1, ox, oy, idx, x, y, z, s);
+    }
 #else
     integrate_or_conflict(f, m0, p.px, p.py, idx, x, y, z, s);
     if (has2) integrate_or_conflict(f, m1, ox, oy, idx, x, y, z, s);
 #endif
-    if (!s.dirty) return;
-    SM_S(SM_ROW_X, idx) = s.x; SM_S(SM_ROW_Y, idx) = s.y; SM_S(SM_ROW_Z, idx) = s.z;
-    SM_S(SM_ROW_CONFIDENCE, idx) = s.confidence;
-    SM_S(SM_ROW_RADIUS_SQUARED, idx) = s.radius_squared;
-    SM_S(SM_ROW_NORMAL_X, idx) = s.nx; SM_S(SM_ROW_NORMAL_Y, idx) = s.ny; SM_S(SM_ROW_NORMAL_Z, idx) = s.nz;
-    SM_SU(SM_ROW_COLOR, idx) = s.color;
-    if (s.stamped) {
-      SM_SU(SM_ROW_LAST_UPDATE_STAMP, idx) = f.frame_index;
-      SM_SU(kRowMeta, idx) = f.frame_index | (((s.color >> 24) & 1u) ? kMetaDetachBit : 0u);
-    }
-    if (s.replaced) {
-      SM_SMOOTH(0, idx) = s.smooth_x; SM_SMOOTH(1, idx) = s.smooth_y; SM_SMOOTH(2, idx) = s.smooth_z;
-      SM_SU(SM_ROW_CREATION_STAMP, idx) = f.frame_index;
-#pragma unroll
-      for (int i = 0; i < 4; ++i) SM_SU(SM_ROW_NEIGHBOR0 + i, idx) = kInvalidIndex;
-    }
+    if (s.dirty) {
+      SM_S(SM_ROW_X, idx) = s.x; SM_S(SM_ROW_Y, idx) = s.y; SM_S(SM_ROW_Z, idx) = s.z;
+      SM_S(SM_ROW_CONFIDENCE, idx) = s.confidence;
+      SM_S(SM_ROW_RADIUS_SQUARED, idx) = s.radius_squared;
+      SM_S(SM_ROW_NORMAL_X, idx) = s.nx; SM_S(SM_ROW_NORMAL_Y, idx) = s.ny; SM_S(SM_ROW_NORMAL_Z, idx) = s.nz;
+      SM_SU(SM_ROW_COLOR, idx) = s.color;
+      if (s.stamped) {
+        SM_SU(SM_ROW_LAST_UPDATE_STAMP, idx) = f.frame_index;
+        SM_SU(kRowMeta, idx) = f.frame_index | (((s.color >> 24) & 1u) ? kMetaDetachBit : 0u);
+      }
+      if (s.replaced) {
+        SM_SMOOTH(0, idx) = s.smooth_x; SM_SMOOTH(1, idx) = s.smooth_y; SM_SMOOTH(2, idx) = s.smooth_z;
+        SM_SMOOTH_NEXT(0, idx) = s.smooth_x; SM_SMOOTH_NEXT(1, idx) = s.smooth_y; SM_SMOOTH_NEXT(2, idx) = s.smooth_z;
+        SM_SU(SM_ROW_CREATION_STAMP, idx) = f.frame_index;
+#pragma unroll
+        for (int i = 0; i < 4; ++i) SM_SU(SM_ROW_NEIGHBOR0 + i, idx) = kInvalidIndex;
+      }
+    }
+
+    if (s.stamped && !is_active(f.frame_index, f.frame_index, f.active_window)) return false;
+    if (s.radius_squared < 0.f) return false;
+    float cz_ = z;
+    int px = p.px, py = p.py;
+    if (s.dirty) {
+      cz_ = transform_row(f.local_T_global.r2, s.x, s.y, s.z);
+      if (!(cz_ > 0.f)) return false;
+      const float cx_ = transform_row(f.local_T_global.r0, s.x, s.y, s.z);
+      const float cy_ = transform_row(f.local_T_global.r1, s.x, s.y, s.z);
+      const float inv_z = frcp(cz_);
+      px = f2i_trunc(ffma(fmul(cx_, inv_z), f.fx, f.cx));
+      py = f2i_trunc(ffma(fmul(cy_, inv_z), f.fy, f.cy));
+    }
+    constexpr int kBorder = 1;
+    if (px < kBorder || py < kBorder || px >= d.width - kBorder || py >= d.height - kBorder) return false;
+    float measurement_depth = m0.measurement_depth;
+    if (px != p.px || py != p.py) {
+      measurement_depth = fmul(u2f(row_ptr(f.depth, f.depth_pitch, py)[px]), f.inv_depth_scaling);
+    }
+    if (cz_ > fmul(measurement_depth, fadd(f.sensor_noise_factor, 1.0f))) return false;
+    *ux = px;
+    *uy = py;
+    return true;
+}
+
+__global__ void __launch_bounds__(kBlock, 4) k_integrate(DeviceState d, FrameParams f) {
+  pdl_prologue();
+  if (f.skip) return;
+  const TimelineScope timeline_scope(d, f.frame_index, KID_INTEGRATE);
+  for_each_visible(d, &d.counters->surfel_count[f.count_slot], [&](size_t pos, const VisEntry& e) {
+    int ux, uy;
+    if (!integrate_entry(d, f, pos, e, &ux, &uy)) return;
+    const cg::coalesced_group g = cg::coalesced_threads();
+    u32 base = 0;
+    if (g.thread_rank() == 0) base = atomicAdd(d.upd_count, g.size());
+    base = g.shfl(base, 0) + g.thread_rank();
+    d.upd_list[base] = make_uint2(e.x & ~kActiveBit, static_cast<u32>(ux) | (static_cast<u32>(uy) << 16));
   });
 }
 
-#ifndef SM_UPDATE_ANYNEW_FIRST
-#define SM_UPDATE_ANYNEW_FIRST 0
-#endif
-#ifndef SM_UPDATE_EARLY_GATE
-#define SM_UPDATE_EARLY_GATE 1
-#endif
-#ifndef SM_UPDATE_COMPACT
-#define SM_UPDATE_COMPACT 0
-#endif
-
-#ifndef SM_UPDATE_COMPACT_MIN_BLOCKS
-#define SM_UPDATE_COMPACT_MIN_BLOCKS 3
-#endif
-#if SM_UPDATE_COMPACT
 __device__ __forceinline__ void update_neighbors_survivor(const DeviceState& d, const FrameParams& f, u32 idx, int x, int y) {
   const int kDirectionsX[4] = {-1, 1, 0, 0};
   const int kDirectionsY[4] = {0, 0, -1, 1};
@@ -918,7 +947,6 @@
   const float cy_ = transform_row(f.local_T_global.r1, gx, gy, gz);
   float3 ln;
   if (facing_dot(f, cx_, cy_, cz_, nx, ny, nz, &ln) > 0.f) return;
-  if (radius_squared < 0.f) return;
   if (fmul(observation_radius_squared, frcp(radius_squared)) > 2.25f) return;
   bool any_new = false;
 #pragma unroll
@@ -983,257 +1011,16 @@
   }
 }
 
-__global__ void __launch_bounds__(kBlock, SM_UPDATE_COMPACT_MIN_BLOCKS) k_update_neighbors(DeviceState d, FrameParams f) {
-  pdl_prologue();
-  if (f.skip) return;
-  const TimelineScope timeline_scope(d, f.frame_index, KID_UPDATE_NEIGHBORS);
-  constexpr int kPerThread = kSegment / kBlock;
-  constexpr int kBorder = 1;
-  __shared__ u32 s_survivor[kSegment];
-  __shared__ u32 s_pixel[kSegment];
-  __shared__ u32 s_count;
-  const u32 n = d.counters->surfel_count[f.count_slot];
-  const u32 segments = (n + kSegment - 1) / kSegment;
-  const int lane = threadIdx.x & 31;
-  for (u32 segment = blockIdx.x; segment < segments; segment += gridDim.x) {
-    if (threadIdx.x == 0) s_count = 0;
-    __syncthreads();
-    const u32 cnt = d.seg_count[segment];
-    u32 surfel[kPerThread], stamp[kPerThread];
-    float gx[kPerThread], gy[kPerThread], gz[kPerThread];
-    u16 raw_depth[kPerThread];
-    int cached_px[kPerThread], cached_py[kPerThread];
-    bool live[kPerThread];
-    {
-      VisEntry e[kPerThread];
-#pragma unroll
-      for (int u = 0; u < kPerThread; ++u) {
-        const u32 k = u * kBlock + threadIdx.x;
-        live[u] = k < cnt;
-        if (live[u]) e[u] = d.vis[static_cast<size_t>(segment) * kSegment + k];
-      }
-#pragma unroll
-      for (int u = 0; u < kPerThread; ++u) {
-        if (!live[u]) continue;
-        surfel[u] = e[u].x & ~kActiveBit;
-        const Projection cached = project(f, d.width, d.height, __uint_as_float(e[u].y), __uint_as_float(e[u].z), __uint_as_float(e[u].w));
-        cached_px[u] = cached.px;
-        cached_py[u] = cached.py;
-      }
-    }
-#pragma unroll
-    for (int u = 0; u < kPerThread; ++u) {
-      if (!live[u]) continue;
-      const u32 idx = surfel[u];
-      stamp[u] = SM_SU(SM_ROW_LAST_UPDATE_STAMP, idx);
-      gx[u] = SM_S(SM_ROW_X, idx); gy[u] = SM_S(SM_ROW_Y, idx); gz[u] = SM_S(SM_ROW_Z, idx);
-      raw_depth[u] = row_ptr(f.depth, f.depth_pitch, cached_py[u])[cached_px[u]];
-    }
-#pragma unroll
-    for (int u = 0; u < kPerThread; ++u) {
-      bool pass = live[u];
-      int x = 0, y = 0;
-      if (pass) pass = is_active(stamp[u], f.frame_index, f.active_window);
-      if (pass) {
-        const float cz_ = transform_row(f.local_T_global.r2, gx[u], gy[u], gz[u]);
-        pass = cz_ > 0.f;
-        if (pass) {
-          const float cx_ = transform_row(f.local_T_global.r0, gx[u], gy[u], gz[u]);
-          const float cy_ = transform_row(f.local_T_global.r1, gx[u], gy[u], gz[u]);
-          const float inv_z = frcp(cz_);
-          x = f2i_trunc(ffma(fmul(cx_, inv_z), f.fx, f.cx));
-          y = f2i_trunc(ffma(fmul(cy_, inv_z), f.fy, f.cy));
-          pass = !(x < kBorder || y < kBorder || x >= d.width - kBorder || y >= d.height - kBorder);
-          if (pass) {
-            u16 depth_here = raw_depth[u];
-            if (x != cached_px[u] || y != cached_py[u]) depth_here = row_ptr(f.depth, f.depth_pitch, y)[x];
-            const float measurement_depth = fmul(u2f(depth_here), f.inv_depth_scaling);
-            pass = !(cz_ > fmul(measurement_depth, fadd(f.sensor_noise_factor, 1.0f)));
-          }
-        }
-      }
-      const unsigned ballot = __ballot_sync(0xFFFFFFFFu, pass);
-      if (ballot) {
-        u32 base = 0;
-        if (lane == 0) base = atomicAdd(&s_count, static_cast<u32>(__popc(ballot)));
-        base = __shfl_sync(0xFFFFFFFFu, base, 0);
-        if (pass) {
-          const u32 slot = base + __popc(ballot & ((1u << lane) - 1u));
-          s_survivor[slot] = surfel[u];
-          s_pixel[slot] = static_cast<u32>(x) | (static_cast<u32>(y) << 16);
-        }
-      }
-    }
-    __syncthreads();
-    const u32 survivors = s_count;
-    for (u32 q = threadIdx.x; q < survivors; q += kBlock) {
-      const u32 pixel = s_pixel[q];
-      update_neighbors_survivor(d, f, s_survivor[q], static_cast<int>(pixel & 0xFFFFu), static_cast<int>(pixel >> 16));
-    }
-    __syncthreads();
-  }
-}
-#else
 __global__ void __launch_bounds__(kBlock) k_update_neighbors(DeviceState d, FrameParams f) {
   pdl_prologue();
   if (f.skip) return;
   const TimelineScope timeline_scope(d, f.frame_index, KID_UPDATE_NEIGHBORS);
-  for_each_visible(d, &d.counters->surfel_count[f.count_slot], [&](size_t, const VisEntry& e) {
-    const u32 idx = e.x & ~kActiveBit;
-    constexpr int kBorder = 1;
-    const int kDirectionsX[4] = {-1, 1, 0, 0};
-    const int kDirectionsY[4] = {0, 0, -1, 1};
-#if SM_UPDATE_EARLY_GATE
-    const Projection cached = project(f, d.width, d.height, __uint_as_float(e.y), __uint_as_float(e.z), __uint_as_float(e.w));
-    const u32 stamp = SM_SU(SM_ROW_LAST_UPDATE_STAMP, idx);
-    const float gx = SM_S(SM_ROW_X, idx), gy = SM_S(SM_ROW_Y, idx), gz = SM_S(SM_ROW_Z, idx);
-    u16 raw_depth = row_ptr(f.depth, f.depth_pitch, cached.py)[cached.px];
-    if (!is_active(stamp, f.frame_index, f.active_window)) return;
-    const float cz_ = transform_row(f.local_T_global.r2, gx, gy, gz);
-    if (!(cz_ > 0.f)) return;
-    const float cx_ = transform_row(f.local_T_global.r0, gx, gy, gz);
-    const float cy_ = transform_row(f.local_T_global.r1, gx, gy, gz);
-    const float inv_z = frcp(cz_);
-    const int x = f2i_trunc(ffma(fmul(cx_, inv_z), f.fx, f.cx));
-    const int y = f2i_trunc(ffma(fmul(cy_, inv_z), f.fy, f.cy));
-    if (x < kBorder || y < kBorder || x >= d.width - kBorder || y >= d.height - kBorder) return;
-    if (x != cached.px || y != cached.py) raw_depth = row_ptr(f.depth, f.depth_pitch, y)[x];
-    const float measurement_depth = fmul(u2f(raw_depth), f.inv_depth_scaling);
-    if (cz_ > fmul(measurement_depth, fadd(f.sensor_noise_factor, 1.0f))) return;
-#if SM_UPDATE_ANYNEW_FIRST
-    u32 neighbor_surfel_indices[4];
-#pragma unroll
-    for (int m = 0; m < 4; ++m) neighbor_surfel_indices[m] = SM_SU(SM_ROW_NEIGHBOR0 + m, idx);
-    u32 candidate[4];
-#pragma unroll
-    for (int direction = 0; direction < 4; ++direction) {
-      const int candidate_pixel = (y + kDirectionsY[direction]) * d.width + x + kDirectionsX[direction];
-      candidate[direction] = supporting_index(f.tb, d.assoc[candidate_pixel].x, static_cast<u32>(candidate_pixel));
-    }
-    {
-      bool any_new_first = false;
-#pragma unroll
-      for (int direction = 0; direction < 4; ++direction) {
-        const u32 q = candidate[direction];
-        if (q == kInvalidIndex || q == idx) continue;
-        any_new_first |= q != neighbor_surfel_indices[0] && q != neighbor_surfel_indices[1] &&
-                         q != neighbor_surfel_indices[2] && q != neighbor_surfel_indices[3];
-      }
-      if (!any_new_first) return;
-    }
-    const float nx = SM_S(SM_ROW_NORMAL_X, idx), ny = SM_S(SM_ROW_NORMAL_Y, idx), nz = SM_S(SM_ROW_NORMAL_Z, idx);
-    const float radius_squared = SM_S(SM_ROW_RADIUS_SQUARED, idx);
-    const float observation_radius_squared = row_ptr(f.radius, f.radius_pitch, y)[x];
-#else
-    const float nx = SM_S(SM_ROW_NORMAL_X, idx), ny = SM_S(SM_ROW_NORMAL_Y, idx), nz = SM_S(SM_ROW_NORMAL_Z, idx);
-    const float radius_squared = SM_S(SM_ROW_RADIUS_SQUARED, idx);
-    u32 neighbor_surfel_indices[4];
-#pragma unroll
-    for (int m = 0; m < 4; ++m) neighbor_surfel_indices[m] = SM_SU(SM_ROW_NEIGHBOR0 + m, idx);
-    const float observation_radius_squared = row_ptr(f.radius, f.radius_pitch, y)[x];
-    u32 candidate[4];
-#pragma unroll
-    for (int direction = 0; direction < 4; ++direction) {
-      const int candidate_pixel = (y + kDirectionsY[direction]) * d.width + x + kDirectionsX[direction];
-      candidate[direction] = supporting_index(f.tb, d.assoc[candidate_pixel].x, static_cast<u32>(candidate_pixel));
-    }
-#endif
-#else
-    const u32 stamp = SM_SU(SM_ROW_LAST_UPDATE_STAMP, idx);
-    const float gx = SM_S(SM_ROW_X, idx), gy = SM_S(SM_ROW_Y, idx), gz = SM_S(SM_ROW_Z, idx);
-    const float nx = SM_S(SM_ROW_NORMAL_X, idx), ny = SM_S(SM_ROW_NORMAL_Y, idx), nz = SM_S(SM_ROW_NORMAL_Z, idx);
-    const float radius_squared = SM_S(SM_ROW_RADIUS_SQUARED, idx);
-    u32 neighbor_surfel_indices[4];
-#pragma unroll
-    for (int m = 0; m < 4; ++m) neighbor_surfel_indices[m] = SM_SU(SM_ROW_NEIGHBOR0 + m, idx);
-    if (!is_active(stamp, f.frame_index, f.active_window)) return;
-    const float cz_ = transform_row(f.local_T_global.r2, gx, gy, gz);
-    if (!(cz_ > 0.f)) return;
-    const float cx_ = transform_row(f.local_T_global.r0, gx, gy, gz);
-    const float cy_ = transform_row(f.local_T_global.r1, gx, gy, gz);
-    const float inv_z = frcp(cz_);
-    const int x = f2i_trunc(ffma(fmul(cx_, inv_z), f.fx, f.cx));
-    const int y = f2i_trunc(ffma(fmul(cy_, inv_z), f.fy, f.cy));
-    if (x < kBorder || y < kBorder || x >= d.width - kBorder || y >= d.height - kBorder) return;
-
-    const float measurement_depth = fmul(u2f(row_ptr(f.depth, f.depth_pitch, y)[x]), f.inv_depth_scaling);
-    const float observation_radius_squared = row_ptr(f.radius, f.radius_pitch, y)[x];
-    u32 candidate[4];
-#pragma unroll
-    for (int direction = 0; direction < 4; ++direction) {
-      const int candidate_pixel = (y + kDirectionsY[direction]) * d.width + x + kDirectionsX[direction];
-      candidate[direction] = supporting_index(f.tb, d.assoc[candidate_pixel].x, static_cast<u32>(candidate_pixel));
-    }
-    if (cz_ > fmul(measurement_depth, fadd(f.sensor_noise_factor, 1.0f))) return;
-#endif
-    float3 ln;
-    if (facing_dot(f, cx_, cy_, cz_, nx, ny, nz, &ln) > 0.f) return;
-    if (radius_squared < 0.f) return;
-    if (fmul(observation_radius_squared, frcp(radius_squared)) > 2.25f) return;
-    bool any_new = false;
-#pragma unroll
-    for (int direction = 0; direction < 4; ++direction) {
-      const u32 q = candidate[direction];
-      if (q == kInvalidIndex || q == idx) { candidate[direction] = kInvalidIndex; continue; }
-      any_new |= q != neighbor_surfel_indices[0] && q != neighbor_surfel_indices[1] &&
-                 q != neighbor_surfel_indices[2] && q != neighbor_surfel_indices[3];
-    }
-    if (!any_new) return;
-
-    float neighbor_distances_squared[4];
-#pragma unroll
-    for (int m = 0; m < 4; ++m) {
-      const u32 q = neighbor_surfel_indices[m];
-      if (q == kInvalidIndex) {
-        neighbor_distances_squared[m] = __int_as_float(0x7f800000);
-      } else {
-        neighbor_distances_squared[m] = squared_norm(fsub(gx, SM_S(SM_ROW_X, q)), fsub(gy, SM_S(SM_ROW_Y, q)),
-                                                     fsub(gz, SM_S(SM_ROW_Z, q)));
-      }
-    }
-    const float max_distance_squared = fmul(radius_squared, f.radius_factor_squared);
-    float cand_distance[4], cand_dot[4];
-#pragma unroll
-    for (int direction = 0; direction < 4; ++direction) {
-      const u32 q = candidate[direction];
-      if (q == kInvalidIndex) continue;
-      cand_distance[direction] = squared_norm(fsub(SM_S(SM_ROW_X, q), gx), fsub(SM_S(SM_ROW_Y, q), gy),
-                                              fsub(SM_S(SM_ROW_Z, q), gz));
-      cand_dot[direction] = dot3(nx, ny, nz, SM_S(SM_ROW_NORMAL_X, q), SM_S(SM_ROW_NORMAL_Y, q), SM_S(SM_ROW_NORMAL_Z, q));
-    }
-    bool changed = false;
-#pragma unroll
-    for (int direction = 0; direction < 4; ++direction) {
-      const u32 q = candidate[direction];
-      if (q == kInvalidIndex) continue;
-      const float distance_squared = cand_distance[direction];
-      if (distance_squared > max_distance_squared) continue;
-      if (cand_dot[direction] <= 0.f) continue;
-      int best_n = -1;
-      float best_distance_squared = -1.f;
-#pragma unroll
-      for (int m = 0; m < 4; ++m) {
-        if (q == neighbor_surfel_indices[m]) { best_n = -1; break; }
-        if (neighbor_distances_squared[m] > best_distance_squared) {
-          best_n = m;
-          best_distance_squared = neighbor_distances_squared[m];
-        }
-      }
-      if (best_n >= 0 && distance_squared < best_distance_squared) {
-#pragma unroll
-        for (int m = 0; m < 4; ++m) {
-          if (m == best_n) { neighbor_surfel_indices[m] = q; neighbor_distances_squared[m] = distance_squared; }
-        }
-        changed = true;
-      }
-    }
-    if (changed) {
-#pragma unroll
-      for (int m = 0; m < 4; ++m) SM_SU(SM_ROW_NEIGHBOR0 + m, idx) = neighbor_surfel_indices[m];
-    }
-  });
-}
-#endif
+  const u32 n = *d.upd_count;
+  for (u32 k = blockIdx.x * blockDim.x + threadIdx.x; k < n; k += gridDim.x * blockDim.x) {
+    const uint2 w = d.upd_list[k];
+    update_neighbors_survivor(d, f, w.x, static_cast<int>(w.y & 0xFFFFu), static_cast<int>(w.y >> 16));
+  }
+}
 
 __device__ __forceinline__ unsigned long long load_scan_state(unsigned long long* p) { return atomicAdd(p, 0ull); }
 
@@ -1405,9 +1192,11 @@
     SM_S(SM_ROW_GRADIENT_COUNT, idx) = 0.f;
     d.gradient[idx] = make_float4(0.f, 0.f, 0.f, 0.f);
     const float rcp_count = frcp(i2f(existing_neighbor_count_plus_1));
-    SM_SMOOTH(0, idx) = fmul(fadd(g.x, sum_x), rcp_count);
-    SM_SMOOTH(1, idx) = fmul(fadd(g.y, sum_y), rcp_count);
-    SM_SMOOTH(2, idx) = fmul(fadd(g.z, sum_z), rcp_count);
+    const float sx = fmul(fadd(g.x, sum_x), rcp_count);
+    const float sy = fmul(fadd(g.y, sum_y), rcp_count);
+    const float sz = fmul(fadd(g.z, sum_z), rcp_count);
+    SM_SMOOTH(0, idx) = sx; SM_SMOOTH(1, idx) = sy; SM_SMOOTH(2, idx) = sz;
+    SM_SMOOTH_NEXT(0, idx) = sx; SM_SMOOTH_NEXT(1, idx) = sy; SM_SMOOTH_NEXT(2, idx) = sz;
   }
 }
 
@@ -1576,6 +1365,7 @@
   status = CheckLaunch("integrate (pipelined)");
   if (status != SM_OK) return status;
   const int old_slot = f.count_slot, new_slot = (f.count_slot + 1) % kCountSlots;
+  NoteIntegratedFrame(d, f.frame_index);
   if (reg.disable_denoising) {
     status = RegularizeSurfels(crit, d, true, f.frame_index, reg.radius_factor, reg.regularizer_weight, reg.window,
                                new_slot, old_slot, plan);
@@ -1633,9 +1423,6 @@
   plan->merge = resident(k_merge, kBlock, 4);
   plan->integrate = resident(k_integrate, kBlock, 3);
   plan->update_neighbors = resident(k_update_neighbors, kBlock, 3);
-#if SM_UPDATE_COMPACT
-  plan->update_neighbors = ScaleGrid(sm_count * 8);
-#endif
   if (const char* pe = std::getenv("SM_B200_OFFCHAIN_GRID_PERCENT")) {
     const int percent = std::atoi(pe);
     if (percent > 0 && percent < 100) {
diff --git a/surfelmeshing_b200/csrc/pipeline.cu b/surfelmeshing_b200/csrc/pipeline.cu
--- a/surfelmeshing_b200/csrc/pipeline.cu
+++ b/surfelmeshing_b200/csrc/pipeline.cu
@@ -128,6 +128,7 @@
     DeviceState d = r->d;
     d.assoc = r->assoc_set[set]; d.first_depth = r->first_depth_set[set]; d.supported = r->supported_set[set];
     d.vis = r->vis_set[set]; d.seg_count = r->seg_count_set[set]; d.merge_flag = r->merge_flag_set[set];
+    d.upd_list = r->upd_list_set[set]; d.upd_count = r->upd_count_set[set];
     return d;
   }
   FrameParams Params(int frame, int set) const {
@@ -265,6 +266,7 @@
     SM_CUDA(cudaStreamWaitEvent(pipelined ? r->pipe.front : stream, r->pre_done[set], 0));
     r->d.assoc = r->assoc_set[set]; r->d.first_depth = r->first_depth_set[set]; r->d.supported = r->supported_set[set];
     r->d.vis = r->vis_set[set]; r->d.seg_count = r->seg_count_set[set]; r->d.merge_flag = r->merge_flag_set[set];
+    r->d.upd_list = r->upd_list_set[set]; r->d.upd_count = r->upd_count_set[set];
     if (pipelined) {
       RecordOperation(r, static_cast<int>(static_cast<u32>(frame) - static_cast<u32>(c.ip->regularization_frame_window_size)));
       const FrameParams f = c.Params(frame, set);
@@ -475,6 +477,7 @@
         if (status != SM_OK) return status;
       }
       const int old_slot = f.count_slot, new_slot = (f.count_slot + 1) % kCountSlots;
+      if (active(crit)) NoteIntegratedFrame(d, static_cast<u32>(frame));
       for (int i = 0; i < (disable_denoising ? 1 : iterations); ++i) {
         KernelLaunch* first = &launches[l.reg0 + (disable_denoising ? 0 : 2 * i)];
         KernelLaunch* second = disable_denoising ? nullptr : first + 1;
@@ -486,8 +489,11 @@
           smooth_next = smooth;
           smooth = filled;
           d.smooth = smooth; d.smooth_next = smooth_next;
+          NoteRegStep(d, static_cast<u32>(frame), c.ip->regularization_frame_window_size);
         }
       }
+      r->d.reg_t_prev = d.reg_t_prev;
+      r->d.reg_full_sweep = d.reg_full_sweep;
       if (active(crit)) ++*integrated;
     }
     {
@@ -554,6 +560,7 @@
     const DeviceState last_set = c.SetState((c.last - 1) % kSets);
     r->d.assoc = last_set.assoc; r->d.first_depth = last_set.first_depth; r->d.supported = last_set.supported;
     r->d.vis = last_set.vis; r->d.seg_count = last_set.seg_count; r->d.merge_flag = last_set.merge_flag;
+    r->d.upd_list = last_set.upd_list; r->d.upd_count = last_set.upd_count;
   }
   r->count_slot = c.CountSlot(c.last);
   SM_CUDA(cudaEventRecord(r->graph_exit, gs));
diff --git a/surfelmeshing_b200/csrc/regularize.cu b/surfelmeshing_b200/csrc/regularize.cu
--- a/surfelmeshing_b200/csrc/regularize.cu
+++ b/surfelmeshing_b200/csrc/regularize.cu
@@ -29,6 +29,8 @@
   int count_slot;
   int remove_below_slot;
   int skip;
+  int t_prev;
+  int full_sweep;
 };
 
 __device__ __forceinline__ bool outside_window(u32 stamp, const RegParams& p) {
@@ -114,27 +116,21 @@
   const u32 n = d.counters->surfel_count[p.count_slot];
   const u32 step = gridDim.x * blockDim.x;
   u32 i = blockIdx.x * blockDim.x + threadIdx.x;
-  u32 stamp_ahead = 0, nbr_ahead[4] = {kInvalidIndex, kInvalidIndex, kInvalidIndex, kInvalidIndex};
-  if (i < d.stride) {
-    stamp_ahead = SM_SU(SM_ROW_LAST_UPDATE_STAMP, i);
-#pragma unroll
-    for (int k = 0; k < 4; ++k) nbr_ahead[k] = SM_SU(SM_ROW_NEIGHBOR0 + k, i);
-  }
+  u32 stamp_ahead = 0;
+  if (i < d.stride) stamp_ahead = SM_SU(SM_ROW_LAST_UPDATE_STAMP, i);
   for (; i < n; i += step) {
     const u32 stamp = stamp_ahead;
+    if (i + step < n) stamp_ahead = SM_SU(SM_ROW_LAST_UPDATE_STAMP, i + step);
+    if (outside_window(stamp, p)) {
+      if (p.full_sweep || static_cast<int>(stamp) >= p.t_prev) {
+        SM_SMOOTH_NEXT(0, i) = SM_SMOOTH(0, i); SM_SMOOTH_NEXT(1, i) = SM_SMOOTH(1, i); SM_SMOOTH_NEXT(2, i) = SM_SMOOTH(2, i);
+      }
+      continue;
+    }
     u32 nbr[4];
 #pragma unroll
-    for (int k = 0; k < 4; ++k) nbr[k] = nbr_ahead[k];
-    if (i + step < n) {
-      stamp_ahead = SM_SU(SM_ROW_LAST_UPDATE_STAMP, i + step);
-#pragma unroll
-      for (int k = 0; k < 4; ++k) nbr_ahead[k] = SM_SU(SM_ROW_NEIGHBOR0 + k, i + step);
-    }
+    for (int k = 0; k < 4; ++k) nbr[k] = SM_SU(SM_ROW_NEIGHBOR0 + k, i);
     const float sx = SM_SMOOTH(0, i), sy = SM_SMOOTH(1, i), sz = SM_SMOOTH(2, i);
-    if (outside_window(stamp, p)) {
-      SM_SMOOTH_NEXT(0, i) = sx; SM_SMOOTH_NEXT(1, i) = sy; SM_SMOOTH_NEXT(2, i) = sz;
-      continue;
-    }
     const float nx = SM_S(SM_ROW_NORMAL_X, i), ny = SM_S(SM_ROW_NORMAL_Y, i), nz = SM_S(SM_ROW_NORMAL_Z, i);
     const float4 accumulated = d.gradient[i];
     float gx = ffma(fsub(sx, SM_S(SM_ROW_X, i)), 2.0f, accumulated.x);
@@ -196,9 +192,9 @@
       }
     }
     if (outside_window(SM_SU(SM_ROW_LAST_UPDATE_STAMP, i), p)) continue;
-    SM_SMOOTH(0, i) = SM_S(SM_ROW_X, i);
-    SM_SMOOTH(1, i) = SM_S(SM_ROW_Y, i);
-    SM_SMOOTH(2, i) = SM_S(SM_ROW_Z, i);
+    const float x = SM_S(SM_ROW_X, i), y = SM_S(SM_ROW_Y, i), z = SM_S(SM_ROW_Z, i);
+    SM_SMOOTH(0, i) = x; SM_SMOOTH(1, i) = y; SM_SMOOTH(2, i) = z;
+    SM_SMOOTH_NEXT(0, i) = x; SM_SMOOTH_NEXT(1, i) = y; SM_SMOOTH_NEXT(2, i) = z;
   }
 }
 
@@ -232,6 +228,8 @@
   p.count_slot = count_slot;
   p.remove_below_slot = remove_replaced_below_slot;
   p.skip = skip ? 1 : 0;
+  p.t_prev = d.reg_t_prev;
+  p.full_sweep = d.reg_full_sweep;
   static_assert(sizeof(DeviceState) + sizeof(RegParams) + 32 <= sizeof(first->storage), "KernelLaunch::storage too small");
   if (disable_denoising) {
     first->Reset(reinterpret_cast<const void*>(k_reg_copy_only), dim3(plan.reg_copy), dim3(kBlock), 0, KID_REG_COPY_ONLY);
@@ -262,6 +260,7 @@
   float* const filled = d.smooth_next;
   d.smooth_next = d.smooth;
   d.smooth = filled;
+  NoteRegStep(d, frame_index, regularization_frame_window_size);
   return CheckLaunch("regularize");
 }
 
diff --git a/surfelmeshing_b200/csrc/sm_handle.cuh b/surfelmeshing_b200/csrc/sm_handle.cuh
--- a/surfelmeshing_b200/csrc/sm_handle.cuh
+++ b/surfelmeshing_b200/csrc/sm_handle.cuh
@@ -59,6 +59,8 @@
   smb::VisEntry* vis_set[smb::kSets] = {};
   smb::u32* seg_count_set[smb::kSets] = {};
   smb::u8* merge_flag_set[smb::kSets] = {};
+  uint2* upd_list_set[smb::kSets] = {};
+  smb::u32* upd_count_set[smb::kSets] = {};
   smb::u16* run_depth[smb::kSets] = {}; size_t run_depth_pitch = 0;
   float2* run_normals[smb::kSets] = {}; size_t run_normals_pitch = 0;
   float* run_radius[smb::kSets] = {}; size_t run_radius_pitch = 0;
diff --git a/surfelmeshing_b200/csrc/sm_kernels.cuh b/surfelmeshing_b200/csrc/sm_kernels.cuh
--- a/surfelmeshing_b200/csrc/sm_kernels.cuh
+++ b/surfelmeshing_b200/csrc/sm_kernels.cuh
@@ -146,6 +146,8 @@
   VisEntry* vis;
   u32* seg_count;
   u8* merge_flag;
+  uint2* upd_list;
+  u32* upd_count;
   u8* new_flag;
   u32* new_index;
   u32* new_list;
@@ -154,6 +156,8 @@
   float4* gradient;
   float* smooth;
   float* smooth_next;
+  int reg_t_prev;
+  int reg_full_sweep;
   unsigned long long* timeline;
   u32 timeline_frames;
 };
@@ -346,6 +350,13 @@
 int ExportVertices(cudaStream_t stream, const DeviceState& d, int count_slot, int sm_count, float* position_buffer,
                    u8* color_buffer);
 
+inline void NoteRegStep(DeviceState& d, u32 frame_index, int window) {
+  d.reg_t_prev = static_cast<int>(frame_index - static_cast<u32>(window));
+  d.reg_full_sweep = 0;
+}
+inline void NoteIntegratedFrame(DeviceState& d, u32 frame_index) {
+  if (static_cast<int>(frame_index) < d.reg_t_prev) d.reg_t_prev = static_cast<int>(frame_index);
+}
 int RebuildMetaRow(cudaStream_t stream, const DeviceState& d, u32 count, int sm_count);
 int RegularizeSurfels(cudaStream_t stream, DeviceState& d, bool disable_denoising, u32 frame_index,
                       float radius_factor_for_regularization_neighbors, float regularizer_weight,
```

Measured after the change: 9025, median of 6. 1.05x the previous value.
